# HuttleyLab/DiverseSeq

Hardware: AMD Instinct MI355X
Metric: sequences scored/sec (delta-JSD, k=6) (higher is better)
Workload: dtype f64 (results and every set update in f64; reject/accept decisions tiered: f32 and f32-log scores decide rows farther from the threshold than their proven error bands, f64 the rest)

## Files before the change

### diverseseq_amd/csrc/api.cpp

```cpp
#include "dvs_internal.h"

#include <cmath>
#include <cstring>
#include <mutex>

uint64_t dvs_pow_u64(uint32_t base, uint32_t exp, bool *overflow);
void dvs_matrix_free_fields(dvs_matrix *m);
int dvs_matrix_fill_counts(dvs_ctx *ctx, dvs_matrix *m, const dvs_seq_view &sv, const uint64_t *offsets, bool no_wait);
int dvs_matrix_fill_freq_entropy(dvs_ctx *ctx, dvs_matrix *m);
int dvs_hist_prepare(dvs_ctx *ctx, const uint64_t *offsets, uint32_t nseq, uint32_t k, uint64_t nbins, uint64_t nbytes, size_t *n_long_out);
bool dvs_hist_rows_fit_u16(const dvs_ctx *ctx, uint64_t B, size_t n_long);
int dvs_matrix_fill_freq_totals(dvs_ctx *ctx, dvs_matrix *m, const double *d_meta);
int dvs_matrix_fill_compacted(dvs_ctx *ctx, dvs_matrix *m, const double *d_in, const double *d_meta);

static std::string g_create_err;

int dvs_set_error(dvs_ctx *ctx, int code, const char *fmt, ...) {
    char buf[512];
    va_list ap;
    va_start(ap, fmt);
    vsnprintf(buf, sizeof buf, fmt, ap);
    va_end(ap);
    if (ctx) ctx->err = buf;
    else g_create_err = buf;
    return code;
}

int dvs_hip_fail(dvs_ctx *ctx, hipError_t e, const char *what) {
    (void)hipGetLastError();
    const int code = (e == hipErrorOutOfMemory) ? DVS_ERR_NOMEM : DVS_ERR_RUNTIME;
    return dvs_set_error(ctx, code, "HIP error %d (%s) in %s", int(e), hipGetErrorString(e), what);
}

int dvs_dev_alloc(dvs_ctx *ctx, void **ptr, size_t bytes, const char *what) {
    const size_t sz = ((bytes ? bytes : 1) + 4095) & ~size_t(4095);
    auto it = ctx->pool.find(sz);
    if (it != ctx->pool.end()) {
        *ptr = it->second;
        ctx->pool.erase(it);
        ctx->pool_bytes -= sz;
        ctx->live[*ptr] = sz;
        return DVS_OK;
    }
    hipError_t e = hipMalloc(ptr, sz);
    if (e != hipSuccess && !ctx->pool.empty()) {
        (void)hipGetLastError();
        dvs_dev_trim(ctx);
        e = hipMalloc(ptr, sz);
    }
    if (e != hipSuccess) {
        *ptr = nullptr;
        return dvs_hip_fail(ctx, e, what);
    }
    ctx->live[*ptr] = sz;
    return DVS_OK;
}

void dvs_dev_free(dvs_ctx *ctx, void *ptr) {
    if (!ptr) return;
    auto it = ctx ? ctx->live.find(ptr) : std::map<void *, size_t>::iterator();
    if (!ctx || it == ctx->live.end()) {
        (void)hipFree(ptr);
        return;
    }
    ctx->pool.emplace(it->second, ptr);
    ctx->pool_bytes += it->second;
    ctx->live.erase(it);
}

int dvs_pinned_get(dvs_ctx *ctx, void **ptr) {
    if (!ctx->pinned_pool.empty()) {
        *ptr = ctx->pinned_pool.back();
        ctx->pinned_pool.pop_back();
        return DVS_OK;
    }
    hipError_t e = hipHostMalloc(ptr, 4096, hipHostMallocDefault);
    if (e != hipSuccess) return dvs_hip_fail(ctx, e, "hipHostMalloc");
    return DVS_OK;
}
void dvs_pinned_put(dvs_ctx *ctx, void *ptr) {
    if (!ptr) return;
    if (ctx) ctx->pinned_pool.push_back(ptr);
    else (void)hipHostFree(ptr);
}
hipEvent_t dvs_event_get(dvs_ctx *ctx) {
    if (!ctx->event_pool.empty()) {
        hipEvent_t e = ctx->event_pool.back();
        ctx->event_pool.pop_back();
        return e;
    }
    hipEvent_t e = nullptr;
    (void)hipEventCreate(&e);
    return e;
}
void dvs_event_put(dvs_ctx *ctx, hipEvent_t e) {
    if (!e) return;
    if (ctx) ctx->event_pool.push_back(e);
    else (void)hipEventDestroy(e);
}

void dvs_dev_trim(dvs_ctx *ctx) {
    (void)hipStreamSynchronize(ctx->stream);
    for (auto &kv : ctx->pool) (void)hipFree(kv.second);
    ctx->pool.clear();
    ctx->pool_bytes = 0;
}

void dvs_knobs_from_env(dvs_knobs *k) {
    auto on = [](const char *name) { return getenv(name) != nullptr; };
    *k = dvs_knobs();
    k->no_uniform_offsets = on("DVS_NO_UNIFORM_OFFSETS");
    k->no_offsets_cache = on("DVS_NO_OFFSETS_CACHE");
    k->counts_u32 = on("DVS_COUNTS_U32");
    k->build_wait = on("DVS_BUILD_WAIT");
    k->no_packed_upload = on("DVS_NO_PACKED_UPLOAD");
    k->cu_mask_set = on("HSA_CU_MASK") || on("ROC_GLOBAL_CU_MASK");
    k->no_persist = on("DVS_NO_PERSIST");
    k->no_fast_step = on("DVS_NO_FAST_STEP");
    k->no_head_phase = on("DVS_NO_HEAD_PHASE");
    k->persist_no_seeded = on("DVS_PERSIST_NO_SEEDED");
    k->persist_no_small = on("DVS_PERSIST_NO_SMALL");
    k->persist_no_coarse = on("DVS_PERSIST_NO_COARSE");
    k->persist_no_events = on("DVS_PERSIST_NO_EVENTS");
    k->persist_debug = on("DVS_PERSIST_DEBUG");
    const char *rounds = getenv("DVS_PERSIST_WG_ROUNDS");
    k->persist_wg_rounds = rounds ? atoi(rounds) : -1;
    k->ingest_no_stream = on("DVS_INGEST_NO_STREAM");
    const char *tk = getenv("DVS_TEST_KNOBS");
    k->test_persist_fake_error = tk && strstr(tk, "fake_persist_error") != nullptr;
    if (const char *lt = tk ? strstr(tk, "long_tile_") : nullptr) k->test_long_tile = uint32_t(strtoul(lt + 10, nullptr, 10));
    k->test_rowlog_ring = 0;
    if (const char *rr = tk ? strstr(tk, "rowlog_ring_") : nullptr) k->test_rowlog_ring = uint32_t(strtoul(rr + 12, nullptr, 10));
}

extern "C" {

int dvs_abi_version(void) { return DVS_ABI_VERSION; }

int dvs_ctx_refresh_knobs(dvs_ctx *ctx) {
    if (!ctx) return dvs_set_error(ctx, DVS_ERR_VALUE, "null argument");
    dvs_knobs_from_env(&ctx->knobs);
    ctx->off_cache.n_off = 0;
    return DVS_OK;
}

int dvs_ctx_create(int device, void *stream, dvs_ctx **out) {
    if (!out) return dvs_set_error(nullptr, DVS_ERR_VALUE, "null argument");
    *out = nullptr;
    int ndev = 0;
    hipError_t e = hipGetDeviceCount(&ndev);
    if (e != hipSuccess || ndev == 0)
        return dvs_set_error(nullptr, DVS_ERR_RUNTIME,
                             "no HIP device available (%s): libdvs_hip has no CPU fallback",
                             e != hipSuccess ? hipGetErrorString(e) : "device count 0");
    if (device < 0) {
        e = hipGetDevice(&device);
        if (e != hipSuccess) return dvs_hip_fail(nullptr, e, "hipGetDevice");
    }
    if (device >= ndev)
        return dvs_set_error(nullptr, DVS_ERR_VALUE, "device %d out of range (%d devices)", device, ndev);
    e = hipSetDevice(device);
    if (e != hipSuccess) return dvs_hip_fail(nullptr, e, "hipSetDevice");
    hipDeviceProp_t prop;
    e = hipGetDeviceProperties(&prop, device);
    if (e != hipSuccess) return dvs_hip_fail(nullptr, e, "hipGetDeviceProperties");
    dvs_ctx *ctx = new dvs_ctx();
    dvs_knobs_from_env(&ctx->knobs);
    ctx->device = device;
    ctx->n_cu = prop.multiProcessorCount;
    ctx->lds_per_block = prop.sharedMemPerBlockOptin ? prop.sharedMemPerBlockOptin
                                                     : prop.sharedMemPerBlock;
    if (ctx->lds_per_block < prop.sharedMemPerBlock) ctx->lds_per_block = prop.sharedMemPerBlock;
    if (stream) {
        ctx->stream = static_cast<hipStream_t>(stream);
    } else {
        e = hipStreamCreateWithFlags(&ctx->stream, hipStreamNonBlocking);
        if (e != hipSuccess) {
            delete ctx;
            return dvs_hip_fail(nullptr, e, "hipStreamCreate");
        }
        ctx->own_stream = true;
    }
    *out = ctx;
    return DVS_OK;
}

void dvs_ctx_destroy(dvs_ctx *ctx) {
    if (!ctx || ctx->owner_gone) return;
    ctx->owner_gone = true;
    dvs_ctx_release(ctx);
}

}

int dvs_raise_dyn_lds(dvs_ctx *ctx, const void *fn, size_t bytes) {
    if (bytes <= 48 * 1024) return DVS_OK;
    size_t &have = ctx->lds_raised[fn];
    if (have >= bytes) return DVS_OK;
    DVS_HIP(ctx, hipFuncSetAttribute(fn, hipFuncAttributeMaxDynamicSharedMemorySize, int(bytes)));
    have = bytes;
    return DVS_OK;
}

hipStream_t dvs_ctx_stream2(dvs_ctx *ctx) {
    if (!ctx->stream2 && hipStreamCreateWithFlags(&ctx->stream2, hipStreamNonBlocking) != hipSuccess) {
        (void)hipGetLastError();
        ctx->stream2 = nullptr;
    }
    return ctx->stream2;
}

bool dvs_ctx_cu_split(dvs_ctx *ctx) {
    if (ctx->cu_split_tried) return ctx->stream_head != nullptr;
    ctx->cu_split_tried = true;
    if (ctx->n_cu < 128 || ctx->n_cu % 8) return false;
    if (ctx->knobs.cu_mask_set) return false;
    int head = 64;
    head = std::max(16, std::min(ctx->n_cu / 2, head)) & ~7;
    const uint32_t words = uint32_t(ctx->n_cu + 31) / 32;
    std::vector<uint32_t> lo(words, 0u), hi(words, 0u);
    for (int i = 0; i < ctx->n_cu; i++) (i < head ? lo : hi)[i / 32] |= 1u << (i % 32);
    hipStream_t a = nullptr, b = nullptr;
    if (hipExtStreamCreateWithCUMask(&a, words, lo.data()) != hipSuccess ||
        hipExtStreamCreateWithCUMask(&b, words, hi.data()) != hipSuccess) {
        (void)hipGetLastError();
        if (a) (void)hipStreamDestroy(a);
        return false;
    }
    ctx->stream_head = a;
    ctx->stream_rest = b;
    ctx->head_cus = head;
    return true;
}

void dvs_ctx_retain(dvs_ctx *ctx) {
    if (ctx) ctx->refs++;
}

void dvs_ctx_release(dvs_ctx *ctx) {
    if (!ctx || --ctx->refs > 0) return;
    (void)hipSetDevice(ctx->device);
    dvs_dev_free(ctx, ctx->off_cache.d_off);
    dvs_dev_free(ctx, ctx->off_cache.d_rows);
    dvs_dev_free(ctx, ctx->off_cache.d_tiles);
    if (ctx->off_cache.ev_up) (void)hipEventDestroy(ctx->off_cache.ev_up);
    if (ctx->off_cache.h_off) (void)hipHostFree(ctx->off_cache.h_off);
    if (ctx->pack_ev) (void)hipEventDestroy(ctx->pack_ev);
    if (ctx->h_pack) (void)hipHostFree(ctx->h_pack);
    dvs_dev_free(ctx, ctx->d_clog_tbl);
    dvs_dev_trim(ctx);
    for (void *p : ctx->pinned_pool) (void)hipHostFree(p);
    for (hipEvent_t e : ctx->event_pool) (void)hipEventDestroy(e);
    if (ctx->stream2) (void)hipStreamDestroy(ctx->stream2);
    if (ctx->stream_head) (void)hipStreamDestroy(ctx->stream_head);
    if (ctx->stream_rest) (void)hipStreamDestroy(ctx->stream_rest);
    if (ctx->own_stream && ctx->stream) (void)hipStreamDestroy(ctx->stream);
    delete ctx;
}

extern "C" {

const char *dvs_last_error(const dvs_ctx *ctx) { return ctx ? ctx->err.c_str() : g_create_err.c_str(); }

int dvs_ctx_trim(dvs_ctx *ctx) {
    if (!ctx) return DVS_ERR_VALUE;
    dvs_dev_trim(ctx);
    return DVS_OK;
}

int dvs_ctx_sync(dvs_ctx *ctx) {
    if (!ctx) return DVS_ERR_VALUE;
    DVS_HIP(ctx, hipStreamSynchronize(ctx->stream));
    return DVS_OK;
}

int dvs_ctx_set_timing(dvs_ctx *ctx, int on) {
    if (!ctx) return DVS_ERR_VALUE;
    ctx->timing = on != 0;
    return DVS_OK;
}

int dvs_ctx_device_info(dvs_ctx *ctx, char *name, size_t name_len, int *n_cu, uint64_t *hbm_bytes) {
    if (!ctx) return DVS_ERR_VALUE;
    hipDeviceProp_t prop;
    DVS_HIP(ctx, hipGetDeviceProperties(&prop, ctx->device));
    if (name && name_len) {
        snprintf(name, name_len, "%s (%s)", prop.name, prop.gcnArchName);
    }
    if (n_cu) *n_cu = prop.multiProcessorCount;
    if (hbm_bytes) *hbm_bytes = prop.totalGlobalMem;
    return DVS_OK;
}

static int matrix_alloc(dvs_ctx *ctx, dvs_matrix *m) {
    const size_t cells = size_t(m->nrows) * m->nbins;
    const size_t bytes = cells * (m->kind == 0 ? 4 : m->kind == 2 ? 2 : 8);
    size_t free_b = 0, total_b = 0;
    const bool cached = ctx->pool.count(((bytes ? bytes : 4) + 4095) & ~size_t(4095)) > 0;
    if (!cached) DVS_HIP(ctx, hipMemGetInfo(&free_b, &total_b));
    if (!cached && bytes + size_t(m->nrows) * 12 + (64u << 20) > free_b + ctx->pool_bytes)
        return dvs_set_error(ctx, DVS_ERR_NOMEM,
                             "%u x %llu matrix needs %zu bytes of HBM, %zu free", m->nrows,
                             (unsigned long long)m->nbins, bytes, free_b);
    const size_t nr = m->nrows ? m->nrows : 1;
    m->ctx = ctx;
    dvs_ctx_retain(ctx);
    int rc;
    if (m->kind == 0) rc = dvs_dev_alloc(ctx, (void **)&m->d_counts, bytes ? bytes : 4, "matrix counts");
    else if (m->kind == 2) rc = dvs_dev_alloc(ctx, (void **)&m->d_counts16, bytes ? bytes : 4, "matrix counts (16-bit)");
    else rc = dvs_dev_alloc(ctx, (void **)&m->d_freqs, bytes ? bytes : 8, "matrix freqs");
    if (!rc) rc = dvs_dev_alloc(ctx, (void **)&m->d_totals, nr * 4, "matrix totals");
    if (!rc) rc = dvs_dev_alloc(ctx, (void **)&m->d_entropy, nr * 8, "matrix entropy");
    return rc;
}

static int build_shape(dvs_ctx *ctx, uint32_t k, uint32_t num_states, uint64_t *B_out) {
    if (k == 0) return dvs_set_error(ctx, DVS_ERR_VALUE, "k cannot be 0");
    if (num_states < 1 || num_states > 255)
        return dvs_set_error(ctx, DVS_ERR_VALUE, "num_states %u outside 1..255", num_states);
    if (k > 17) return dvs_set_error(ctx, DVS_ERR_UNSUPPORTED, "k = %u > 17 is not supported", k);
    bool ovf = false;
    const uint64_t B = dvs_pow_u64(num_states, k, &ovf);
    if (ovf || B > (1ull << 32))
        return dvs_set_error(ctx, DVS_ERR_UNSUPPORTED, "%u^%u bins do not fit a dense count row",
                             num_states, k);
    *B_out = B;
    return DVS_OK;
}

static int matrix_build_view(dvs_ctx *ctx, const dvs_seq_view &sv, const uint64_t *offsets, uint32_t nseq, uint32_t k,
                             uint32_t num_states, bool no_wait, dvs_matrix **out) {
    *out = nullptr;
    uint64_t B = 0;
    const int arc = build_shape(ctx, k, num_states, &B);
    if (arc) return arc;
    size_t n_long = 0;
    if (nseq) {
        const int prc = dvs_hist_prepare(ctx, offsets, nseq, k, B, sv.nbytes, &n_long);
        if (prc) return prc;
    }
    dvs_matrix *m = new dvs_matrix();
    m->kind = (nseq && dvs_hist_rows_fit_u16(ctx, B, n_long)) ? 2 : 0;
    m->nrows = nseq;
    m->nbins = B;
    m->k = k;
    m->num_states = num_states;
    m->device = ctx->device;
    int rc = matrix_alloc(ctx, m);
    if (!rc && nseq) rc = dvs_matrix_fill_counts(ctx, m, sv, offsets, no_wait);
    if (rc) {
        dvs_matrix_free_fields(m);
        delete m;
        return rc;
    }
    *out = m;
    return DVS_OK;
}

int dvs_matrix_build(dvs_ctx *ctx, const uint8_t *seqs, int seqs_on_device, const uint64_t *offsets,
                     uint32_t nseq, uint32_t k, uint32_t num_states, dvs_matrix **out) {
    if (!ctx || !offsets || !out || (!seqs && nseq && offsets[nseq] > 0))
        return dvs_set_error(ctx, DVS_ERR_VALUE, "null argument");
    *out = nullptr;
    {
        uint64_t B_ = 0;
        const int arc = build_shape(ctx, k, num_states, &B_);
        if (arc) return arc;
    }
    DVS_HIP(ctx, hipSetDevice(ctx->device));
    const uint64_t nbytes = nseq ? offsets[nseq] : 0;
    dvs_seq_view sv;
    if (seqs_on_device) {
        if (reinterpret_cast<uintptr_t>(seqs) & 15)
            return dvs_set_error(ctx, DVS_ERR_VALUE, "device sequence buffer must be 16-byte aligned");
        sv.seqs = seqs;
        sv.nbytes = nbytes;
        return matrix_build_view(ctx, sv, offsets, nseq, k, num_states, !ctx->knobs.build_wait, out);
    }
    if (nbytes && dvs_packed_upload_wanted(ctx, num_states, nbytes)) {
        dvs_packed *p = nullptr;
        int rc = dvs_packed_alloc(ctx, nbytes, &p);
        if (!rc) rc = dvs_packed_fill_from_host(ctx, p, seqs);
        if (!rc) {
            sv.codes = p->d_codes;
            sv.mask = p->d_mask;
            sv.nbytes = nbytes;
            rc = matrix_build_view(ctx, sv, offsets, nseq, k, num_states, false, out);
        }
        if (p) {
            (void)hipStreamSynchronize(ctx->stream);
            dvs_packed_destroy(p);
        }
        return rc;
    }
    const uint64_t padded = ((nbytes + 15) & ~15ull) + 16;
    uint8_t *d_tmp = nullptr;
    int rc = dvs_dev_alloc(ctx, (void **)&d_tmp, padded, "sequence upload buffer");
    if (rc) return rc;
    hipError_t ue = hipMemsetAsync(d_tmp + (nbytes & ~15ull), 0xFF, padded - (nbytes & ~15ull), ctx->stream);
    if (ue == hipSuccess && nbytes) ue = hipMemcpyAsync(d_tmp, seqs, nbytes, hipMemcpyHostToDevice, ctx->stream);
    if (ue != hipSuccess) {
        (void)hipStreamSynchronize(ctx->stream);
        dvs_dev_free(ctx, d_tmp);
        return dvs_hip_fail(ctx, ue, "sequence upload");
    }
    sv.seqs = d_tmp;
    sv.nbytes = padded;
    rc = matrix_build_view(ctx, sv, offsets, nseq, k, num_states, false, out);
    (void)hipStreamSynchronize(ctx->stream);
    dvs_dev_free(ctx, d_tmp);
    return rc;
}

int dvs_matrix_build_packed(dvs_ctx *ctx, const dvs_packed *p, const uint64_t *offsets, uint32_t nseq, uint32_t k,
                            dvs_matrix **out) {
    if (!ctx || !p || !offsets || !out) return dvs_set_error(ctx, DVS_ERR_VALUE, "null argument");
    *out = nullptr;
    DVS_HIP(ctx, hipSetDevice(ctx->device));
    dvs_seq_view sv;
    sv.codes = p->d_codes;
    sv.mask = p->d_mask;
    sv.nbytes = p->nbases;
    p->async_readers = true;
    return matrix_build_view(ctx, sv, offsets, nseq, k, 4, !ctx->knobs.build_wait, out);
}

int dvs_matrix_from_freqs(dvs_ctx *ctx, const double *freqs, uint32_t nrows, uint64_t nbins,
                          dvs_matrix **out) {
    if (!ctx || !out || (!freqs && nrows)) return dvs_set_error(ctx, DVS_ERR_VALUE, "null argument");
    *out = nullptr;
    if (nbins == 0)
        return dvs_set_error(ctx, DVS_ERR_VALUE, "cannot calculate entropy as frequency vector empty");
    const double tol = double(nbins) * DVS_EPS;
    for (uint32_t r = 0; r < nrows; r++) {
        const double *row = freqs + uint64_t(r) * nbins;
        double tot = 0.0;
        for (uint64_t i = 0; i < nbins; i++)
            if (row[i] != 0.0) tot += row[i];
        if (!(std::fabs(tot - 1.0) <= tol))
            return dvs_set_error(ctx, DVS_ERR_VALUE,
                                 "cannot calculate entropy as frequency vector total %.17g!=1.0", tot);
    }
    DVS_HIP(ctx, hipSetDevice(ctx->device));
    dvs_matrix *m = new dvs_matrix();
    m->kind = 1;
    m->nrows = nrows;
    m->nbins = nbins;
    m->device = ctx->device;
    int rc = matrix_alloc(ctx, m);
    if (!rc && nrows) {
        std::vector<uint32_t> ones(nrows, 1u);
        hipError_t e = hipMemcpyAsync(m->d_freqs, freqs, size_t(nrows) * nbins * 8,
                                      hipMemcpyHostToDevice, ctx->stream);
        if (e == hipSuccess)
            e = hipMemcpyAsync(m->d_totals, ones.data(), size_t(nrows) * 4, hipMemcpyHostToDevice,
                               ctx->stream);
        if (e != hipSuccess) rc = dvs_hip_fail(ctx, e, "hipMemcpyAsync(freqs)");
        if (!rc) rc = dvs_matrix_fill_freq_entropy(ctx, m);
        if (!rc && hipStreamSynchronize(ctx->stream) != hipSuccess)
            rc = dvs_set_error(ctx, DVS_ERR_RUNTIME, "stream sync failed");
    }
    if (rc) {
        dvs_matrix_free_fields(m);
        delete m;
        return rc;
// ... 118 lines not shown
```

### diverseseq_amd/csrc/dvs_internal.h

```cpp
#pragma once

#include <hip/hip_runtime.h>

#include <cstdarg>
#include <cstdint>
#include <cstdio>
#include <map>
#include <string>
#include <vector>

#include "../../include/dvs_hip.h"

#define DVS_EPS 2.220446049250313e-16
#define DVS_HEAD_ROWS 1024u

struct dvs_knobs {
    bool no_uniform_offsets = false;
    bool no_offsets_cache = false;
    bool counts_u32 = false;
    bool build_wait = false;
    bool no_packed_upload = false;
    bool cu_mask_set = false;
    bool no_fast_step = false;
    bool no_persist = false;
    bool no_head_phase = false;
    bool persist_no_seeded = false;
    bool persist_no_small = false;
    bool persist_no_coarse = false;
    bool persist_no_events = false;
    bool persist_debug = false;
    int persist_wg_rounds = -1;
    bool ingest_no_stream = false;
    bool test_persist_fake_error = false;
    uint32_t test_long_tile = 0;
    uint32_t test_rowlog_ring = 0;
};
void dvs_knobs_from_env(dvs_knobs *k);

struct dvs_ctx {
    dvs_knobs knobs;
    int device = 0;
    hipStream_t stream = nullptr;
    bool own_stream = false;
    hipStream_t stream2 = nullptr;
    hipStream_t stream_head = nullptr, stream_rest = nullptr;
    int head_cus = 0;
    bool cu_split_tried = false;
    int persist_timeouts = 0;
    int n_cu = 0;
    size_t lds_per_block = 0;
    double *d_clog_tbl = nullptr;
    bool timing = false;
    std::string err;
    std::multimap<size_t, void *> pool;
    std::vector<void *> pinned_pool;
    std::vector<hipEvent_t> event_pool;
    std::map<void *, size_t> live;
    size_t pool_bytes = 0;
    int refs = 1;
    bool owner_gone = false;
    std::map<const void *, size_t> lds_raised;
    std::map<std::pair<const void *, size_t>, bool> persist_fits;
    struct OffsetsCache {
        uint64_t *h_off = nullptr;
        size_t h_cap = 0, n_off = 0;
        hipEvent_t ev_up = nullptr;
        std::vector<uint32_t> h_long_rows;
        std::vector<unsigned char> h_tiles;
        uint64_t nbytes = 0;
        uint32_t k = 0;
        void *d_off = nullptr, *d_rows = nullptr, *d_tiles = nullptr;
        size_t d_off_cap = 0;
        size_t n_long = 0, n_tiles = 0;
        bool uniform = false;
        uint64_t uni_base = 0, uni_stride = 0;
    } off_cache;
    void *h_pack = nullptr;
    size_t h_pack_cap = 0;
    hipEvent_t pack_ev = nullptr;
};
int dvs_raise_dyn_lds(dvs_ctx *ctx, const void *fn, size_t bytes);
void dvs_ctx_retain(dvs_ctx *ctx);
hipStream_t dvs_ctx_stream2(dvs_ctx *ctx);
bool dvs_ctx_cu_split(dvs_ctx *ctx);
void dvs_ctx_release(dvs_ctx *ctx);

struct dvs_matrix;
int dvs_matrix_settle(dvs_ctx *ctx, const dvs_matrix *m);
int dvs_dev_alloc(dvs_ctx *ctx, void **ptr, size_t bytes, const char *what);
void dvs_dev_free(dvs_ctx *ctx, void *ptr);
void dvs_dev_trim(dvs_ctx *ctx);
int dvs_pinned_get(dvs_ctx *ctx, void **ptr);
void dvs_pinned_put(dvs_ctx *ctx, void *ptr);
hipEvent_t dvs_event_get(dvs_ctx *ctx);
void dvs_event_put(dvs_ctx *ctx, hipEvent_t e);

int dvs_set_error(dvs_ctx *ctx, int code, const char *fmt, ...);
int dvs_hip_fail(dvs_ctx *ctx, hipError_t e, const char *what);

#define DVS_HIP(ctx, call)                                        \
    do {                                                          \
        hipError_t e__ = (call);                                  \
        if (e__ != hipSuccess) return dvs_hip_fail(ctx, e__, #call); \
    } while (0)

struct dvs_matrix {
    int kind = 0;
    uint16_t *d_counts16 = nullptr;
    uint32_t nrows = 0;
    uint64_t nbins = 0;
    uint32_t k = 0, num_states = 0;
    uint32_t *d_counts = nullptr;
    double *d_freqs = nullptr;
    uint32_t *d_totals = nullptr;
    double *d_entropy = nullptr;
    uint32_t *d_src_row = nullptr;
    std::vector<uint32_t> h_head_totals;
    uint32_t *h_head_pinned = nullptr;
    hipEvent_t ev_built = nullptr;
    hipEvent_t ev_join = nullptr;
    uint32_t head_count = 0;
    uint32_t head_rows_built = 0;
    bool rest_beside_head = false;
    int device = 0;
    dvs_ctx *ctx = nullptr;
};

struct dvs_packed {
    dvs_ctx *ctx = nullptr;
    uint32_t *d_codes = nullptr;
    uint16_t *d_mask = nullptr;
    uint64_t nbases = 0, nwords = 0;
    mutable bool async_readers = false;
};
struct dvs_seq_view {
    const uint8_t *seqs = nullptr;
    const uint32_t *codes = nullptr;
    const uint16_t *mask = nullptr;
    uint64_t nbytes = 0;
};
int dvs_packed_alloc(dvs_ctx *ctx, uint64_t nbases, dvs_packed **out);
int dvs_packed_fill_from_device(dvs_ctx *ctx, dvs_packed *p, const uint8_t *d_seqs);
int dvs_packed_fill_from_host(dvs_ctx *ctx, dvs_packed *p, const uint8_t *seqs);
bool dvs_packed_upload_wanted(const dvs_ctx *ctx, uint32_t num_states, uint64_t nbytes);

template <typename F>
auto dvs_mat_dispatch(const dvs_matrix *m, F &&f) {
    if (m->kind == 0) return f(static_cast<const uint32_t *>(m->d_counts));
    if (m->kind == 2) return f(static_cast<const uint16_t *>(m->d_counts16));
    return f(static_cast<const double *>(m->d_freqs));
}

#ifdef __HIPCC__
__device__ __forceinline__ uint32_t dvs_pack4(uint32_t w) {
    const uint32_t x = w & 0x03030303u;
    return ((x << 6) | (x >> 4) | (x >> 14) | (x >> 24)) & 0xFFu;
}
__device__ __forceinline__ uint32_t dvs_inv4(uint32_t w) {
    uint32_t t = w & 0xFCFCFCFCu;
    t |= t >> 4;
    t |= t >> 2;
    t |= t >> 1;
    t &= 0x01010101u;
    return ((t << 3) | (t >> 6) | (t >> 15) | (t >> 24)) & 0xFu;
}
__device__ __forceinline__ uint32_t dvs_pack16(uint4 v) {
    return (dvs_pack4(v.x) << 24) | (dvs_pack4(v.y) << 16) | (dvs_pack4(v.z) << 8) | dvs_pack4(v.w);
}
__device__ __forceinline__ uint32_t dvs_inv16(uint4 v) {
    return (dvs_inv4(v.x) << 12) | (dvs_inv4(v.y) << 8) | (dvs_inv4(v.z) << 4) | dvs_inv4(v.w);
}
__device__ __forceinline__ double dvs_wave_sum(double v) {
#pragma unroll
    for (int o = 32; o > 0; o >>= 1) v += __shfl_xor(v, o, 64);
    return v;
}
template <int CTRL>
__device__ __forceinline__ double dvs_dpp_mov(double v) {
    const long long b = __double_as_longlong(v);
    int lo = int(b), hi = int(b >> 32);
    lo = __builtin_amdgcn_update_dpp(0, lo, CTRL, 0xF, 0xF, true);
    hi = __builtin_amdgcn_update_dpp(0, hi, CTRL, 0xF, 0xF, true);
    return __longlong_as_double((long long)(((unsigned long long)(unsigned)hi << 32) | (unsigned)lo));
}
__device__ __forceinline__ double dvs_wave_sum_dpp(double v) {
    v += dvs_dpp_mov<0xB1>(v);
    v += dvs_dpp_mov<0x4E>(v);
    v += dvs_dpp_mov<0x141>(v);
    v += dvs_dpp_mov<0x140>(v);
    const long long b = __double_as_longlong(v);
    const int lo = int(b), hi = int(b >> 32);
    auto row = [&](int l) {
        return __longlong_as_double((long long)(((unsigned long long)(unsigned)__builtin_amdgcn_readlane(hi, l) << 32) |
                                                (unsigned)__builtin_amdgcn_readlane(lo, l)));
    };
    return (row(0) + row(16)) + (row(32) + row(48));
}
__device__ __forceinline__ double dvs_wave_min(double v) {
#pragma unroll
    for (int o = 32; o > 0; o >>= 1) v = fmin(v, __shfl_xor(v, o, 64));
    return v;
}
__device__ __forceinline__ double dvs_wave_min_dpp(double v) {
    v = fmin(v, dvs_dpp_mov<0xB1>(v));
    v = fmin(v, dvs_dpp_mov<0x4E>(v));
    v = fmin(v, dvs_dpp_mov<0x141>(v));
    v = fmin(v, dvs_dpp_mov<0x140>(v));
    const long long b = __double_as_longlong(v);
    const int lo = int(b), hi = int(b >> 32);
    auto row = [&](int l) {
        return __longlong_as_double((long long)(((unsigned long long)(unsigned)__builtin_amdgcn_readlane(hi, l) << 32) |
                                                (unsigned)__builtin_amdgcn_readlane(lo, l)));
    };
    return fmin(fmin(row(0), row(16)), fmin(row(32), row(48)));
}
__device__ __forceinline__ unsigned long long dvs_wave_sum_u64(unsigned long long v) {
#pragma unroll
    for (int o = 32; o > 0; o >>= 1) v += __shfl_xor(v, o, 64);
    return v;
}
__device__ __forceinline__ double dvs_block_sum(double v, double *scratch) {
    const int lane = threadIdx.x & 63, wave = threadIdx.x >> 6;
    const int nwave = (blockDim.x + 63) >> 6;
    v = dvs_wave_sum(v);
    __syncthreads();
    if (lane == 0) scratch[wave] = v;
    __syncthreads();
    double t = 0.0;
    for (int i = 0; i < nwave; i++) t += scratch[i];
    return t;
}
__device__ __forceinline__ double dvs_block_min(double v, double *scratch) {
    const int lane = threadIdx.x & 63, wave = threadIdx.x >> 6;
    const int nwave = (blockDim.x + 63) >> 6;
    v = dvs_wave_min(v);
    __syncthreads();
    if (lane == 0) scratch[wave] = v;
    __syncthreads();
    double t = scratch[0];
    for (int i = 1; i < nwave; i++) t = fmin(t, scratch[i]);
    return t;
}
#endif
```

### diverseseq_amd/csrc/kmer_hist.hip

```cpp
#include "dvs_internal.h"

#include <algorithm>
#include <cstring>
#include <cmath>
#include <cstdlib>

namespace {

constexpr int HIST_THREADS = 256;
constexpr int HIST_MAX_THREADS = 512;
constexpr uint32_t TILE_LEN = 32768;
static_assert(TILE_LEN < 65536, "a whole-sequence tile's counts must fit the packed 16-bit LDS counters");
constexpr int CLOG_TBL = 256;

struct KTile {
    uint64_t begin;
    uint64_t end;
    uint64_t seq_begin;
    uint32_t row;
    uint32_t single;
};

__device__ __forceinline__ uint4 load16(const uint8_t *base, uint64_t off, uint64_t nbytes) {
    if (off + 16 <= nbytes) return *reinterpret_cast<const uint4 *>(base + off);
    uint32_t w[4] = {0xFFFFFFFFu, 0xFFFFFFFFu, 0xFFFFFFFFu, 0xFFFFFFFFu};
    for (int i = 0; i < 16; i++) {
        if (off + i < nbytes) {
            w[i >> 2] &= ~(0xFFu << (8 * (i & 3)));
            w[i >> 2] |= uint32_t(base[off + i]) << (8 * (i & 3));
        }
    }
    return make_uint4(w[0], w[1], w[2], w[3]);
}

template <bool LDS_HIST, bool PK16 = false>
__device__ __forceinline__ void bump(uint32_t *hist, uint32_t idx) {
    if (PK16) atomicAdd(&hist[idx >> 1], (idx & 1u) ? 0x10000u : 1u);
    else atomicAdd(&hist[idx], 1u);
}

__device__ __forceinline__ double clog2c(uint32_t c, const double *tbl) {
    if (c < CLOG_TBL) return tbl[c];
    const double d = double(c);
    return d * log2(d);
}

template <bool NS4, bool LDS_HIST, bool PK16 = false, bool OUT16 = false, bool PACKED = false>
__global__ __launch_bounds__(HIST_MAX_THREADS) void kmer_hist_kernel(
    const uint8_t *__restrict__ seqs, const uint16_t *__restrict__ pmask, uint64_t nbytes,
    const uint64_t *__restrict__ offsets,
    const KTile *__restrict__ tiles, uint32_t *__restrict__ counts, uint32_t *__restrict__ totals,
    double *__restrict__ entropy, const double *__restrict__ clog_tbl, uint32_t k, uint32_t ns,
    uint64_t B, uint32_t hot_rows, uint32_t row0, uint64_t uni_base, uint64_t uni_stride) {
    extern __shared__ __attribute__((aligned(16))) unsigned char smem[];
    KTile t;
    if (tiles) {
        t = tiles[blockIdx.x];
    } else {
        const uint32_t r = row0 + (hot_rows ? gridDim.x - 1 - blockIdx.x : blockIdx.x);
        const uint64_t s0 = offsets ? offsets[r] : uni_base + uint64_t(r) * uni_stride;
        const uint64_t s1 = offsets ? offsets[r + 1] : s0 + uni_stride;
        t.row = r;
        t.single = 1;
        t.seq_begin = s0;
        t.begin = s0 + k - 1;
        t.end = s1;
        if (s1 - s0 >= k && s1 - t.begin > TILE_LEN) return;
        if (s1 - s0 < k) t.begin = t.end = s1;
    }
    static_assert(!OUT16 || PK16, "16-bit rows come from the packed histogram");
    static_assert(!PACKED || NS4, "only four-state sequences have a packed form");
    uint32_t *row = OUT16 ? counts + uint64_t(t.row) * (B / 2) : counts + uint64_t(t.row) * B;
    uint32_t *hist = LDS_HIST ? reinterpret_cast<uint32_t *>(smem) : row;
    double *tbl = reinterpret_cast<double *>(smem + (LDS_HIST ? ((B * (PK16 ? 2 : 4) + 15) & ~15ull) : 0));
    double *scratch = tbl + CLOG_TBL;
    const int tid = threadIdx.x;
    const int nthreads = blockDim.x;

    if (LDS_HIST) {
        if ((B & 3) == 0) {
            uint4 *h4 = reinterpret_cast<uint4 *>(hist);
            for (uint64_t i = tid; i < B / (PK16 ? 8 : 4); i += nthreads) h4[i] = make_uint4(0, 0, 0, 0);
            if (PK16 && (B & 7) && tid == 0) reinterpret_cast<uint2 *>(hist)[B / 4 - 1] = make_uint2(0, 0);
        } else {
            for (uint64_t i = tid; i < B; i += nthreads) hist[i] = 0;
        }
    }
    for (int i = tid; i < CLOG_TBL; i += nthreads) tbl[i] = clog_tbl[i];
    __syncthreads();

    uint32_t nvalid = 0;
    const uint64_t abase = t.begin & ~15ull;
    const uint64_t nchunks = t.end > t.begin ? (t.end - abase + 15) >> 4 : 0;
    const uint32_t bmask = uint32_t(B - 1);

    if (NS4) {
        const uint32_t lane = tid & 63, wave = tid >> 6, nwaves = (nthreads + 63) >> 6;
        const uint64_t per_wave = ((nchunks + nwaves - 1) / nwaves + 63) & ~63ull;
        const uint64_t c_lo = uint64_t(wave) * per_wave;
        const uint64_t c_hi = c_lo + per_wave < nchunks ? c_lo + per_wave : nchunks;
        uint32_t carryP = 0, carryI = 0xFFFFu;
        if (c_lo < c_hi) {
            const uint64_t A0 = abase + (c_lo << 4);
            if (A0 >= 16) {
                if constexpr (PACKED) {
                    carryP = reinterpret_cast<const uint32_t *>(seqs)[(A0 >> 4) - 1];
                    carryI = pmask[(A0 >> 4) - 1];
                } else {
                    const uint4 pv = load16(seqs, A0 - 16, nbytes);
                    carryP = dvs_pack16(pv);
                    carryI = dvs_inv16(pv);
                }
            }
        }
        for (uint64_t c0 = c_lo; c0 < c_hi; c0 += 64) {
            const uint64_t c = c0 + lane;
            const bool live = c < c_hi;
            const uint64_t A = abase + ((live ? c : c_hi - 1) << 4);
            uint32_t Pc, Ic = 0;
            if constexpr (PACKED) {
                Pc = reinterpret_cast<const uint32_t *>(seqs)[A >> 4];
                Ic = pmask[A >> 4];
            } else {
                const uint4 cur = load16(seqs, A, nbytes);
                Pc = dvs_pack16(cur);
                const uint32_t hib = (cur.x | cur.y | cur.z | cur.w) & 0xFCFCFCFCu;
                if (__ballot(hib != 0)) Ic = dvs_inv16(cur);
            }
            const uint32_t Pp = uint32_t(__builtin_amdgcn_update_dpp(int(carryP), int(Pc), 0x138, 0xF, 0xF, false));
            const uint32_t Ip = uint32_t(__builtin_amdgcn_update_dpp(int(carryI), int(Ic), 0x138, 0xF, 0xF, false));
            carryP = uint32_t(__builtin_amdgcn_readlane(int(Pc), 63));
            carryI = uint32_t(__builtin_amdgcn_readlane(int(Ic), 63));
            const uint64_t P = (uint64_t(Pp) << 32) | Pc;
            uint32_t I = (Ip << 16) | Ic;
            const int64_t lead = int64_t(t.seq_begin) - (int64_t(A) - 16);
            if (lead > 0) I |= (lead >= 32) ? 0xFFFFFFFFu : ~(0xFFFFFFFFu >> lead);
            uint32_t W = I;
            if (__ballot(I != 0)) {
                uint32_t cover = 1;
                while (2 * cover <= k) {
                    W |= W >> cover;
                    cover *= 2;
                }
                if (cover < k) W |= W >> (k - cover);
            }
            const uint32_t lo = t.begin > A ? uint32_t(t.begin - A < 16 ? t.begin - A : 16) : 0u;
            const uint32_t hi = t.end > A ? uint32_t(t.end - A < 16 ? t.end - A : 16) : 0u;
            const uint32_t R = (live && hi > lo) ? ((0xFFFFu >> lo) & ~(0xFFFFu >> hi)) : 0u;
            const uint32_t ok = R & ~W & 0xFFFFu;
            nvalid += __popc(ok);
            if (__ballot(ok != 0xFFFFu) == 0) {
                if constexpr (PK16) {
                    const uint64_t P2 = P << 1;
                    const uint32_t p2lo = uint32_t(P2), p2hi = uint32_t(P2 >> 32);
                    const uint32_t amask = (bmask << 1) & ~3u;
                    unsigned char *hb = smem;
#pragma unroll
                    for (int j = 0; j < 16; j++) {
                        const uint32_t tq = __builtin_amdgcn_alignbit(p2hi, p2lo, 2 * (15 - j));
                        uint32_t half = __builtin_amdgcn_ubfe(tq, 1, 1);
                        asm volatile("" : "+v"(half));
                        atomicAdd(reinterpret_cast<uint32_t *>(hb + (tq & amask)), __umul24(half, 0xFFFFu) + 1u);
                    }
                } else {
#pragma unroll
                    for (int j = 0; j < 16; j++) bump<LDS_HIST, PK16>(hist, uint32_t(P >> (2 * (15 - j))) & bmask);
                }
            } else {
#pragma unroll
                for (int j = 0; j < 16; j++) {
                    const uint32_t idx = uint32_t(P >> (2 * (15 - j))) & bmask;
                    if ((ok >> (15 - j)) & 1u) bump<LDS_HIST, PK16>(hist, idx);
                }
            }
        }
    } else {
        for (uint64_t c = tid; c < nchunks; c += nthreads) {
            const uint64_t A = abase + (c << 4);
            const uint4 cur = load16(seqs, A, nbytes);
            const uint4 prev = (A >= 16) ? load16(seqs, A - 16, nbytes)
                                         : make_uint4(0xFFFFFFFFu, 0xFFFFFFFFu, 0xFFFFFFFFu, 0xFFFFFFFFu);
            const int64_t lead = int64_t(t.seq_begin) - (int64_t(A) - 16);
            const uint32_t w[8] = {prev.x, prev.y, prev.z, prev.w, cur.x, cur.y, cur.z, cur.w};
            uint32_t idx = 0, run = 0;
            const uint32_t Bd = uint32_t(B / ns);
#pragma unroll
            for (int q = 0; q < 32; q++) {
                const uint32_t b = (w[q >> 2] >> (8 * (q & 3))) & 0xFFu;
                const bool ok = (b < ns) && (int64_t(q) >= lead);
                idx = ok ? (idx % Bd) * ns + b : 0u;
                run = ok ? run + 1 : 0u;
                if (q >= 16) {
                    const uint64_t p = A + (q - 16);
                    if (p >= t.begin && p < t.end && run >= k) {
                        bump<LDS_HIST, PK16>(hist, idx);
                        nvalid++;
                    }
                }
            }
        }
    }
    if (!LDS_HIST) __threadfence();
    __syncthreads();

    if constexpr (PK16) {
        const uint2 *h2 = reinterpret_cast<const uint2 *>(hist);
        uint4 *r4 = reinterpret_cast<uint4 *>(row);
        typedef uint32_t u32x4 __attribute__((ext_vector_type(4)));
        double sv[2] = {0.0, 0.0}, tv[2] = {0.0, 0.0};
#pragma unroll
        for (int half = 0; half < 2; half++)
            for (uint64_t u = uint64_t(tid) + 128u * half; u < B / 4; u += HIST_THREADS) {
                const uint2 w = h2[u];
                const uint4 v = make_uint4(w.x & 0xFFFFu, w.x >> 16, w.y & 0xFFFFu, w.y >> 16);
                if constexpr (OUT16) {
                    typedef uint32_t u32x2 __attribute__((ext_vector_type(2)));
                    uint2 *r2 = reinterpret_cast<uint2 *>(row);
                    if (t.row < hot_rows) r2[u] = w;
                    else __builtin_nontemporal_store((u32x2){w.x, w.y}, reinterpret_cast<u32x2 *>(r2 + u));
                } else if (t.row < hot_rows) r4[u] = v;
                else __builtin_nontemporal_store((u32x4){v.x, v.y, v.z, v.w}, reinterpret_cast<u32x4 *>(r4 + u));
                if (((w.x | w.y) & 0xFF00FF00u) == 0) sv[half] += ((tbl[v.x] + tbl[v.y]) + tbl[v.z]) + tbl[v.w];
                else sv[half] += clog2c(v.x, tbl) + clog2c(v.y, tbl) + clog2c(v.z, tbl) + clog2c(v.w, tbl);
            }
        tv[0] = double(nvalid);
        const int lane = tid & 63, wave = tid >> 6;
        double sums[2];
#pragma unroll
        for (int q = 0; q < 2; q++) {
            const double a = dvs_wave_sum(q ? tv[0] : sv[0]), b = dvs_wave_sum(q ? tv[1] : sv[1]);
            __syncthreads();
            if (lane == 0) {
                scratch[wave] = a;
                scratch[wave + 2] = b;
            }
            __syncthreads();
            double acc = 0.0;
            for (int i = 0; i < 4; i++) acc += scratch[i];
            sums[q] = acc;
        }
        if (tid == 0) {
            totals[t.row] = uint32_t(sums[1]);
            entropy[t.row] = sums[1] > 0.0 ? log2(sums[1]) - sums[0] / sums[1] : 0.0;
        }
    } else if (t.single) {
        double s = 0.0, tot = 0.0;
        if (tid >= HIST_THREADS) {
        } else if (LDS_HIST) {
            if ((B & 3) == 0) {
                const uint4 *h4 = reinterpret_cast<const uint4 *>(hist);
                uint4 *r4 = reinterpret_cast<uint4 *>(row);
                for (uint64_t i = tid; i < B / 4; i += HIST_THREADS) {
                    const uint4 v = h4[i];
                    typedef uint32_t u32x4 __attribute__((ext_vector_type(4)));
                    if (t.row < hot_rows) r4[i] = v;
                    else __builtin_nontemporal_store((u32x4){v.x, v.y, v.z, v.w}, reinterpret_cast<u32x4 *>(r4 + i));
                    s += clog2c(v.x, tbl) + clog2c(v.y, tbl) + clog2c(v.z, tbl) + clog2c(v.w, tbl);
                    tot += double(v.x) + double(v.y) + double(v.z) + double(v.w);
                }
            } else {
                for (uint64_t i = tid; i < B; i += HIST_THREADS) {
                    const uint32_t v = hist[i];
                    row[i] = v;
                    s += clog2c(v, tbl);
                    tot += double(v);
                }
            }
        } else {
            for (uint64_t i = tid; i < B; i += HIST_THREADS) {
                const uint32_t v = __hip_atomic_load(&row[i], __ATOMIC_RELAXED, __HIP_MEMORY_SCOPE_AGENT);
                s += clog2c(v, tbl);
                tot += double(v);
            }
        }
        s = dvs_block_sum(s, scratch);
        tot = dvs_block_sum(tot, scratch);
        if (tid == 0) {
            totals[t.row] = uint32_t(tot);
            entropy[t.row] = tot > 0.0 ? log2(tot) - s / tot : 0.0;
        }
    } else if (LDS_HIST) {
        for (uint64_t i = tid; i < B; i += nthreads) {
            const uint32_t v = hist[i];
            if (v) atomicAdd(&row[i], v);
        }
    }
}

__global__ void clog_tbl_kernel(double *tbl) {
    const int c = threadIdx.x;
    tbl[c] = c ? double(c) * log2(double(c)) : 0.0;
}

__global__ __launch_bounds__(HIST_THREADS) void row_stats_kernel(
    const uint32_t *__restrict__ counts, const uint32_t *__restrict__ rows,
    uint32_t *__restrict__ totals, double *__restrict__ entropy, uint64_t B) {
    __shared__ double tbl[CLOG_TBL];
    __shared__ double scratch[32];
    const int tid = threadIdx.x;
    if (tid < CLOG_TBL) tbl[tid] = tid ? double(tid) * log2(double(tid)) : 0.0;
    __syncthreads();
    const uint32_t r = rows[blockIdx.x];
    const uint32_t *row = counts + uint64_t(r) * B;
    double s = 0.0, tot = 0.0;
    for (uint64_t i = tid; i < B; i += HIST_THREADS) {
        const uint32_t v = row[i];
        s += clog2c(v, tbl);
        tot += double(v);
    }
    s = dvs_block_sum(s, scratch);
    tot = dvs_block_sum(tot, scratch);
    if (tid == 0) {
        totals[r] = uint32_t(tot);
        entropy[r] = tot > 0.0 ? log2(tot) - s / tot : 0.0;
    }
}

__global__ __launch_bounds__(HIST_THREADS) void zero_rows_kernel(uint32_t *__restrict__ counts,
                                                                const uint32_t *__restrict__ rows,
                                                                uint64_t B) {
    uint32_t *row = counts + uint64_t(rows[blockIdx.x]) * B;
    for (uint64_t i = threadIdx.x; i < B; i += HIST_THREADS) row[i] = 0;
}

__global__ __launch_bounds__(HIST_THREADS) void freq_entropy_kernel(
    const double *__restrict__ freqs, double *__restrict__ entropy, uint64_t B) {
    __shared__ double scratch[32];
    const double *row = freqs + uint64_t(blockIdx.x) * B;
    double h = 0.0;
    for (uint64_t i = threadIdx.x; i < B; i += HIST_THREADS) {
        const double f = row[i];
        if (f != 0.0) h += -f * log2(f);
    }
    h = dvs_block_sum(h, scratch);
    if (threadIdx.x == 0) entropy[blockIdx.x] = h;
}

__global__ __launch_bounds__(HIST_THREADS) void compact_freq_rows_kernel(
    const double *__restrict__ in, const double *__restrict__ meta, double *__restrict__ out,
    uint32_t *__restrict__ totals, uint32_t *__restrict__ src, uint32_t nrows, uint64_t B) {
    __shared__ uint32_t s_cnt[2];
    const uint32_t r = blockIdx.x;
    if (threadIdx.x < 2) s_cnt[threadIdx.x] = 0;
    __syncthreads();
    uint32_t before = 0, all = 0;
    for (uint32_t q = threadIdx.x; q < nrows; q += HIST_THREADS) {
        const uint32_t v = meta[2 * q + 1] != 0.0 ? 1u : 0u;
        all += v;
        if (q < r) before += v;
    }
    atomicAdd(&s_cnt[0], before);
    atomicAdd(&s_cnt[1], all);
    __syncthreads();
    const bool real = meta[2 * r + 1] != 0.0;
    const uint32_t dest = real ? s_cnt[0] : s_cnt[1] + (r - s_cnt[0]);
    const double *a = in + uint64_t(r) * B;
    double *o = out + uint64_t(dest) * B;
    for (uint64_t i = threadIdx.x; i < B; i += HIST_THREADS) o[i] = a[i];
    if (threadIdx.x == 0) {
        totals[dest] = real ? 1u : 0u;
        src[dest] = r;
    }
}

__global__ void freq_totals_kernel(uint32_t *__restrict__ totals, const double *__restrict__ meta,
                                   uint32_t nrows) {
    const uint32_t r = blockIdx.x * blockDim.x + threadIdx.x;
    if (r < nrows) totals[r] = (!meta || meta[2 * r + 1] != 0.0) ? 1u : 0u;
}

template <typename K>
int set_dyn_lds(dvs_ctx *ctx, K kernel, size_t bytes) {
    return dvs_raise_dyn_lds(ctx, reinterpret_cast<const void *>(kernel), bytes);
}

}

uint64_t dvs_pow_u64(uint32_t base, uint32_t exp, bool *overflow) {
    uint64_t r = 1;
    *overflow = false;
    for (uint32_t i = 0; i < exp; i++) {
        if (r > UINT64_MAX / (base ? base : 1)) *overflow = true;
        r *= base;
    }
    return r;
}

int dvs_matrix_settle(dvs_ctx *ctx, const dvs_matrix *cm) {
    dvs_matrix *m = const_cast<dvs_matrix *>(cm);
    if (!m || !m->ev_built) return DVS_OK;
    const hipError_t e = hipEventSynchronize(m->ev_built);
    if (e == hipSuccess) m->h_head_totals.assign(m->h_head_pinned, m->h_head_pinned + m->head_count);
    else m->h_head_totals.clear();
    dvs_event_put(m->ctx, m->ev_built);
    dvs_pinned_put(m->ctx, m->h_head_pinned);
    m->ev_built = nullptr;
    m->h_head_pinned = nullptr;
    if (e != hipSuccess) return dvs_hip_fail(ctx ? ctx : m->ctx, e, "histogram kernels");
    return DVS_OK;
}

void dvs_matrix_free_fields(dvs_matrix *m) {
    if (!m) return;
    (void)dvs_matrix_settle(m->ctx, m);
    if (m->ev_join) dvs_event_put(m->ctx, m->ev_join);
    m->ev_join = nullptr;
    dvs_dev_free(m->ctx, m->d_counts);
    dvs_dev_free(m->ctx, m->d_counts16);
    m->d_counts16 = nullptr;
    dvs_dev_free(m->ctx, m->d_freqs);
    dvs_dev_free(m->ctx, m->d_totals);
    dvs_dev_free(m->ctx, m->d_entropy);
    dvs_dev_free(m->ctx, m->d_src_row);
    m->d_src_row = nullptr;
    m->d_counts = nullptr;
    m->d_freqs = nullptr;
    m->d_totals = nullptr;
    m->d_entropy = nullptr;
    dvs_ctx_release(m->ctx);
    m->ctx = nullptr;
}

int dvs_hist_prepare(dvs_ctx *ctx, const uint64_t *offsets, uint32_t nseq, uint32_t k, uint64_t nbins, uint64_t nbytes,
                     size_t *n_long_out) {
    dvs_ctx::OffsetsCache &oc = ctx->off_cache;
    const size_t n_off = size_t(nseq) + 1;
    oc.uniform = false;
    if (nseq >= 1 && !ctx->knobs.no_uniform_offsets) {
        const uint64_t base = offsets[0], stride = offsets[1] - offsets[0];
        bool uni = offsets[1] >= offsets[0] && stride < uint64_t(TILE_LEN) + k;
        uint64_t diff = 0;
        for (uint32_t r = 0; r < nseq && uni; r += 4096) {
            const uint32_t e = std::min<uint32_t>(nseq, r + 4096);
            for (uint32_t q = r; q < e; q++) diff |= (offsets[q + 1] - offsets[q]) ^ stride;
            uni = diff == 0;
        }
        if (uni && base + uint64_t(nseq) * stride <= nbytes) {
            dvs_dev_free(ctx, oc.d_rows);
            dvs_dev_free(ctx, oc.d_tiles);
            oc.d_rows = oc.d_tiles = nullptr;
            oc.n_long = oc.n_tiles = 0;
            oc.n_off = 0;
            oc.uniform = true;
            oc.uni_base = base;
            oc.uni_stride = stride;
            *n_long_out = 0;
            return DVS_OK;
        }
    }
    const bool hit = oc.d_off && oc.h_off && oc.k == k && oc.nbytes == nbytes && oc.n_off == n_off &&
                     !ctx->knobs.no_offsets_cache && std::memcmp(oc.h_off, offsets, n_off * 8) == 0;
    if (!hit) {
        if (oc.ev_up) (void)hipEventSynchronize(oc.ev_up);
        if (oc.h_cap < n_off) {
            if (oc.h_off) (void)hipHostFree(oc.h_off);
            oc.h_off = nullptr;
            oc.h_cap = 0;
            const size_t cap = std::max<size_t>(n_off + n_off / 4, 1024);
            const hipError_t he = hipHostMalloc((void **)&oc.h_off, cap * 8, hipHostMallocDefault);
            if (he != hipSuccess) {
                oc.h_off = nullptr;
                return dvs_hip_fail(ctx, he, "pinned offsets block");
            }
            oc.h_cap = cap;
        }
        oc.n_off = 0;
        std::vector<KTile> tiles;
        std::vector<uint32_t> long_rows;
        uint64_t *dst = oc.h_off;
        uint64_t bad = 0, longest = 0;
        dst[0] = offsets[0];
        for (uint32_t r = 0; r < nseq; r++) {
            const uint64_t s0 = offsets[r], s1 = offsets[r + 1];
            dst[r + 1] = s1;
            bad |= uint64_t(s1 < s0) | uint64_t(s1 > nbytes);
            const uint64_t len = s1 - s0;
            longest = len > longest ? len : longest;
        }
        if (bad || longest >= uint64_t(TILE_LEN) + k) {
            uint64_t long_windows = 0;
            for (uint32_t r = 0; r < nseq; r++) {
                const uint64_t s0 = offsets[r], s1 = offsets[r + 1];
                if (s1 < s0 || s1 > nbytes)
                    return dvs_set_error(ctx, DVS_ERR_VALUE, "offsets[%u..%u] = %llu..%llu out of range", r,
                                         r + 1, (unsigned long long)s0, (unsigned long long)s1);
                if (s1 - s0 >= k && s1 - (s0 + k - 1) > TILE_LEN) long_windows += s1 - (s0 + k - 1);
            }
            uint64_t tile_long = TILE_LEN;
            {
                const uint64_t B_ = nbins ? nbins : 1;
                while (tile_long < 262144 && tile_long < 16 * B_ && long_windows / (2 * tile_long) >= 2048) tile_long *= 2;
                if (ctx->knobs.test_long_tile >= TILE_LEN) tile_long = std::min<uint64_t>(ctx->knobs.test_long_tile, uint64_t(1) << 20);
            }
            for (uint32_t r = 0; r < nseq; r++) {
                const uint64_t s0 = offsets[r], s1 = offsets[r + 1];
                if (s1 - s0 < k) continue;
                const uint64_t first = s0 + k - 1;
                if (s1 - first <= TILE_LEN) continue;
                long_rows.push_back(r);
                for (uint64_t b = first; b < s1; b += tile_long) {
                    KTile t;
                    t.begin = b;
                    t.end = std::min<uint64_t>(b + tile_long, s1);
                    t.seq_begin = s0;
                    t.row = r;
                    t.single = 0;
                    tiles.push_back(t);
                }
            }
        }
        dvs_dev_free(ctx, oc.d_rows);
        dvs_dev_free(ctx, oc.d_tiles);
        oc.d_rows = oc.d_tiles = nullptr;
        oc.n_long = oc.n_tiles = 0;
        int arc = DVS_OK;
        if (oc.d_off_cap < n_off) {
            dvs_dev_free(ctx, oc.d_off);
            oc.d_off = nullptr;
            oc.d_off_cap = 0;
            arc = dvs_dev_alloc(ctx, &oc.d_off, (n_off + n_off / 4) * 8, "offsets");
            if (!arc) oc.d_off_cap = n_off + n_off / 4;
        }
        if (!arc && !long_rows.empty()) arc = dvs_dev_alloc(ctx, &oc.d_rows, long_rows.size() * 4, "row list");
        if (!arc && !tiles.empty()) arc = dvs_dev_alloc(ctx, &oc.d_tiles, tiles.size() * sizeof(KTile), "tile list");
        hipError_t ue = hipSuccess;
        oc.h_tiles.assign(reinterpret_cast<const unsigned char *>(tiles.data()),
                          reinterpret_cast<const unsigned char *>(tiles.data()) + tiles.size() * sizeof(KTile));
        oc.h_long_rows = long_rows;
        if (!arc) ue = hipMemcpyAsync(oc.d_off, oc.h_off, n_off * 8, hipMemcpyHostToDevice, ctx->stream);
        if (!arc && ue == hipSuccess) {
            if (!oc.ev_up) oc.ev_up = dvs_event_get(ctx);
            if (oc.ev_up) ue = hipEventRecord(oc.ev_up, ctx->stream);
        }
        if (!arc && ue == hipSuccess && !long_rows.empty()) {
            ue = hipMemcpyAsync(oc.d_rows, oc.h_long_rows.data(), long_rows.size() * 4, hipMemcpyHostToDevice, ctx->stream);
            if (ue == hipSuccess)
                ue = hipMemcpyAsync(oc.d_tiles, oc.h_tiles.data(), oc.h_tiles.size(), hipMemcpyHostToDevice,
                                    ctx->stream);
        }
        if (arc || ue != hipSuccess) {
            dvs_dev_free(ctx, oc.d_rows);
            dvs_dev_free(ctx, oc.d_tiles);
            oc.d_rows = oc.d_tiles = nullptr;
            return arc ? arc : dvs_hip_fail(ctx, ue, "histogram setup");
        }
        oc.n_off = n_off;
        oc.nbytes = nbytes;
        oc.k = k;
        oc.n_long = long_rows.size();
        oc.n_tiles = tiles.size();
    }
    *n_long_out = oc.n_long;
    return DVS_OK;
}

bool dvs_hist_rows_fit_u16(const dvs_ctx *ctx, uint64_t B, size_t n_long) {
    return n_long == 0 && B <= 4096 && (B & 3) == 0 && !ctx->knobs.counts_u32;
}

int dvs_matrix_fill_counts(dvs_ctx *ctx, dvs_matrix *m, const dvs_seq_view &sv, const uint64_t *offsets,
                           bool no_wait) {
    const bool packed = sv.codes != nullptr;
    const uint8_t *d_seqs = packed ? reinterpret_cast<const uint8_t *>(sv.codes) : sv.seqs;
    const uint16_t *d_pmask = sv.mask;
    const uint64_t nbytes = sv.nbytes;
    const uint32_t nseq = m->nrows, k = m->k, ns = m->num_states;
    if (packed && ns != 4) return dvs_set_error(ctx, DVS_ERR_VALUE, "packed sequences have four states, not %u", ns);
    const uint64_t B = m->nbins;
    const bool lds_hist = B * 4 <= 64 * 1024;
    const bool ns4 = ns == 4;
    (void)offsets;
    dvs_ctx::OffsetsCache &oc = ctx->off_cache;
    uint64_t *d_off = oc.uniform ? nullptr : static_cast<uint64_t *>(oc.d_off);
    const uint64_t uni_base = oc.uni_base, uni_stride = oc.uni_stride;
    uint32_t *d_rows = static_cast<uint32_t *>(oc.d_rows);
    KTile *d_tiles = static_cast<KTile *>(oc.d_tiles);
    const size_t n_long = oc.n_long, n_tiles = oc.n_tiles;
    auto cleanup = [&]() {};
    int rc = DVS_OK;
    hipError_t e = hipSuccess;
    if (!lds_hist)
        e = hipMemsetAsync(m->d_counts, 0, size_t(nseq) * B * 4, ctx->stream);
    if (e == hipSuccess && n_long && lds_hist)
        hipLaunchKernelGGL(zero_rows_kernel, dim3(uint32_t(n_long)), dim3(HIST_THREADS), 0, ctx->stream,
                           m->d_counts, d_rows, B);
    if (e != hipSuccess) return dvs_hip_fail(ctx, e, "histogram setup");
    if (!ctx->d_clog_tbl) {
        rc = dvs_dev_alloc(ctx, (void **)&ctx->d_clog_tbl, CLOG_TBL * sizeof(double), "c log2 c table");
        if (rc) {
            cleanup();
            return rc;
        }
        hipLaunchKernelGGL(clog_tbl_kernel, dim3(1), dim3(CLOG_TBL), 0, ctx->stream, ctx->d_clog_tbl);
    }
    int nthreads = HIST_THREADS;
    const int tile_threads = (lds_hist && B * 4 > 32768) ? HIST_MAX_THREADS : HIST_THREADS;
    const size_t lds = (lds_hist ? ((B * 4 + 15) & ~15ull) : 0) + (CLOG_TBL + 32) * sizeof(double);
#define DVS_LAUNCH_HIST(NS4, LH, PKD, GRID, TILES, NTHR, HOT)                                             \
    do {                                                                                         \
        rc = set_dyn_lds(ctx, kmer_hist_kernel<NS4, LH, false, false, PKD>, lds);                \
        if (!rc)                                                                                 \
            hipLaunchKernelGGL((kmer_hist_kernel<NS4, LH, false, false, PKD>), dim3(GRID), dim3(NTHR), lds,  \
                               ctx->stream, d_seqs, d_pmask, nbytes, d_off, TILES, m->d_counts,  \
                               m->d_totals, m->d_entropy, ctx->d_clog_tbl, k, ns, B, HOT, 0u, uni_base, uni_stride);   \
    } while (0)
#define DVS_LAUNCH_HIST_ANY(GRID, TILES, NTHR, HOT)                            \
    do {                                                                  \
        if (packed && lds_hist) DVS_LAUNCH_HIST(true, true, true, GRID, TILES, NTHR, HOT);   \
        else if (packed) DVS_LAUNCH_HIST(true, false, true, GRID, TILES, NTHR, HOT);         \
        else if (ns4 && lds_hist) DVS_LAUNCH_HIST(true, true, false, GRID, TILES, NTHR, HOT);   \
        else if (ns4) DVS_LAUNCH_HIST(true, false, false, GRID, TILES, NTHR, HOT);         \
        else if (lds_hist) DVS_LAUNCH_HIST(false, true, false, GRID, TILES, NTHR, HOT);    \
        else DVS_LAUNCH_HIST(false, false, false, GRID, TILES, NTHR, HOT);                 \
    } while (0)
    uint32_t hot_rows = uint32_t(std::min<uint64_t>(nseq, (192ull << 20) / (B * (m->kind == 2 ? 2 : 4))));
    const bool pk16 = lds_hist && (B & 3) == 0;
    uint32_t head_rows = 0;
    if (m->kind == 2 && no_wait) {
        uint32_t want = DVS_HEAD_ROWS;
        head_rows = std::min<uint32_t>(nseq, want);
    }
    if (head_rows == nseq) head_rows = 0;
    bool head_event_done = false;
    if (m->kind == 2) {
        const size_t lds16 = ((B * 2 + 15) & ~15ull) + (CLOG_TBL + 32) * sizeof(double);
        uint32_t *out16 = reinterpret_cast<uint32_t *>(m->d_counts16);
        auto launch16 = [&](uint32_t row0, uint32_t count, uint32_t hot_end, hipStream_t on) {
            if (packed) {
                rc = set_dyn_lds(ctx, kmer_hist_kernel<true, true, true, true, true>, lds16);
                if (!rc)
                    hipLaunchKernelGGL((kmer_hist_kernel<true, true, true, true, true>), dim3(count), dim3(128), lds16, on,
                                       d_seqs, d_pmask, nbytes, d_off, static_cast<const KTile *>(nullptr), out16,
                                       m->d_totals, m->d_entropy, ctx->d_clog_tbl, k, ns, B, hot_end, row0, uni_base, uni_stride);
            } else if (ns4) {
                rc = set_dyn_lds(ctx, kmer_hist_kernel<true, true, true, true>, lds16);
                if (!rc)
                    hipLaunchKernelGGL((kmer_hist_kernel<true, true, true, true>), dim3(count), dim3(128), lds16, on,
                                       d_seqs, d_pmask, nbytes, d_off, static_cast<const KTile *>(nullptr), out16,
                                       m->d_totals, m->d_entropy, ctx->d_clog_tbl, k, ns, B, hot_end, row0, uni_base, uni_stride);
            } else {
                rc = set_dyn_lds(ctx, kmer_hist_kernel<false, true, true, true>, lds16);
                if (!rc)
                    hipLaunchKernelGGL((kmer_hist_kernel<false, true, true, true>), dim3(count), dim3(128), lds16, on,
                                       d_seqs, d_pmask, nbytes, d_off, static_cast<const KTile *>(nullptr), out16,
                                       m->d_totals, m->d_entropy, ctx->d_clog_tbl, k, ns, B, hot_end, row0, uni_base, uni_stride);
            }
        };
        if (head_rows) {
            const bool split = nseq - head_rows >= 16u * head_rows && dvs_ctx_cu_split(ctx);
            hipEvent_t ev_fork = split ? dvs_event_get(ctx) : nullptr;
            bool forked = ev_fork && hipEventRecord(ev_fork, ctx->stream) == hipSuccess &&
                          hipStreamWaitEvent(ctx->stream_rest, ev_fork, 0) == hipSuccess;
            launch16(0, head_rows, head_rows, ctx->stream);
            void *pin = nullptr;
            if (!rc && dvs_pinned_get(ctx, &pin) == DVS_OK) {
                m->head_count = uint32_t(std::min<size_t>(head_rows, 4096 / sizeof(uint32_t)));
                m->h_head_pinned = static_cast<uint32_t *>(pin);
                m->ev_built = dvs_event_get(ctx);
                if (m->ev_built &&
                    hipMemcpyAsync(m->h_head_pinned, m->d_totals, size_t(m->head_count) * 4, hipMemcpyDeviceToHost,
                                   ctx->stream) == hipSuccess &&
                    hipEventRecord(m->ev_built, ctx->stream) == hipSuccess) {
                    head_event_done = true;
                    m->head_rows_built = head_rows;
                } else {
                    if (m->ev_built) dvs_event_put(ctx, m->ev_built);
                    dvs_pinned_put(ctx, pin);
                    m->ev_built = nullptr;
                    m->h_head_pinned = nullptr;
                }
            }
            if (!rc) {
                const uint32_t hot_end = uint32_t(std::min<uint64_t>(nseq, uint64_t(head_rows) + hot_rows));
                forked = forked && head_event_done;
                launch16(head_rows, nseq - head_rows, hot_end, forked ? ctx->stream_rest : ctx->stream);
                if (forked) {
                    hipEvent_t ev_join = dvs_event_get(ctx);
                    if (!ev_join || hipEventRecord(ev_join, ctx->stream_rest) != hipSuccess ||
                        hipStreamWaitEvent(ctx->stream, ev_join, 0) != hipSuccess) {
                        (void)hipGetLastError();
                        (void)hipStreamSynchronize(ctx->stream_rest);
                    } else {
                        m->rest_beside_head = true;
                    }
                    m->ev_join = ev_join;
                }
            }
            if (ev_fork) dvs_event_put(ctx, ev_fork);
        } else {
            launch16(0, nseq, hot_rows, ctx->stream);
        }
    } else if (pk16) {
        const size_t lds16 = ((B * 2 + 15) & ~15ull) + (CLOG_TBL + 32) * sizeof(double);
        if (packed) {
            rc = set_dyn_lds(ctx, kmer_hist_kernel<true, true, true, false, true>, lds16);
            if (!rc)
                hipLaunchKernelGGL((kmer_hist_kernel<true, true, true, false, true>), dim3(nseq), dim3(128), lds16, ctx->stream,
                                   d_seqs, d_pmask, nbytes, d_off, static_cast<const KTile *>(nullptr), m->d_counts,
                                   m->d_totals, m->d_entropy, ctx->d_clog_tbl, k, ns, B, hot_rows, 0u, uni_base, uni_stride);
        } else if (ns4) {
            rc = set_dyn_lds(ctx, kmer_hist_kernel<true, true, true>, lds16);
            if (!rc)
                hipLaunchKernelGGL((kmer_hist_kernel<true, true, true>), dim3(nseq), dim3(128), lds16, ctx->stream,
                                   d_seqs, d_pmask, nbytes, d_off, static_cast<const KTile *>(nullptr), m->d_counts,
                                   m->d_totals, m->d_entropy, ctx->d_clog_tbl, k, ns, B, hot_rows, 0u, uni_base, uni_stride);
        } else {
            rc = set_dyn_lds(ctx, kmer_hist_kernel<false, true, true>, lds16);
            if (!rc)
                hipLaunchKernelGGL((kmer_hist_kernel<false, true, true>), dim3(nseq), dim3(128), lds16, ctx->stream,
                                   d_seqs, d_pmask, nbytes, d_off, static_cast<const KTile *>(nullptr), m->d_counts,
                                   m->d_totals, m->d_entropy, ctx->d_clog_tbl, k, ns, B, hot_rows, 0u, uni_base, uni_stride);
        }
    } else
        DVS_LAUNCH_HIST_ANY(nseq, static_cast<const KTile *>(nullptr), nthreads, hot_rows);
    if (!rc && n_tiles) {
        DVS_LAUNCH_HIST_ANY(uint32_t(n_tiles), d_tiles, tile_threads, 0u);
        if (!rc)
            hipLaunchKernelGGL(row_stats_kernel, dim3(uint32_t(n_long)), dim3(HIST_THREADS), 0,
                               ctx->stream, m->d_counts, d_rows, m->d_totals, m->d_entropy, B);
    }
#undef DVS_LAUNCH_HIST_ANY
#undef DVS_LAUNCH_HIST
    if (!rc && (e = hipGetLastError()) != hipSuccess) rc = dvs_hip_fail(ctx, e, "histogram launch");
    if (!rc && no_wait && head_event_done) return DVS_OK;
    if (!rc && no_wait) {
        void *pin = nullptr;
        if (dvs_pinned_get(ctx, &pin) == DVS_OK) {
            m->head_count = uint32_t(std::min<size_t>(nseq, 4096 / sizeof(uint32_t)));
            m->h_head_pinned = static_cast<uint32_t *>(pin);
            m->ev_built = dvs_event_get(ctx);
            if (m->ev_built &&
                hipMemcpyAsync(m->h_head_pinned, m->d_totals, size_t(m->head_count) * 4, hipMemcpyDeviceToHost,
                               ctx->stream) == hipSuccess &&
                hipEventRecord(m->ev_built, ctx->stream) == hipSuccess) {
                cleanup();
                return DVS_OK;
            }
            if (m->ev_built) dvs_event_put(ctx, m->ev_built);
            dvs_pinned_put(ctx, pin);
            m->ev_built = nullptr;
            m->h_head_pinned = nullptr;
        }
    }
    m->h_head_totals.assign(std::min<size_t>(nseq, 4096), 0u);
    if (!rc && !m->h_head_totals.empty() &&
        hipMemcpyAsync(m->h_head_totals.data(), m->d_totals, m->h_head_totals.size() * 4, hipMemcpyDeviceToHost,
                       ctx->stream) != hipSuccess)
        m->h_head_totals.clear();
    if (hipStreamSynchronize(ctx->stream) != hipSuccess && !rc)
        rc = dvs_set_error(ctx, DVS_ERR_RUNTIME, "histogram kernels failed");
    cleanup();
    return rc;
}

int dvs_matrix_fill_freq_entropy(dvs_ctx *ctx, dvs_matrix *m) {
    hipLaunchKernelGGL(freq_entropy_kernel, dim3(m->nrows), dim3(HIST_THREADS), 0, ctx->stream,
                       m->d_freqs, m->d_entropy, m->nbins);
    DVS_HIP(ctx, hipGetLastError());
    return DVS_OK;
}

int dvs_matrix_fill_compacted(dvs_ctx *ctx, dvs_matrix *m, const double *d_in, const double *d_meta) {
    hipLaunchKernelGGL(compact_freq_rows_kernel, dim3(m->nrows), dim3(HIST_THREADS), 0, ctx->stream, d_in, d_meta,
                       m->d_freqs, m->d_totals, m->d_src_row, m->nrows, m->nbins);
    DVS_HIP(ctx, hipGetLastError());
    return DVS_OK;
}

int dvs_matrix_fill_freq_totals(dvs_ctx *ctx, dvs_matrix *m, const double *d_meta) {
    hipLaunchKernelGGL(freq_totals_kernel, dim3((m->nrows + 255) / 256), dim3(256), 0, ctx->stream,
                       m->d_totals, d_meta, m->nrows);
    DVS_HIP(ctx, hipGetLastError());
    return DVS_OK;
}
```

### diverseseq_amd/csrc/persist.hip

```cpp
#include "select_dev.h"

#include <algorithm>
#include <type_traits>
#include <cstddef>
#include <cstdlib>
#include <cstring>

namespace {

constexpr int P_THREADS = 512;
constexpr int P_J = 8;
constexpr int P_CH = 16;
constexpr uint32_t P_MAXN = 512;
constexpr uint32_t P_MAXN_BIG = 256;
constexpr uint32_t P_MAXN_MAX = 896;
constexpr uint32_t p_maxn(bool cached, bool maxm = false) { return cached ? (maxm ? P_MAXN_MAX : P_MAXN) : P_MAXN_BIG; }
constexpr uint32_t P_SMALLN = 16;
constexpr uint32_t P_SMALL_ROWS = 13;
constexpr uint32_t p_maxjobs(bool cached, bool maxm = false) { return p_maxn(cached, maxm) + 1; }
constexpr size_t p_acc_bytes(uint32_t maxn) { return size_t(8) * (maxn + 1) * 2 * sizeof(unsigned long long); }
__device__ __forceinline__ unsigned long long p_acc_word(double v) {
    return ((unsigned long long)__double2ll_rn(v * 0x1p50) << 6) + 1ull;
}
__device__ __forceinline__ double p_acc_value(unsigned long long w) { return double((long long)w >> 6) * 0x1p-50; }
// ... 79 lines not shown
constexpr uint32_t P_TAG0 = 0xFFFFFEu;
constexpr uint32_t P_EPOCH_MAX = 0xFFFFF0u;
constexpr unsigned long long P_POS_NONE = (1ull << 37) - 1;
__device__ __forceinline__ unsigned long long p_word(uint32_t epoch, uint64_t pos, bool sure) {
    return ((unsigned long long)(P_TAG0 - epoch) << 40) | ((pos == SEL_NONE ? P_POS_NONE : pos) << 3) | (sure ? 0ull : 1ull);
}
__device__ __forceinline__ bool p_word_is(unsigned long long w, uint32_t epoch) { return uint32_t(w >> 40) == P_TAG0 - epoch; }
__device__ __forceinline__ uint64_t p_word_pos(unsigned long long w, uint32_t epoch) {
    const unsigned long long pos = (w >> 3) & P_POS_NONE;
    return (!p_word_is(w, epoch) || pos == P_POS_NONE) ? SEL_NONE : uint64_t(pos);
}
__device__ __forceinline__ bool p_word_sure(unsigned long long w) { return (w & 1ull) == 0; }
__device__ __forceinline__ uint32_t p_word_listed(unsigned long long w) { return uint32_t(w >> 1) & 3u; }

__device__ bool grid_barrier(PSync *sync, uint32_t G, uint32_t &gen, int *s_ok) {
    __syncthreads();
    if (threadIdx.x == 0) {
        const uint32_t target = gen + 1;
        const uint32_t x = blockIdx.x & 7u, ng = G < 8u ? G : 8u;
        const uint32_t gsz = (G - x + 7u) >> 3;
        int ok = 1;
        bool released = false;
        const bool last = G <= P_FLAT_GRID
                              ? __hip_atomic_fetch_add(&sync->count, 1u, RLX_AGENT) == G * target - 1
                              : (__hip_atomic_fetch_add(&sync->gcount[x].v, 1u, RLX_AGENT) == gsz * target - 1 &&
                                 __hip_atomic_fetch_add(&sync->count, 1u, RLX_AGENT) == ng * target - 1);
        if (last) {
            for (uint32_t g = 0; g < ng; g++) __hip_atomic_store(&sync->ggen[g].v, target, RLX_AGENT);
            released = true;
        }
        if (!released) {
            uint32_t spins = 0;
            while (__hip_atomic_load(&sync->ggen[x].v, RLX_AGENT) < target) {
                if ((++spins & 255u) == 0 &&
                    (spins > P_SPIN_LIMIT || __hip_atomic_load(&sync->timeout, RLX_AGENT))) {
                    __hip_atomic_store(&sync->timeout, 1u, RLX_AGENT);
                    ok = 0;
                    break;
                }
                __builtin_amdgcn_s_sleep(1);
            }
        }
        *s_ok = ok;
    }
    __syncthreads();
    gen++;
    return *s_ok != 0;
}

__device__ __forceinline__ uint4 p_load16_agent(const void *ptr) {
    uint4 v;
    asm volatile("global_load_dwordx4 %0, %1, off sc1\n\ts_waitcnt vmcnt(0)" : "=v"(v) : "v"(ptr) : "memory");
    return v;
}

struct PWin {
    uint32_t epoch;
    const unsigned long long *hintp;
    PRel *rel;
    unsigned long long *wgev;
    uint32_t *nlist;
    unsigned long long *mysoft;
};
__device__ __forceinline__ uint64_t p_hint_pos(const PWin &w) {
    return p_word_pos(__hip_atomic_load(w.hintp, RLX_AGENT), w.epoch);
}
__device__ __forceinline__ void p_post_event_wave(const PWin &w, uint64_t p, bool sure, uint32_t lane) {
    const unsigned long long word = p_word(w.epoch, p, sure);
    if (lane == 0) atomicMin(w.wgev, word);
    if (lane < 8) atomicMin(&w.rel[lane].hint, word);
}
__device__ __forceinline__ void p_post_event_thread(const PWin &w, uint64_t p, bool sure) {
    const unsigned long long word = p_word(w.epoch, p, sure);
    atomicMin(w.wgev, word);
    for (uint32_t g = 0; g < 8; g++) atomicMin(&w.rel[g].hint, word);
}
__device__ __forceinline__ void p_list_candidate(const PWin &w, uint64_t p) {
    const uint32_t idx = atomicAdd(w.nlist, 1u);
    if (idx < P_LIST) __hip_atomic_store(w.mysoft + idx, p_word(w.epoch, p, false), RLX_AGENT);
    else p_post_event_thread(w, p, false);
}
template <int CTRL>
__device__ __forceinline__ unsigned long long p_dpp_mov_u64(unsigned long long v) {
    int lo = int(uint32_t(v)), hi = int(uint32_t(v >> 32));
    lo = __builtin_amdgcn_update_dpp(0, lo, CTRL, 0xF, 0xF, true);
    hi = __builtin_amdgcn_update_dpp(0, hi, CTRL, 0xF, 0xF, true);
    return ((unsigned long long)uint32_t(hi) << 32) | uint32_t(lo);
}
__device__ __forceinline__ unsigned long long p_wave_min_u64(unsigned long long v) {
    auto mn = [](unsigned long long a, unsigned long long b) { return b < a ? b : a; };
    v = mn(v, p_dpp_mov_u64<0xB1>(v));
    v = mn(v, p_dpp_mov_u64<0x4E>(v));
    v = mn(v, p_dpp_mov_u64<0x141>(v));
    v = mn(v, p_dpp_mov_u64<0x140>(v));
    const int lo = int(uint32_t(v)), hi = int(uint32_t(v >> 32));
    auto row = [&](int l) {
        return ((unsigned long long)uint32_t(__builtin_amdgcn_readlane(hi, l)) << 32) | uint32_t(__builtin_amdgcn_readlane(lo, l));
    };
    return mn(mn(row(0), row(16)), mn(row(32), row(48)));
}

__device__ __forceinline__ unsigned long long p_gather(PSync *sync, uint32_t G, uint32_t epoch, unsigned long long own,
                                                       uint32_t lane, bool &ok, unsigned long long *seen_all = nullptr,
                                                       unsigned long long *stored = nullptr) {
    constexpr uint32_t Q = P_MAXG / 64;
    unsigned long long w[Q];
    bool have[Q];
#pragma unroll
    for (uint32_t q = 0; q < Q; q++) {
        w[q] = ~0ull;
        have[q] = lane + 64 * q >= G - 1;
    }
    uint32_t spins = 0;
    ok = true;
    for (;;) {
        unsigned long long got[Q];
#pragma unroll
        for (uint32_t q = 0; q < Q; q++)
            got[q] = have[q] ? 0ull : __hip_atomic_load(&sync->wrec[epoch & 1u][lane + 64 * q], RLX_AGENT);
        bool all = true;
#pragma unroll
        for (uint32_t q = 0; q < Q; q++) {
            if (!have[q] && p_word_is(got[q], epoch)) {
                w[q] = got[q];
                have[q] = true;
            }
            all = all && have[q];
        }
        if (__ballot(!all) == 0ull) break;
        if ((++spins & 255u) == 0 && (spins > P_SPIN_LIMIT || __hip_atomic_load(&sync->timeout, RLX_AGENT))) {
            ok = false;
            break;
        }
        __builtin_amdgcn_s_sleep(1);
    }
    if (seen_all) *seen_all = __builtin_amdgcn_s_memrealtime();
    unsigned long long m = own & ~6ull, fl = own & 6ull;
#pragma unroll
    for (uint32_t q = 0; q < Q; q++)
        if (lane + 64 * q < G - 1 && have[q]) {
            m = (w[q] & ~6ull) < m ? (w[q] & ~6ull) : m;
            fl |= w[q] & 6ull;
        }
    m = p_wave_min_u64(m);
    const bool anyl = __ballot(fl != 0ull) != 0ull;
    const unsigned long long relw = m | (anyl ? 2ull : 0ull);
    if (ok && lane < 8) __hip_atomic_store(&sync->rel[lane].rel, relw, RLX_AGENT);
    if (!ok && lane == 0) __hip_atomic_store(&sync->timeout, 1u, RLX_AGENT);
    if (stored) *stored = __builtin_amdgcn_s_memrealtime();
    return relw;
}

template <typename T, bool COARSE>
__device__ __forceinline__ void p_scan_rows(const T *__restrict__ mat,
                                            const uint32_t *__restrict__ totals,
                                            const double *__restrict__ rowH, const double *sl,
                                            const float *slf, uint64_t B, const PState &st, double he_base,
                                            const PWin &win,
                                            uint64_t first, uint64_t stride, uint64_t nrows,
                                            uint32_t lane, uint32_t &nread,
                                            uint32_t &nprecise, uint32_t &nmid, bool coarse_on,
                                            bool burst_drop = true) {
    const double dn = double(st.n), rn = 1.0 / dn;
    const double thr_lo = st.thr - st.band;
    const double thr_fast = thr_lo - FAST_BAND, thr_sure = st.thr + st.band + FAST_BAND;
    (void)thr_lo;
    const bool vec = (B & 255) == 0;
    const double cband = coarse_band(B);
    const double thr_c_lo = st.thr - st.band - cband, thr_c_hi = st.thr + st.band + cband;
    for (uint64_t r = first; r < nrows; r += stride) {
        const uint64_t p = st.cursor + r;
        const T *rp = mat + p * B;
        const uint64_t ev = p_hint_pos(win);
        const uint32_t tot = totals[p];
        const double hrow = rowH[p];
        if (ev < p) break;
        if (tot == 0) continue;
        const double rt = 1.0 / double(tot);
        const double mean_entropy = (he_base + hrow) / dn;
        nread++;
        if constexpr (COARSE) {
            if (vec && coarse_on) {
                const float rtn = float(rt * rn);
                const dvs_f2 r2 = {rtn, rtn};
                double c0 = 0.0, c1 = 0.0;
                bool done16 = false;
                if constexpr (sizeof(T) == 2) {
                    if (B == 4096) {
                        uint4 raw8[8];
#pragma unroll
                        for (int j = 0; j < 8; j++) raw8[j] = *reinterpret_cast<const uint4 *>(rp + j * 512 + lane * 8);
                        __builtin_amdgcn_sched_barrier(0);
#pragma unroll
                        for (int j = 0; j < 8; j++) {
                            asm volatile("" : "+v"(raw8[j].x), "+v"(raw8[j].y), "+v"(raw8[j].z), "+v"(raw8[j].w));
                            coarse8(raw8[j], slf + j * 512 + lane * 8, r2, c0, c1);
                        }
                        done16 = true;
                    }
                }
                if (!done16) {
                constexpr int C_CH = sizeof(T) == 2 ? 16 : 8;
                const uint64_t full = B - B % (256 * C_CH);
                uint64_t i0 = 0;
                bool dropped = false;
                for (; i0 < full; i0 += 256 * C_CH) {
                    if (i0 && burst_drop && p_hint_pos(win) < p) {
                        dropped = true;
                        break;
                    }
                    Raw4<T> raw[C_CH];
#pragma unroll
                    for (int j = 0; j < C_CH; j++) raw[j].load(rp + i0 + uint64_t(j) * 256 + lane * 4);
                    __builtin_amdgcn_sched_barrier(0);
#pragma unroll
                    for (int j = 0; j < C_CH; j += 2) {
                        const uint64_t i = i0 + uint64_t(j) * 256 + lane * 4;
                        raw[j].pin();
                        raw[j + 1].pin();
                        c0 += double(coarse4(raw[j].c, *reinterpret_cast<const float4 *>(slf + i), r2));
                        c1 += double(coarse4(raw[j + 1].c, *reinterpret_cast<const float4 *>(slf + i + 256), r2));
                    }
                }
                if (dropped) {
                    nread--;
                    break;
                }
                for (; i0 < B; i0 += 256) {
                    const uint64_t i = i0 + lane * 4;
                    Raw4<T> raw;
                    raw.load(rp + i);
                    c0 += double(coarse4(raw.c, *reinterpret_cast<const float4 *>(slf + i), r2));
                }
                }
                const double jf0 = -dvs_wave_sum_dpp(c0 + c1) - mean_entropy;
                if (!(jf0 > thr_c_lo)) continue;
                if (jf0 > thr_c_hi) {
                    p_post_event_wave(win, p, true, lane);
                    continue;
                }
                nmid++;
            }
        }
        double a0 = 0.0, a1 = 0.0, a2 = 0.0, a3 = 0.0, xmin = 0.0;
        if (vec) {
            constexpr int F_CH = COARSE ? P_CH / 2 : P_CH;
            const uint64_t full = B - B % (256 * F_CH);
            uint64_t i0 = 0;
            for (; i0 < full; i0 += 256 * F_CH) {
                Raw4<T> raw[F_CH];
#pragma unroll
                for (int j = 0; j < F_CH; j++) raw[j].load(rp + i0 + uint64_t(j) * 256 + lane * 4);
#pragma unroll
                for (int j = 0; j < F_CH; j++) {
                    const uint64_t i = i0 + uint64_t(j) * 256 + lane * 4;
                    const double2 b01 = *reinterpret_cast<const double2 *>(sl + i);
                    const double2 b23 = *reinterpret_cast<const double2 *>(sl + i + 2);
                    double v0, v1, v2, v3;
                    raw[j].get(v0, v1, v2, v3);
                    const double x0 = fma(v0, rt, b01.x) * rn, x1 = fma(v1, rt, b01.y) * rn;
                    const double x2 = fma(v2, rt, b23.x) * rn, x3 = fma(v3, rt, b23.y) * rn;
                    a0 += fast_neg_xlog2x(x0);
                    a1 += fast_neg_xlog2x(x1);
                    a2 += fast_neg_xlog2x(x2);
                    a3 += fast_neg_xlog2x(x3);
                    xmin = fmin(fmin(xmin, fmin(x0, x1)), fmin(x2, x3));
                }
            }
            for (; i0 < B; i0 += 256) {
                const uint64_t i = i0 + lane * 4;
                double v0, v1, v2, v3;
                load4(rp, i, v0, v1, v2, v3);
                const double2 b01 = *reinterpret_cast<const double2 *>(sl + i);
                const double2 b23 = *reinterpret_cast<const double2 *>(sl + i + 2);
                const double x0 = fma(v0, rt, b01.x) * rn, x1 = fma(v1, rt, b01.y) * rn;
                const double x2 = fma(v2, rt, b23.x) * rn, x3 = fma(v3, rt, b23.y) * rn;
                a0 += fast_neg_xlog2x(x0);
                a1 += fast_neg_xlog2x(x1);
                a2 += fast_neg_xlog2x(x2);
                a3 += fast_neg_xlog2x(x3);
                xmin = fmin(fmin(xmin, fmin(x0, x1)), fmin(x2, x3));
            }
        } else {
            for (uint64_t i = lane; i < B; i += 64) {
                const double x = fma(row_value(rp, i), rt, sl[i]) * rn;
                a0 += fast_neg_xlog2x(x);
                xmin = fmin(xmin, x);
            }
        }
        const double hf = dvs_wave_sum((a0 + a1) + (a2 + a3));
        const double mn = dvs_wave_min(xmin);
        const double jf = hf - mean_entropy;
        if (!(mn < 0.0) && jf > thr_sure) {
            p_post_event_wave(win, p, true, lane);
        } else if (!(mn < 0.0) && jf > thr_fast && lane == 0) {
            {
                nprecise++;
                p_list_candidate(win, p);
            }
        }
    }
}

template <typename T, bool COARSE>
__device__ __forceinline__ void p_scan_rows_wg(const T *__restrict__ mat, const uint32_t *__restrict__ totals,
                                               const double *__restrict__ rowH, const double *sl,
                                               const float *slf, uint64_t B,
                                               const PState &st, double he_base, const PWin &win,
                                               uint64_t first, uint64_t stride,
                                               uint64_t nrows, double *red, uint32_t &nread,
                                               uint32_t &nprecise, uint32_t &nmid, bool coarse_on,
                                            bool burst_drop = true) {
    const uint32_t tid = threadIdx.x, lane = tid & 63, wave = tid >> 6;
    const double dn = double(st.n), rn = 1.0 / dn;
    const double thr_fast = st.thr - st.band - FAST_BAND, thr_sure = st.thr + st.band + FAST_BAND;
    const bool vec = (B & 2047) == 0;
    const double cband = coarse_band(B);
    const double thr_c_lo = st.thr - st.band - cband, thr_c_hi = st.thr + st.band + cband;
    uint32_t par = 0;
    for (uint64_t r = first; r < nrows; r += stride, par ^= 1) {
        const uint64_t p = st.cursor + r;
        const T *rp = mat + p * B;
        const uint64_t ev = wave == 0 ? p_hint_pos(win) : 0ull;
        const uint32_t tot = totals[p];
        const double hrow = rowH[p];
        const double rt = tot ? 1.0 / double(tot) : 0.0;
        if constexpr (COARSE) {
            if (vec && B <= 4 * 2048 && coarse_on) {
                const float rtn = float(rt * rn);
                const dvs_f2 r2 = {rtn, rtn};
                double c0 = 0.0;
#pragma unroll
                for (int j = 0; j < 4; j++) {
                    const uint64_t i = uint64_t(j) * 2048 + tid * 4;
                    if (i < B) {
                        Raw4<T> raw;
                        raw.load(rp + i);
                        c0 += double(coarse4(raw.c, *reinterpret_cast<const float4 *>(slf + i), r2));
                    }
                }
                c0 = dvs_wave_sum_dpp(c0);
                double *cslot = red + 48 + par * 16;
                if (lane == 0) {
                    cslot[wave] = c0;
                    if (wave == 0) cslot[8] = __longlong_as_double((long long)ev);
                }
                __syncthreads();
                if ((unsigned long long)__double_as_longlong(cslot[8]) < p) break;
                if (tot == 0) continue;
                double hc = 0.0;
#pragma unroll
                for (int w = 0; w < P_THREADS / 64; w++) hc += cslot[w];
                const double jf0 = -hc - (he_base + hrow) / dn;
                if (tid == 0) nread++;
                if (!(jf0 > thr_c_lo)) continue;
                if (jf0 > thr_c_hi) {
                    if (tid < 8) p_post_event_wave(win, p, true, tid);
                    continue;
                }
                if (tid == 0) {
                    nmid++;
                    nread--;
                }
            }
        }
        double a0 = 0.0, a1 = 0.0, a2 = 0.0, a3 = 0.0, xmin = 0.0;
        if (vec) {
            for (uint64_t i0 = 0; i0 < B; i0 += 4 * 2048) {
                Raw4<T> raw[4];
#pragma unroll
                for (int j = 0; j < 4; j++)
                    if (i0 + uint64_t(j) * 2048 < B) raw[j].load(rp + i0 + uint64_t(j) * 2048 + tid * 4);
#pragma unroll
                for (int j = 0; j < 4; j++) {
                    const uint64_t i = i0 + uint64_t(j) * 2048 + tid * 4;
                    if (i < B) {
                        const double2 b01 = *reinterpret_cast<const double2 *>(sl + i);
                        const double2 b23 = *reinterpret_cast<const double2 *>(sl + i + 2);
                        double v0, v1, v2, v3;
                        raw[j].get(v0, v1, v2, v3);
                        const double x0 = fma(v0, rt, b01.x) * rn, x1 = fma(v1, rt, b01.y) * rn;
                        const double x2 = fma(v2, rt, b23.x) * rn, x3 = fma(v3, rt, b23.y) * rn;
                        a0 += fast_neg_xlog2x(x0);
                        a1 += fast_neg_xlog2x(x1);
                        a2 += fast_neg_xlog2x(x2);
                        a3 += fast_neg_xlog2x(x3);
                        xmin = fmin(fmin(xmin, fmin(x0, x1)), fmin(x2, x3));
                    }
                }
            }
        } else {
            for (uint64_t i = tid; i < B; i += P_THREADS) {
                const double x = fma(row_value(rp, i), rt, sl[i]) * rn;
                a0 += fast_neg_xlog2x(x);
                xmin = fmin(xmin, x);
            }
        }
        const double hw = dvs_wave_sum((a0 + a1) + (a2 + a3));
        const bool negw = __ballot(xmin < 0.0) != 0ull;
        double *slot = red + par * 24;
        if (lane == 0) {
            slot[wave] = hw;
            slot[8 + wave] = negw ? 1.0 : 0.0;
            if (wave == 0) slot[16] = __longlong_as_double((long long)ev);
        }
        __syncthreads();
        if ((unsigned long long)__double_as_longlong(slot[16]) < p) break;
        if (tot == 0) continue;
        double hf = 0.0, neg = 0.0;
#pragma unroll
        for (int w = 0; w < P_THREADS / 64; w++) {
            hf += slot[w];
            neg += slot[8 + w];
        }
        const double jf = hf - (he_base + hrow) / dn;
        if (tid < 8 && neg == 0.0 && jf > thr_fast && jf > thr_sure) p_post_event_wave(win, p, true, tid);
        if (tid == 0) {
            nread++;
            if (neg == 0.0 && jf > thr_fast) {
                if (jf > thr_sure) {
                } else {
                    nprecise++;
                    p_list_candidate(win, p);
                }
            }
        }
    }
}

template <typename T>
__device__ __forceinline__ void p_scan_rows_wg_stream(const T *__restrict__ mat,
                                                      const uint32_t *__restrict__ totals,
                                                      const double *__restrict__ rowH, const double *sl,
                                                      const float *slf, const PState &st, double he_base,
                                                      const PWin &win, uint64_t first,
                                                      uint64_t stride, uint64_t nrows, double *red,
                                                      uint32_t &nread, uint32_t &nprecise, uint32_t &nmid,
                                                      bool no_first_poll = true) {
    constexpr uint64_t B = 4096;
    constexpr int D = 4;
    const uint32_t tid = threadIdx.x, lane = tid & 63, wave = tid >> 6;
    const double dn = double(st.n), rn = 1.0 / dn;
    const double cband = coarse_band(B);
    const double thr_c_lo = st.thr - st.band - cband, thr_c_hi = st.thr + st.band + cband;
    constexpr bool W16 = sizeof(T) == 2;
    struct Row {
        Raw4<T> r0, r1;
        uint4 q;
        uint32_t tot;
        double hrow;
        unsigned long long ev;
    };
    auto issue = [&](Row &w, uint64_t r, bool poll) {
        const uint64_t p = st.cursor + r;
        const T *rp = mat + p * B;
        if constexpr (W16) {
            w.q = *reinterpret_cast<const uint4 *>(rp + tid * 8);
        } else {
            w.r0.load(rp + tid * 4);
            w.r1.load(rp + 2048 + tid * 4);
        }
        w.tot = totals[p];
        if (wave == 0) {
            w.hrow = rowH[p];
            w.ev = poll ? p_hint_pos(win) : SEL_NONE;
        }
    };
    uint32_t par = 0;
    auto process = [&](Row &w, uint64_t r) -> bool {
        const uint64_t p = st.cursor + r;
        const float rtn = w.tot ? float(rn / double(w.tot)) : 0.0f;
        const dvs_f2 r2 = {rtn, rtn};
        double c;
        if constexpr (W16) {
            asm volatile("" : "+v"(w.q.x), "+v"(w.q.y), "+v"(w.q.z), "+v"(w.q.w));
            double ca = 0.0, cb = 0.0;
            coarse8(w.q, slf + tid * 8, r2, ca, cb);
            c = ca + cb;
        } else {
            w.r0.pin();
            w.r1.pin();
            c = double(coarse4(w.r0.c, *reinterpret_cast<const float4 *>(slf + tid * 4), r2)) +
                double(coarse4(w.r1.c, *reinterpret_cast<const float4 *>(slf + 2048 + tid * 4), r2));
        }
        const double cs = dvs_wave_sum_dpp(c);
        double *slot = red + 48 + par * 16;
        par ^= 1;
        if (lane == 0) {
            slot[wave] = cs;
            if (wave == 0) {
                slot[8] = __longlong_as_double((long long)w.ev);
                slot[9] = w.hrow;
            }
        }
        __syncthreads();
        if ((unsigned long long)__double_as_longlong(slot[8]) < p) return false;
        if (w.tot == 0) return true;
        double hc = 0.0;
#pragma unroll
        for (int q = 0; q < P_THREADS / 64; q++) hc += slot[q];
        const double jf0 = -hc - (he_base + slot[9]) / dn;
        if (tid == 0) nread++;
        if (!(jf0 > thr_c_lo)) return true;
        if (jf0 > thr_c_hi) {
            if (tid < 8) p_post_event_wave(win, p, true, tid);
            return true;
        }
        if (tid == 0) {
            nmid++;
            nread--;
        }
        uint32_t nm = 0;
        p_scan_rows_wg<T, false>(mat, totals, rowH, sl, slf, B, st, he_base, win, r, nrows, nrows, red,
                                 nread, nprecise, nm, false);
        return true;
    };
    Row w[D];
#pragma unroll
    for (int d = 0; d < D; d++)
        if (first + uint64_t(d) * stride < nrows) issue(w[d], first + uint64_t(d) * stride, no_first_poll ? d >= 2 : true);
    for (uint64_t base = first; base < nrows; base += uint64_t(D) * stride) {
#pragma unroll
        for (int d = 0; d < D; d++) {
            const uint64_t r = base + uint64_t(d) * stride;
            if (r >= nrows) return;
            if (!process(w[d], r)) return;
            if (r + uint64_t(D) * stride < nrows) issue(w[d], r + uint64_t(D) * stride, true);
        }
    }
}

__device__ __forceinline__ uint32_t p_next_window(const PState &st, uint32_t nwg, uint32_t wg_thresh,
                                                  double wg_scale, bool &wgmode) {
    if (wg_thresh) {
        uint64_t w = uint64_t(double(st.cursor) * wg_scale / double(st.n ? st.n : 1u));
        w = (w + nwg - 1) / nwg * nwg;
        if (w < nwg) w = nwg;
        if (w <= uint64_t(wg_thresh) * nwg) {
            wgmode = true;
            return uint32_t(w);
        }
    }
    wgmode = false;
    return sel_next_window(st.cursor, st.n, st.wmin, st.wmax, st.wscale);
}

template <uint32_t Q>
__device__ __forceinline__ void p_argmin(const double *s_dl, const double *s_ds, uint32_t n, uint64_t B,
                                         uint32_t lane, double *scratch) {
    const double v0 = lane < n ? s_dl[lane] : 1e6;
    auto val = [&](uint32_t q) { return (Q == 1 || q == 0) ? v0 : s_dl[lane + 64 * q]; };
    double best = 1e6, acc = 0.0;
    bool rk = false;
#pragma unroll
    for (uint32_t q = 0; q < Q; q++) {
        const uint32_t r = lane + 64 * q;
        if (r < n) {
            const double v = val(q);
            rk |= sum_risky(s_ds[r], B);
            acc += v;
            if (v < best) best = v;
        }
    }
    const double dn = double(n);
    const double mnv = dvs_wave_min(best);
    double fi = 4294967295.0;
#pragma unroll
    for (uint32_t q = 0; q < Q; q++)
        if (mnv < 1e6 && lane + 64 * q < n && val(q) == mnv) fi = fmin(fi, double(lane + 64 * q));
    const double first = dvs_wave_min(fi);
    const uint32_t lw = (first < 4294967295.0) ? uint32_t(first) : 0u;
    const double mu = dvs_wave_sum(acc) / dn;
    double sec = 1e6, tv = 0.0;
#pragma unroll
    for (uint32_t q = 0; q < Q; q++) {
        const uint32_t r = lane + 64 * q;
        if (r < n) {
            const double v = val(q);
            if (r != lw && v < sec) sec = v;
            const double t = v - mu;
            tv += t * t;
        }
    }
    sec = dvs_wave_min(sec);
    const double var = dvs_wave_sum(tv);
    const unsigned long long anyr = __ballot(rk);
    if (lane == 0) {
        scratch[100] = mnv;
        scratch[101] = double(lw);
        scratch[102] = sec;
        scratch[103] = mu;
        scratch[104] = sqrt(var / (dn - 1.0));
        scratch[105] = anyr ? 1.0 : 0.0;
    }
}

template <typename T, bool CACHED, bool MAXM = false, bool SMALL = false>
__global__ __launch_bounds__(P_THREADS, 2) void persist_nmost_kernel(SelDev d, const T *__restrict__ mat,
                                                                    PSync *sync, unsigned long long *part, uint32_t G) {
    static_assert(!SMALL || (CACHED && !MAXM && sizeof(T) == 2), "SMALL: nmost, 16-bit rows, state in the register cache");
    constexpr uint32_t maxn = SMALL ? P_SMALLN : p_maxn(CACHED, MAXM);
    constexpr bool SPEC = CACHED && !MAXM && sizeof(T) <= 4;
    constexpr bool SPEC_BIG = !CACHED && !MAXM && sizeof(T) <= 4;
    constexpr bool OWN = SPEC && !SMALL;
    extern __shared__ __attribute__((aligned(16))) unsigned char smem[];
    const uint64_t B0 = d.B;
    const uint64_t B = B0;
    double *sl = reinterpret_cast<double *>(smem);
    constexpr bool COARSE = CACHED && sizeof(T) <= 4;
    float *slf = reinterpret_cast<float *>(sl + ((B + 1) & ~1ull));
    static_assert(!MAXM || CACHED, "the growth phase keeps the candidate's frequencies in registers");
    double *Sl = sl + ((B + 1) & ~1ull) + (COARSE ? ((B + 3) & ~3ull) / 2 : 0);
    double *scratch = Sl + (MAXM ? ((B + 1) & ~1ull) : 0);
    double *s_mH = scratch + 128;
    double *s_tot = s_mH + maxn;
    double *s_rt = s_tot + maxn;
    double *s_dl = s_rt + maxn;
    double *s_ds = s_dl + maxn;
    uint64_t *s_pos = reinterpret_cast<uint64_t *>(s_ds + maxn);
    uint32_t *s_slot = reinterpret_cast<uint32_t *>(s_pos + maxn);
    unsigned long long *s_win = reinterpret_cast<unsigned long long *>(s_slot + maxn + (maxn & 1));
    int *s_flag = reinterpret_cast<int *>(s_win + P_WINWORDS);
    static_assert(maxn % 4 == 0 && P_WINWORDS % 2 == 0, "s_ltab below must sit on a 16-byte boundary");
    double2 *s_ltab = reinterpret_cast<double2 *>(s_win + P_WINWORDS + 2);
    unsigned long long *s_prev = reinterpret_cast<unsigned long long *>(s_ltab + 128);
    unsigned char *s_tail = reinterpret_cast<unsigned char *>(s_prev + uint64_t(maxn + 1) * 2);
    [[maybe_unused]] uint16_t *s_rows = reinterpret_cast<uint16_t *>(s_tail);
    [[maybe_unused]] uint32_t *s_inv = reinterpret_cast<uint32_t *>(s_tail);
    [[maybe_unused]] T *s_own = reinterpret_cast<T *>(s_inv + maxn);
    [[maybe_unused]] double *s_bt = reinterpret_cast<double *>(s_tail);
    [[maybe_unused]] double *s_bH = s_bt + P_BATCH;
    [[maybe_unused]] double *s_bev = s_bH + P_BATCH;
    [[maybe_unused]] double *s_bpart = s_bev + 12 * P_BATCH;
    if (threadIdx.x < 128) log2_tab_fill(s_ltab, threadIdx.x);
    for (uint32_t i = threadIdx.x; i < (maxn + 1) * 2; i += P_THREADS) s_prev[i] = 0ull;
    SelCtl *ctl = d.ctl;
    const int tid0 = threadIdx.x;
    const int tid = tid0;
    [[maybe_unused]] const uint32_t lane = tid & 63, wave = tid >> 6;
    const bool two_roles = G >= 3;
    const bool gath = blockIdx.x == G - 1;
    const bool lead = blockIdx.x == (two_roles ? G - 2 : G - 1);
    const uint32_t n_work = G > 1 ? G - (two_roles ? 2u : 1u) : 1u;

    PState st;
    st.cursor = ctl->cursor;
    st.npos = ctl->npos;
    const bool head_phase = sync->stop_at != 0u && uint64_t(sync->stop_at) < st.npos;
    if (head_phase) st.npos = sync->stop_at;
    st.window = ctl->window;
    st.wmin = ctl->window_min;
    st.wmax = sync->wmax > ctl->window_max ? sync->wmax : ctl->window_max;
    st.n = ctl->size;
    st.li = ctl->lowest;
    st.sumH = ctl->sum_entropy;
    st.total_jsd = ctl->total_jsd;
    st.thr = ctl->thr;
    st.band = ctl->band;
    st.wscale = ctl->wscale;
    st.n_windows = st.n_events = st.n_accepts = 0;
    st.max_size = MAXM ? ctl->max_size : st.n;
    st.stat = ctl->stat;
    st.mean_d = ctl->mean_delta;
    st.std_d = ctl->std_delta;
    st.cov_d = ctl->cov_delta;
    if (lead && tid == 0) ctl->rows_before_launch = ctl->rows_scored;
    if (ctl->status != SEL_RUN || ctl->ev_kind != 0 || st.n > maxn || st.n < 2) {
        if (lead && tid == 0 && ctl->status == SEL_RUN) ctl->why[7]++;
        return;
    }
    if (MAXM && st.n < st.max_size && (ctl->s_is_resum == 0 || st.n + 2 > maxn)) {
        if (lead && tid == 0) ctl->why[6]++;
        return;
    }
    const bool seeded = !MAXM && CACHED && sync->seeded != 0u;
    for (uint32_t r = tid; r < st.n; r += P_THREADS) {
        const uint32_t slot = seeded ? r : d.ord[r];
        const uint64_t mp = seeded ? sync->seed_list[r] : d.mPos[slot];
        const double t = double(d.totals[mp]);
        s_slot[r] = slot;
        s_mH[r] = seeded ? d.rowH[mp] : d.mH[slot];
        s_pos[r] = mp;
        s_tot[r] = t;
        s_rt[r] = 1.0 / t;
    }
    __syncthreads();
    if (!seeded) {
        const double *low = d.M + uint64_t(s_slot[st.li]) * B;
        const double rn0 = 1.0 / double(st.n);
        for (uint64_t i = tid; i < B; i += P_THREADS) {
            const double v = d.S[i] - low[i];
            sl[i] = v;
            if (COARSE) slf[i] = coarse_sl(v, rn0);
            if (MAXM) Sl[i] = d.S[i];
        }
    }
    __syncthreads();

    uint32_t gen = 0, epoch = 0;
    uint32_t nread = 0, nprecise = 0, nmid = 0;
    uint32_t exit_status = SEL_RUN;
    uint32_t arb_stage = 0;
    uint64_t arb_pos = 0;
    uint32_t pend_kind = 0;
    bool bail = false;
    [[maybe_unused]] uint32_t mx_batch = 1;
    [[maybe_unused]] uint32_t n_batches = 0;
    uint32_t early_rec = 0xFFFFFFFFu;
    auto announce_early = [&](uint32_t next_epoch) {
        if (lead && two_roles && !MAXM) {
            if (threadIdx.x == 0)
                __hip_atomic_store(&sync->wrec[next_epoch & 1u][blockIdx.x], p_word(next_epoch, SEL_NONE, false), RLX_AGENT);
            early_rec = next_epoch;
        }
    };
    const uint64_t wpb = P_THREADS / 64;
    const uint32_t nwg = n_work;
    const uint64_t nwaves = uint64_t(nwg) * wpb;
    const uint32_t wg_thresh = sync->wg_thresh;
    const double wg_scale = double(sync->wg_scale);
    const bool coarse_on = (sync->no_coarse & 1u) == 0;
    bool wgmode = false;
    if (wg_thresh) st.window = p_next_window(st, nwg, wg_thresh, wg_scale, wgmode);
    const uint32_t nchunk = uint32_t((B + P_THREADS - 1) / P_THREADS);
    uint32_t K = 1, jobs = 0;
    bool one_job = false, has_job = false;
    auto set_geometry = [&](uint32_t members) {
        K = 1;
        const uint32_t kmax = (members + 1 <= n_work) ? n_work / (members + 1) : 1u;
        while (K * 2 <= kmax && K * 2 <= nchunk && K * 2 <= 32u) K *= 2;
        jobs = (members + 1) * K;
        one_job = jobs <= n_work && G > 1;
        has_job = one_job ? (blockIdx.x < jobs) : true;
    };
    set_geometry(st.n);

    if constexpr (!MAXM && CACHED) {
    if (seeded) {
        const uint32_t n = st.n;
        const double dn0 = double(n), rn0 = 1.0 / dn0, rdiv0 = 1.0 / (dn0 - 1.0);
        double Sreg[P_J];
#pragma unroll
        for (int j = 0; j < P_J; j++) Sreg[j] = 0.0;
        for (uint32_t r0 = 0; r0 < n; r0 += 4) {
            T cv[4][P_J];
#pragma unroll
            for (uint32_t q = 0; q < 4; q++) {
                const T *mrow = mat + s_pos[r0 + q < n ? r0 + q : r0] * B;
#pragma unroll
                for (int j = 0; j < P_J; j++) {
                    const uint64_t i = uint64_t(j) * P_THREADS + tid;
                    if (i < B) cv[q][j] = mrow[i];
                }
            }
#pragma unroll
            for (uint32_t q = 0; q < 4; q++) {
                if (r0 + q < n) {
                    const double mt = s_tot[r0 + q], mr = s_rt[r0 + q];
#pragma unroll
                    for (int j = 0; j < P_J; j++) {
                        const uint64_t i = uint64_t(j) * P_THREADS + tid;
                        if (i < B) Sreg[j] += count_freq_x(cv[q][j], mt, mr);
                    }
                }
            }
        }
        double sh = 0.0;
        for (uint32_t r = 0; r < n; r++) sh += s_mH[r];
#pragma unroll
        for (int j = 0; j < P_J; j++) {
            const uint64_t i = uint64_t(j) * P_THREADS + tid;
            if (i < B) {
                sl[i] = Sreg[j];
                if (lead) d.S[i] = Sreg[j];
            }
        }
        __syncthreads();
        unsigned long long *acc_all = part;
        const unsigned long long *acc = acc_all + uint64_t(blockIdx.x & 7u) * (maxn + 1) * 2;
        bool first_job = true;
        for (uint32_t job = blockIdx.x; job < jobs && has_job; job += G) {
            if ((lead || gath) && one_job) break;
            const uint32_t r = job / K, part_i = job % K;
            const T *mrow = mat + (r < n ? s_pos[r] : 0) * B;
            const double mtot = r < n ? s_tot[r] : 1.0, mrt = r < n ? s_rt[r] : 1.0;
            double h = 0.0, sv = 0.0;
#pragma unroll
            for (int j = 0; j < P_J; j++) {
                const uint64_t i = uint64_t(j) * P_THREADS + tid;
                if ((uint32_t(j) & (K - 1)) == part_i && i < B) {
                    double u;
                    if (r == n) {
                        u = Sreg[j] * rn0;
                    } else {
                        u = (Sreg[j] - count_freq_x(mrow[i], mtot, mrt)) * rdiv0;
                        if (u <= DVS_EPS) u = 0.0;
                    }
                    if (u > 0.0) h -= u * log2_tab(u, s_ltab);
                    sv += u;
                }
            }
            h = dvs_wave_sum_dpp(h);
            sv = dvs_wave_sum_dpp(sv);
            if (!first_job) __syncthreads();
            first_job = false;
            if (lane == 0) {
                scratch[64 + wave] = h;
                scratch[80 + wave] = sv;
            }
            __syncthreads();
            if (tid < 8) {
                double th = 0.0, ts = 0.0;
                for (uint32_t w = 0; w < P_THREADS / 64; w++) {
                    th += scratch[64 + w];
                    ts += scratch[80 + w];
                }
                unsigned long long *dst = acc_all + (uint64_t(tid) * (maxn + 1) + r) * 2;
                p_acc_add(dst, th, ts);
            }
        }
        if (!grid_barrier(sync, G, gen, s_flag)) {
            if (lead && tid == 0) ctl->status = SEL_ERROR;
            return;
        }
        bool acc_ok = true;
        for (uint32_t r = tid; r <= n; r += P_THREADS) {
            const double h = p_acc_value(p_acc_complete(acc + uint64_t(r) * 2, s_prev + uint64_t(r) * 2, K, acc_ok));
            const double sv = p_acc_value(p_acc_complete(acc + uint64_t(r) * 2 + 1, s_prev + uint64_t(r) * 2 + 1, K, acc_ok));
            if (r == n) {
                scratch[110] = h;
                scratch[111] = sv;
            } else {
                s_dl[r] = h - (sh - s_mH[r]) * rdiv0;
                s_ds[r] = sv;
            }
        }
        if (__syncthreads_or(acc_ok ? 0 : 1)) {
            if (lead && tid == 0) ctl->status = SEL_ERROR;
            return;
        }
        const double hm = scratch[110];
        const double tj = hm - sh / dn0;
        const bool evr = sum_risky(scratch[111], B) || !(hm == hm);
        for (uint32_t r = tid; r < n; r += P_THREADS) s_dl[r] = tj - s_dl[r];
        __syncthreads();
        if (wave == 0) p_argmin<(maxn + 63) / 64>(s_dl, s_ds, n, B, lane, scratch);
        __syncthreads();
        const double dmin0 = scratch[100], dsec0 = scratch[102], mean0 = scratch[103], sd0 = scratch[104];
        const uint32_t low0 = uint32_t(scratch[101]);
        const bool anyr0 = scratch[105] != 0.0;
        const double band0 = sel_band(tj + sh / dn0, B);
        if (anyr0 || evr || (n > 1 && dsec0 - dmin0 <= band0 && dsec0 < 1e6)) {
            if (lead && tid == 0) ctl->status = SEL_NEED_SETUP;
            return;
        }
        st.sumH = sh;
        st.total_jsd = tj;
        st.li = low0;
        st.band = band0;
        st.thr = tj + DVS_EPS;
        st.mean_d = mean0;
        st.std_d = sd0;
        st.cov_d = sd0 / mean0;
        {
            const T *lrow = mat + s_pos[low0] * B;
            const double ltot = s_tot[low0], lrt = s_rt[low0];
            T lv[P_J];
#pragma unroll
            for (int j = 0; j < P_J; j++) {
                const uint64_t i = uint64_t(j) * P_THREADS + tid;
                if (i < B) lv[j] = lrow[i];
            }
#pragma unroll
            for (int j = 0; j < P_J; j++) {
// ... 46 lines not shown

    [[maybe_unused]] const uint32_t own_slot = one_job ? blockIdx.x / K : 0u;
    [[maybe_unused]] const bool use_own = OWN && one_job;
    if constexpr (OWN) {
        bool slots_ok = true;
        for (uint32_t r = tid; r < st.n; r += P_THREADS) {
            const uint32_t a = s_slot[r];
            if (a < st.n) s_inv[a] = r;
            else slots_ok = false;
        }
        if (__syncthreads_or(slots_ok ? 0 : 1)) {
            if (lead && tid == 0) ctl->why[7]++;
            return;
        }
        if (use_own && has_job && own_slot < st.n) {
            const T *mrow = mat + s_pos[s_inv[own_slot]] * B;
#pragma unroll
            for (int j = 0; j < P_J; j++) {
                const uint64_t i = uint64_t(j) * P_THREADS + tid;
                s_own[uint32_t(tid) * P_J + j] = i < B ? mrow[i] : T(0);
            }
        }
    }
    if constexpr (SMALL) {
        const uint32_t rows_cap = sync->small_rows;
        bool fits = B == 4096 && st.n <= rows_cap;
        for (uint32_t r = 0; r < st.n; r++) fits = fits && s_slot[r] < rows_cap;
        if (!fits) return;
        for (uint32_t r = 0; r < st.n; r++) {
            const T *mrow = mat + s_pos[r] * B;
            T cv[P_J];
#pragma unroll
            for (int j = 0; j < P_J; j++) cv[j] = mrow[uint64_t(j) * P_THREADS + tid];
            uint4 q;
            q.x = uint32_t(cv[0]) | (uint32_t(cv[1]) << 16);
            q.y = uint32_t(cv[2]) | (uint32_t(cv[3]) << 16);
            q.z = uint32_t(cv[4]) | (uint32_t(cv[5]) << 16);
            q.w = uint32_t(cv[6]) | (uint32_t(cv[7]) << 16);
            *reinterpret_cast<uint4 *>(s_rows + uint64_t(s_slot[r]) * 4096 + uint32_t(tid) * 8) = q;
        }
    }
    if (sync->no_coarse & 2u) st.thr = 1e300;
#ifdef DVS_PERSIST_STAMPS
    unsigned long long *s_dbg = reinterpret_cast<unsigned long long *>(smem + sync->lds_bytes - 128);
    if (tid < 16) s_dbg[tid] = 0ull;
    __syncthreads();
    unsigned long long t_prev = __builtin_amdgcn_s_memrealtime();
#ifdef DVS_PROBE
#define P_PROBE_BEGIN(id)                                                                          \
    do {                                                                                           \
        if ((id) == DVS_PROBE && (blockIdx.x == 0 || blockIdx.x == n_work - 1) && tid == 0)        \
            t_prev = __builtin_amdgcn_s_memrealtime();                                             \
    } while (0)
#define P_PROBE_END(id)                                                                            \
    do {                                                                                           \
        if ((id) == DVS_PROBE && (blockIdx.x == 0 || blockIdx.x == n_work - 1) && tid == 0) {      \
            s_dbg[0] += __builtin_amdgcn_s_memrealtime() - t_prev;                                 \
            s_dbg[1] += 1;                                                                         \
        }                                                                                          \
    } while (0)
#define P_STAMP(k) do { } while (0)
#define P_STAMP_B0(k) do { } while (0)
#define P_TRACE(which) do { } while (0)
#define P_TRACE_G(slot) do { } while (0)
#else
#define P_PROBE_BEGIN(id) do { } while (0)
#define P_PROBE_END(id) do { } while (0)
#define P_STAMP(k)                                                         \
    do {                                                                   \
        if ((lead || blockIdx.x == 0) && tid == 0) {                       \
            const unsigned long long t_now = __builtin_amdgcn_s_memrealtime(); \
            s_dbg[k] += t_now - t_prev;                                    \
            t_prev = t_now;                                                \
        }                                                                  \
    } while (0)
#define P_STAMP_B0(k)                                                      \
    do {                                                                   \
        if (blockIdx.x == 0 && !lead && tid == 0) {                        \
            const unsigned long long t_now = __builtin_amdgcn_s_memrealtime(); \
            s_dbg[k] += t_now - t_prev;                                    \
            t_prev = t_now;                                                \
        }                                                                  \
    } while (0)
#define P_TRACE(which)                                                                             \
    do {                                                                                           \
        if (tid == 0 && (epoch == 12 || epoch == 24 || epoch == 36 || epoch == 48))               \
            sync->trace[epoch / 12 - 1][which][blockIdx.x] = __builtin_amdgcn_s_memrealtime();     \
    } while (0)
#define P_TRACE_G(slot)                                                                            \
    do {                                                                                           \
        if (tid == 0 && (epoch == 12 || epoch == 24 || epoch == 36 || epoch == 48))               \
            sync->trace[epoch / 12 - 1][3][slot] = __builtin_amdgcn_s_memrealtime();               \
    } while (0)
#endif
#else
#define P_STAMP(k) do { } while (0)
#define P_STAMP_B0(k) do { } while (0)
#define P_TRACE(which) do { } while (0)
#define P_TRACE_G(slot) do { } while (0)
#define P_PROBE_BEGIN(id) do { } while (0)
#define P_PROBE_END(id) do { } while (0)
#endif
#ifdef DVS_PERSIST_CHAOS
#define P_CHAOS(k)                                                                                         \
    do {                                                                                                   \
        uint32_t h_ = (epoch * 0x9E3779B1u) ^ ((blockIdx.x + 1u) * 0x85EBCA77u) ^ (uint32_t(k) * 0xC2B2AE3Du); \
        h_ ^= h_ >> 15;                                                                                    \
        h_ *= 0x27D4EB2Fu;                                                                                 \
        h_ ^= h_ >> 13;                                                                                    \
        if ((h_ & 15u) == 0u)                                                                              \
            for (uint32_t z_ = (h_ >> 8) & 31u; z_ > 0; z_--) __builtin_amdgcn_s_sleep(12);               \
        if ((h_ & 0xFFF0u) == 0x1230u)       \
            for (uint32_t z_ = 0; z_ < 160; z_++) __builtin_amdgcn_s_sleep(14);                            \
    } while (0)
#else
#define P_CHAOS(k) do { } while (0)
#endif
    for (;;) {
        uint64_t B = B0;
        int tid = tid0;
        asm volatile("" : "+s"(B));
        asm volatile("" : "+v"(tid));
        const uint32_t lane = uint32_t(tid) & 63u, wave = uint32_t(tid) >> 6;
        if (epoch >= P_EPOCH_MAX) {
            bail = true;
            break;
        }
        PRel *myrel = &sync->rel[blockIdx.x & 7u];
        PWin win;
        win.epoch = epoch;
        win.hintp = &myrel->hint;
        win.rel = sync->rel;
        win.wgev = s_win;
        win.nlist = reinterpret_cast<uint32_t *>(s_win + 1);
        win.mysoft = &sync->soft[epoch & 1u][blockIdx.x][0];
        if (tid == 0) {
            s_win[0] = p_word(epoch, SEL_NONE, false);
            *win.nlist = 0u;
        }
        __syncthreads();
        P_PROBE_END(6);
        P_PROBE_BEGIN(1);
        P_CHAOS(1);
        P_STAMP_B0(9);
        P_TRACE(0);
#ifdef DVS_PERSIST_STAMPS
        const unsigned long long t_window = __builtin_amdgcn_s_memrealtime();
#endif
        const uint64_t end = umin64(st.cursor + uint64_t(st.window), st.npos);
        const uint64_t nrows = end - st.cursor;
        if ((!lead && !gath) || G == 1) {
            if (wgmode && COARSE && B == 4096 && coarse_on) {
                if constexpr (COARSE)
                    p_scan_rows_wg_stream<T>(mat, d.totals, d.rowH, sl, slf, st, st.sumH - s_mH[st.li], win,
                                             blockIdx.x, nwg, nrows, scratch + 32, nread, nprecise, nmid);
            } else if (wgmode)
                p_scan_rows_wg<T, COARSE>(mat, d.totals, d.rowH, sl, slf, B, st, st.sumH - s_mH[st.li], win,
                                          blockIdx.x, nwg, nrows, scratch + 32, nread, nprecise, nmid, coarse_on);
            else
                p_scan_rows<T, COARSE>(mat, d.totals, d.rowH, sl, slf, B, st, st.sumH - s_mH[st.li], win,
                                       uint64_t(blockIdx.x) * wpb + wave, nwaves, nrows, lane, nread, nprecise, nmid, coarse_on,
                                       true);
        }
        double fr[P_J];
        [[maybe_unused]] T craw[P_J];
        [[maybe_unused]] uint64_t craw_pos = SEL_NONE;
        [[maybe_unused]] uint32_t craw_tot = 1;
        [[maybe_unused]] double craw_H = 0.0;
        [[maybe_unused]] uint64_t fr_pos = SEL_NONE;
        [[maybe_unused]] uint64_t spec_job_pos = SEL_NONE;
        [[maybe_unused]] double spec_th = 0.0, spec_ts = 0.0;
        [[maybe_unused]] auto fetch_raw = [&](uint64_t q) {
            if (craw_pos != q) {
                const T *gp = mat + q * B;
#pragma unroll
                for (int j = 0; j < P_J; j++) {
                    const uint64_t i = uint64_t(j) * P_THREADS + tid;
                    craw[j] = i < B ? gp[i] : T(0);
                }
                craw_tot = d.totals[q];
                craw_H = d.rowH[q];
                craw_pos = q;
            }
        };
        [[maybe_unused]] auto small_job = [&](uint32_t r, uint32_t part_i, uint32_t at, uint32_t n_, double &th, double &ts) {
            const double dn_ = double(n_), rn_ = 1.0 / dn_, rdiv_ = 1.0 / (dn_ - 1.0);
            const bool is_new = r == n_ - 1;
            uint32_t mcv[P_J];
#pragma unroll
            for (int j = 0; j < P_J; j++) mcv[j] = 0u;
            double mtot = 1.0, mrt = 1.0;
            if (r < n_ && !is_new) {
                if constexpr (SMALL) {
                    const uint4 q = *reinterpret_cast<const uint4 *>(s_rows + uint64_t(s_slot[at]) * 4096 + uint32_t(tid) * 8);
                    const uint32_t qw[4] = {q.x, q.y, q.z, q.w};
#pragma unroll
                    for (int j = 0; j < P_J; j++) mcv[j] = (qw[j >> 1] >> ((j & 1) * 16)) & 0xFFFFu;
                } else if (use_own) {
#pragma unroll
                    for (int j = 0; j < P_J; j++) mcv[j] = uint32_t(s_own[uint32_t(tid) * P_J + j]);
                } else {
                    const T *mrow = mat + s_pos[at] * B;
#pragma unroll
                    for (int j = 0; j < P_J; j++) {
                        const uint64_t i = uint64_t(j) * P_THREADS + tid;
                        if ((uint32_t(j) & (K - 1)) == part_i && i < B) mcv[j] = uint32_t(mrow[i]);
                    }
                }
                mtot = s_tot[at];
                mrt = s_rt[at];
            }
            double h = 0.0, sv = 0.0;
#pragma unroll
            for (int j = 0; j < P_J; j++) {
                if ((uint32_t(j) & (K - 1)) == part_i && uint64_t(j) * P_THREADS + tid < B) {
                    double v = sl[uint64_t(j) * P_THREADS + tid];
                    if (v <= DVS_EPS) v = 0.0;
                    const double sn = v + fr[j];
                    double u;
                    if (r == n_) {
                        u = sn * rn_;
                    } else {
                        u = (sn - (is_new ? fr[j] : exact_div_u32(double(mcv[j]), mtot, mrt))) * rdiv_;
                        if (u <= DVS_EPS) u = 0.0;
                    }
                    if (u > 0.0) h -= u * log2_tab(u, s_ltab);
                    sv += u;
                }
            }
            h = dvs_wave_sum_dpp(h);
            sv = dvs_wave_sum_dpp(sv);
            __syncthreads();
            if (lane == 0) {
                scratch[64 + wave] = h;
                scratch[80 + wave] = sv;
            }
            __syncthreads();
            th = ts = 0.0;
            if (tid < 8) {
                for (uint32_t w = 0; w < P_THREADS / 64; w++) {
                    th += scratch[64 + w];
                    ts += scratch[80 + w];
                }
            }
        };
        [[maybe_unused]] auto big_job = [&](uint32_t r, uint32_t part_i, uint32_t at, uint32_t n_, const T *rq, double tq,
                                            double rtq, double &th, double &ts) {
            const double dn_ = double(n_), rn_ = 1.0 / dn_, rdiv_ = 1.0 / (dn_ - 1.0);
            const bool is_new = r == n_ - 1;
            const bool need_m = r < n_ && !is_new;
            const T *mrow = mat + (need_m ? s_pos[at] : 0) * B;
            const double mtot = need_m ? s_tot[at] : 1.0, mrt = need_m ? s_rt[at] : 1.0;
            double h = 0.0, sv = 0.0;
            constexpr int NQ = sizeof(T) <= 4 ? 8 : 4;
            for (uint32_t c0 = part_i; c0 < nchunk; c0 += NQ * K) {
                T cv[NQ], mv[NQ];
#pragma unroll
                for (int q = 0; q < NQ; q++) {
                    const uint64_t i = uint64_t(c0 + q * K) * P_THREADS + tid;
                    if (c0 + q * K < nchunk && i < B) {
                        cv[q] = rq[i];
                        if (need_m) mv[q] = mrow[i];
                    }
                }
                double u[NQ];
#pragma unroll
                for (int q = 0; q < NQ; q++) {
                    const uint64_t i = uint64_t(c0 + q * K) * P_THREADS + tid;
                    u[q] = 0.0;
                    if (c0 + q * K < nchunk && i < B) {
                        double v = sl[i];
                        if (v <= DVS_EPS) v = 0.0;
                        const double f = count_freq_x(cv[q], tq, rtq);
                        u[q] = v + f;
                    }
                }
                if (r == n_) {
#pragma unroll
                    for (int q = 0; q < NQ; q++) u[q] = fmax(u[q] * rn_, 0.0);
                } else if (is_new) {
#pragma unroll
                    for (int q = 0; q < NQ; q++) {
                        const uint64_t i = uint64_t(c0 + q * K) * P_THREADS + tid;
                        if (c0 + q * K < nchunk && i < B) {
                            double x = (u[q] - count_freq_x(cv[q], tq, rtq)) * rdiv_;
                            if (x <= DVS_EPS) x = 0.0;
                            u[q] = x;
                        }
                    }
                } else {
#pragma unroll
                    for (int q = 0; q < NQ; q++) {
                        const uint64_t i = uint64_t(c0 + q * K) * P_THREADS + tid;
                        if (c0 + q * K < nchunk && i < B) {
                            double x = (u[q] - count_freq_x(mv[q], mtot, mrt)) * rdiv_;
                            if (x <= DVS_EPS) x = 0.0;
                            u[q] = x;
                        }
                    }
                }
                double mnt[NQ];
                int ex[NQ];
                double2 tb[NQ];
#pragma unroll
                for (int q = 0; q < NQ; q++) {
                    const double x = fmax(u[q], 1e-300);
                    mnt[q] = __builtin_amdgcn_frexp_mant(x);
                    ex[q] = __builtin_amdgcn_frexp_exp(x);
                    tb[q] = s_ltab[(uint32_t(__double2hiint(mnt[q])) >> 13) & 127u];
                }
#pragma unroll
                for (int q = 0; q < NQ; q++) {
                    const double r_ = fma(mnt[q], tb[q].y, -1.0);
// ... 1810 lines not shown
```

### diverseseq_amd/csrc/select.h

```cpp
#pragma once

#include "dvs_internal.h"

#define SEL_NONE 0xFFFFFFFFFFFFFFFFull
#define SEL_SEEDS_AT 512

enum : uint32_t { SEL_RUN = 0, SEL_DONE = 1, SEL_ARBITER = 2, SEL_ERROR = 3,
                  SEL_NEED_SETUP = 4 };
enum : uint32_t { ARB_RESOLVE = 1, ARB_FINALIZE = 2 };
enum : uint32_t { FORCE_NONE = 0, FORCE_ACCEPT = 1, FORCE_REJECT = 2, FORCE_COMMIT = 3, FORCE_ROLLBACK = 4 };

struct SelCtl {
    unsigned long long cursor;
    unsigned long long npos;
    unsigned long long event_pos;
    unsigned long long arb_pos;
    unsigned long long rows_scored, rows_rechecked;
    unsigned long long rows_coarse_passed;
    unsigned long long rows_before_launch;
    uint32_t window, window_min, window_max;
    uint32_t status, arb_stage, forced, forced_lowest;
    uint32_t size, lowest, mode, max_size, stat;
    uint32_t ev_kind;
    uint32_t ev_n;
    uint32_t ev_risky;
    uint32_t s_is_resum;
    uint32_t mb_rows;
    uint32_t mb_stuck;
    uint32_t n_windows, n_events, n_accepts;
    uint32_t n_logged;
    double total_jsd, sum_entropy;
    double thr, band;
    double he_base;
    double mean_delta, std_delta, cov_delta;
    double t_total_jsd, t_sum_entropy;
    double last_jsd;
    double arb_H;
    double wscale;
    uint32_t why[8];
};

struct SelDev {
    SelCtl *ctl = nullptr;
    uint64_t B = 0;
    uint32_t nlabels = 0;
    const uint32_t *order = nullptr;
    const uint32_t *labels = nullptr;
    const uint32_t *totals = nullptr;
    const double *rowH = nullptr;
    double *S = nullptr;
    double *Stmp = nullptr;
    double *base = nullptr;
    double *cand = nullptr;
    double *M = nullptr;
    double *mH = nullptr;
    double *mDelta = nullptr;
    double *dtmp = nullptr;
    double *dsum = nullptr;
    uint32_t *mLabel = nullptr;
    unsigned long long *mPos = nullptr;
    uint32_t *ord = nullptr;
    uint8_t *inset = nullptr;
    uint32_t *wg_rows = nullptr;
    unsigned long long *evlog_pos = nullptr;
    uint32_t *evlog_kind = nullptr;
    const double *gather_all = nullptr;
    uint32_t gather_world = 0;
    double *rowlog = nullptr;
    uint32_t rowlog_cap = 0;
};

struct dvs_select {
    dvs_ctx *ctx = nullptr;
    dvs_select_params params{};
    const dvs_matrix *mat = nullptr;
    int mat_kind = 0;
    uint64_t npos = 0;
    uint32_t cap = 0;
    SelDev dev;
    SelCtl *h_ctl = nullptr;
    SelCtl ctl0{};
    std::vector<uint32_t> h_order, h_labels;
    std::vector<uint32_t> h_out_labels;
    std::vector<uint64_t> seed_positions;
    uint32_t scan_grid = 0, loo_grid = 0;
    size_t scan_lds = 0;
    bool base_in_lds = true;
    bool scan_hot = false;
    bool persist = false;
    uint32_t persist_grid = 0, persist_maxn = 0, persist_maxjobs = 0;
    bool persist_small = false;
    uint32_t persist_small_rows = 0;
    size_t persist_lds = 0;
    void *psync = nullptr;
    std::vector<unsigned char> h_psync;
    std::vector<unsigned char> h_psync_head;
    void *ppart = nullptr;
    double *d_mbres = nullptr;
    uint32_t mb_jw = 0;
    uint32_t mb_launched = 0;
    void *psync_head = nullptr, *ppart_head = nullptr;
    bool persist_seeded = false;
    bool seeded_start = false;
    bool head_prepared = false;
    bool persist_prepared = false;
    bool used_side_streams = false;
    hipEvent_t ev_side_done = nullptr;
    void *d_seed_list = nullptr;
    bool seed_list_in_ctl = false;
    bool inset_clean = false;
    hipStream_t setup_side = nullptr;
    bool head_phase = false;
    int batch = 16;
    bool time_scan = false;
    std::vector<hipEvent_t> ev_pool;
    size_t ev_used = 0;
    double scan_ms = 0.0;
    double scan_ms_last = 0.0;
    uint64_t scan_launches = 0;
    uint32_t n_arbitrated = 0;
    double arbiter_ms = 0.0;
    bool fast_step = false;
    bool fs_need_scan = false;
    unsigned long long *h_fshist = nullptr;
    unsigned long long fs_launches = 0;
    unsigned long long fs_peek_floor = 0;
    double *fs_slot = nullptr;
    double *fs_packed = nullptr;
    double *d_jobres = nullptr;
    void *d_fsync = nullptr;
    uint32_t fs_K = 1, fs_jobs = 0, fs_grid = 0;
    size_t fs_lds = 0;
    std::vector<double> h_rowlog;
    uint64_t rowlog_have = 0;
    uint32_t steps_since_poll = 0;
    void *arbiter = nullptr;
};

int dvs_select_arbitrate(dvs_ctx *ctx, dvs_select *s);
void dvs_select_arbiter_free(dvs_select *s);

int dvs_persist_setup(dvs_ctx *ctx, dvs_select *s);
int dvs_persist_launch(dvs_ctx *ctx, dvs_select *s);
int dvs_persist_launch_head(dvs_ctx *ctx, dvs_select *s, uint32_t grid, uint32_t stop_at, hipStream_t on);
int dvs_persist_prepare_main(dvs_ctx *ctx, dvs_select *s);
int dvs_persist_prepare_head(dvs_ctx *ctx, dvs_select *s, uint32_t stop_at, hipStream_t on);
void dvs_persist_debug_report(dvs_ctx *ctx, const dvs_select *s);
void dvs_persist_debug_done(const SelCtl &c);

hipEvent_t dvs_scan_timing_start(dvs_ctx *ctx, dvs_select *s, hipStream_t on);
```

### diverseseq_amd/csrc/select.hip

```cpp
#include "dvs_internal.h"
#include "select.h"
#include "select_dev.h"

#include <algorithm>
#include <chrono>
#include <type_traits>
#include <cmath>
#include <cstring>
#include <cstdlib>
#include <memory>

namespace {

constexpr int SCAN_THREADS = 512;
constexpr int WIDE_THREADS = 1024;
constexpr int LOO_THREADS = 256;

template <typename T>
__device__ __forceinline__ void scan_rows_hot(SelCtl *ctl, const T *__restrict__ mat,
                                              const uint32_t *__restrict__ totals,
                                              const double *__restrict__ rowH, const double *bvec,
                                              uint64_t B, const ScanState &st, uint64_t first,
                                              uint64_t stride, uint32_t lane, uint32_t &nread,
                                              uint32_t &nprecise) {
// ... 2161 lines not shown
        {(void **)&d.M, size_t(cap) * B * 8, "d.M"},
        {(void **)&d.mH, size_t(cap) * 8, "d.mH"},
        {(void **)&d.mDelta, size_t(cap) * 8, "d.mDelta"},
        {(void **)&d.dtmp, size_t(cap) * 8, "d.dtmp"},
        {(void **)&d.dsum, size_t(cap) * 8, "d.dsum"},
        {(void **)&d.mLabel, size_t(cap) * 4, "d.mLabel"},
        {(void **)&d.mPos, size_t(cap) * 8, "d.mPos"},
        {(void **)&d.ord, size_t(cap) * 4, "d.ord"},
        {(void **)&d.inset, std::max<size_t>(nlabels, 1), "d.inset"},
        {(void **)&d.wg_rows, size_t(s->scan_grid) * 8, "d.wg_rows"},
        {(void **)&d.evlog_pos, nlog * 8, "d.evlog_pos"},
        {(void **)&d.evlog_kind, nlog * 4, "d.evlog_kind"},
    };
    for (const auto &b : blocks)
        if (int rc = dvs_dev_alloc(ctx, b.ptr, b.bytes, b.what)) return rc;
    if (s->params.flags & DVS_SELECT_STEPWISE) {
        uint64_t ring = std::min<uint64_t>(256, std::max<uint64_t>(32, (uint64_t(256) << 20) / (B * 8)));
        if (ctx->knobs.test_rowlog_ring >= 4) ring = ctx->knobs.test_rowlog_ring;
        d.rowlog_cap = uint32_t(ring);
        if (int rc = dvs_dev_alloc(ctx, (void **)&d.rowlog, size_t(ring) * B * 8, "d.rowlog")) return rc;
        uint32_t fsK = 1;
        while (uint64_t(cap + 1) * fsK * 2 <= 96 && uint64_t(fsK) * 2 * FS_JOB_THREADS <= B) fsK *= 2;
        const size_t fs_lds = ((B + 1) & ~1ull) * 16 + size_t(cap + 1) * 3 * 8 + size_t(cap + 1) * fsK * 7 * 8 + 64;
        if (s->params.mode == DVS_MODE_NMOST && s->params.n_seed >= 2 && !labels && !ctx->knobs.no_fast_step &&
            fs_lds <= ctx->lds_per_block && uint64_t(cap + 1) <= FS_MAXJOBS) {
            s->fs_K = fsK;
            s->fs_lds = fs_lds;
            s->fs_grid = uint32_t(ctx->n_cu);
            if (int rc = dvs_dev_alloc(ctx, (void **)&s->d_jobres, size_t(FS_MAXJOBS) * FS_RES * 8 + 8 * 8 * 1024, "s->d_jobres")) return rc;
            DVS_HIP(ctx, hipMemsetAsync(s->d_jobres, 0, size_t(FS_MAXJOBS) * FS_RES * 8 + 8 * 8 * 1024, ctx->stream));
            if (int rc = dvs_dev_alloc(ctx, (void **)&s->d_fsync, sizeof(FsSync), "s->d_fsync")) return rc;
            DVS_HIP(ctx, hipMemsetAsync(s->d_fsync, 0, sizeof(FsSync), ctx->stream));
            void *hh = nullptr;
            if (int rc = dvs_pinned_get(ctx, &hh)) return rc;
            memset(hh, 0, 4096);
            s->h_fshist = static_cast<unsigned long long *>(hh);
            s->fast_step = true;
            s->fs_need_scan = true;
        }
    }
    if (order) {
        if (int rc = dvs_dev_alloc(ctx, (void **)&d.order, size_t(npos) * 4, "d.order")) return rc;
        DVS_HIP(ctx, hipMemcpyAsync((void *)d.order, order, size_t(npos) * 4, hipMemcpyHostToDevice, ctx->stream));
    }
    if (labels) {
        if (int rc = dvs_dev_alloc(ctx, (void **)&d.labels, size_t(npos) * 4, "d.labels")) return rc;
        DVS_HIP(ctx, hipMemcpyAsync((void *)d.labels, labels, size_t(npos) * 4, hipMemcpyHostToDevice, ctx->stream));
    }
    static_assert(sizeof(SelCtl) <= 4096, "control block must fit a cached pinned block");
    return dvs_pinned_get(ctx, (void **)&s->h_ctl);
}

static int sel_prepare_engine(dvs_ctx *ctx, dvs_select *s, const uint32_t *order, const uint32_t *labels) {
    SelDev &d = s->dev;
    const dvs_matrix *m = s->mat;
    const uint32_t n_seed = s->params.n_seed, nlabels = d.nlabels;
    int rc = dvs_persist_setup(ctx, s);
    if (rc) return rc;
    sel_plan_setup_stream(ctx, s);
    if (s->setup_side) s->used_side_streams = true;
    DVS_HIP(ctx, hipMemsetAsync(d.inset, 0, std::max<size_t>(nlabels, 1), s->setup_side ? s->setup_side : ctx->stream));
    s->inset_clean = true;
    DVS_HIP(ctx, hipMemsetAsync(d.wg_rows, 0, size_t(s->scan_grid) * 8, s->setup_side ? s->setup_side : ctx->stream));
    s->seeded_start = s->persist && s->params.mode == DVS_MODE_NMOST && d.B <= 4096 && !order && !labels &&
                      !(s->params.flags & DVS_SELECT_STEPWISE) && n_seed >= 2 && n_seed <= 32 && !ctx->knobs.persist_no_seeded;
    s->persist_seeded = s->seeded_start;
    if (size_t(n_seed) * sizeof(uint64_t) <= 4096 - SEL_SEEDS_AT) {
        s->d_seed_list = reinterpret_cast<unsigned char *>(d.ctl) + SEL_SEEDS_AT;
        s->seed_list_in_ctl = true;
    } else if (s->seeded_start) {
        if ((rc = dvs_dev_alloc(ctx, &s->d_seed_list, size_t(n_seed) * sizeof(uint64_t), "seed list"))) return rc;
    }
    if (s->persist && m->rest_beside_head && ctx->stream_head && m->head_rows_built && s->params.mode == DVS_MODE_NMOST &&
        !order && !labels) {
        s->used_side_streams = true;
        return dvs_persist_prepare_head(ctx, s, m->head_rows_built, ctx->stream_head);
    }
    return DVS_OK;
}

static int sel_read_seeds(dvs_ctx *ctx, dvs_select *s, const uint32_t *order) {
    const dvs_matrix *m = s->mat;
    const uint32_t n_seed = s->params.n_seed;
    std::vector<uint32_t> h_tot(n_seed);
    int rc = dvs_matrix_settle(ctx, m);
    if (rc) return rc;
    hipError_t ce = hipSuccess;
    if (!order && n_seed && n_seed <= m->h_head_totals.size()) {
        std::copy(m->h_head_totals.begin(), m->h_head_totals.begin() + n_seed, h_tot.begin());
    } else if (!order && n_seed) {
        ce = hipMemcpyAsync(h_tot.data(), m->d_totals, size_t(n_seed) * 4, hipMemcpyDeviceToHost, ctx->stream);
    } else {
        for (uint64_t p = 0; p < n_seed && ce == hipSuccess; p++)
            ce = hipMemcpyAsync(&h_tot[p], m->d_totals + order[p], 4, hipMemcpyDeviceToHost, ctx->stream);
    }
    if ((order || n_seed > m->h_head_totals.size()) &&
        (hipStreamSynchronize(ctx->stream) != hipSuccess || ce != hipSuccess))
        return dvs_set_error(ctx, DVS_ERR_RUNTIME, "reading the seed rows' totals failed");
    std::vector<uint64_t> &seeds = s->seed_positions;
    for (uint64_t p = 0; p < n_seed; p++)
        if (h_tot[p] > 0) seeds.push_back(p);
    if (seeds.size() < 2)
        return seeds.empty() ? dvs_set_error(ctx, DVS_ERR_VALUE, "records cannot be empty")
                             : dvs_set_error(ctx, DVS_ERR_VALUE, "must have > 1 KmerSeq");
    return DVS_OK;
}

static void sel_init_ctl(dvs_ctx *ctx, dvs_select *s) {
    SelCtl c;
    std::memset(&c, 0, sizeof c);
    c.cursor = s->params.n_seed;
    c.npos = s->npos;
    c.event_pos = SEL_NONE;
    c.status = SEL_RUN;
    c.size = uint32_t(s->seed_positions.size());
    c.mode = s->params.mode;
    c.max_size = s->params.max_size;
    c.stat = s->params.stat;
    c.forced = FORCE_NONE;
    c.forced_lowest = 0xFFFFFFFFu;
    c.band = 0.0;
    c.wscale = 4.0;
    if (ctx->knobs.persist_no_events) c.wscale = 1e5;
    s->ctl0 = c;
}

extern "C" int dvs_select_run(dvs_ctx *ctx, const dvs_matrix *m, const uint32_t *order,
                              const uint32_t *labels, uint64_t npos,
                              const dvs_select_params *params, dvs_select **out) {
    if (!ctx || !m || !params || !out) return dvs_set_error(ctx, DVS_ERR_VALUE, "null argument");
    *out = nullptr;
    DVS_HIP(ctx, hipSetDevice(ctx->device));
    SelArgs a;
    int rc = sel_check_args(ctx, m, order, labels, npos, params, a);
    if (rc) return rc;
    labels = a.labels;
    std::unique_ptr<dvs_select, void (*)(dvs_select *)> s(new dvs_select(), sel_free);
    s->ctx = ctx;
    dvs_ctx_retain(ctx);
    s->params = *params;
    s->params.n_seed = a.n_seed;
    s->params.max_size = a.max_size;
    s->mat = m;
    s->mat_kind = m->kind;
    s->npos = npos;
    s->h_order.assign(order ? order : nullptr, order ? order + npos : nullptr);
    s->h_labels.assign(labels ? labels : nullptr, labels ? labels + npos : nullptr);
    if (a.caller_labels) s->h_out_labels.assign(a.caller_labels, a.caller_labels + npos);
    s->cap = a.cap;
    s->dev.B = m->nbins;
    s->dev.nlabels = a.nlabels;
    s->dev.totals = m->d_totals;
    s->dev.rowH = m->d_entropy;
    if ((rc = sel_geometry(ctx, s.get(), order, labels)) || (rc = sel_alloc(ctx, s.get(), order, labels)) ||
        (rc = sel_prepare_engine(ctx, s.get(), order, labels)) || (rc = sel_read_seeds(ctx, s.get(), order)))
        return rc;
    sel_init_ctl(ctx, s.get());
    if ((rc = dvs_mat_dispatch(m, [&](auto *mp) { return sel_start(ctx, s.get(), mp); }))) return rc;
    *out = s.release();
    return DVS_OK;
}

extern "C" void dvs_select_destroy(dvs_select *s) { sel_free(s); }

extern "C" int dvs_select_get_summary(dvs_ctx *ctx, const dvs_select *s, dvs_select_summary *out) {
    if (!s || !out) return dvs_set_error(ctx, DVS_ERR_VALUE, "null argument");
    const SelCtl &c = *s->h_ctl;
    std::memset(out, 0, sizeof *out);
    out->size = c.size;
    out->lowest_index = c.lowest;
    out->total_jsd = c.total_jsd;
    out->mean_delta_jsd = c.mean_delta;
    out->std_delta_jsd = c.std_delta;
    out->cov_delta_jsd = c.cov_delta;
    out->summed_entropies = c.sum_entropy;
    out->rows_scored = c.rows_scored;
    out->rows_rechecked = c.rows_rechecked;
    out->n_windows = c.n_windows;
    out->n_events = c.n_events;
    out->n_accepts = c.n_accepts;
    out->n_arbitrated = s->n_arbitrated;
    out->scan_ms = s->scan_ms;
    out->scan_launches = s->scan_launches;
    out->engine = s->persist ? 1u : 0u;
    out->rows_coarse_passed = uint32_t(std::min<unsigned long long>(c.rows_coarse_passed, 0xFFFFFFFFull));
    out->scan_ms_last = s->scan_ms_last;
    out->rows_scored_last = s->persist ? c.rows_scored - std::min(c.rows_before_launch, c.rows_scored) : 0;
    out->arbiter_ms = s->arbiter_ms;
    return DVS_OK;
}

extern "C" int dvs_select_get_members(dvs_ctx *ctx, const dvs_select *s, uint64_t *positions,
                                      uint32_t *labels, double *delta_jsd, double *entropy,
                                      double *freqs) {
    if (!s) return dvs_set_error(ctx, DVS_ERR_VALUE, "null argument");
    const uint32_t n = s->h_ctl->size;
    const uint64_t B = s->dev.B;
    std::vector<uint32_t> ord(n), lab(s->cap);
    std::vector<uint64_t> pos(s->cap);
    std::vector<double> mh(s->cap);
    DVS_HIP(ctx, hipMemcpy(ord.data(), s->dev.ord, size_t(n) * 4, hipMemcpyDeviceToHost));
    DVS_HIP(ctx, hipMemcpy(lab.data(), s->dev.mLabel, size_t(s->cap) * 4, hipMemcpyDeviceToHost));
    DVS_HIP(ctx, hipMemcpy(pos.data(), s->dev.mPos, size_t(s->cap) * 8, hipMemcpyDeviceToHost));
    DVS_HIP(ctx, hipMemcpy(mh.data(), s->dev.mH, size_t(s->cap) * 8, hipMemcpyDeviceToHost));
    if (delta_jsd)
        DVS_HIP(ctx, hipMemcpy(delta_jsd, s->dev.mDelta, size_t(n) * 8, hipMemcpyDeviceToHost));
    for (uint32_t i = 0; i < n; i++) {
        const uint32_t sl = ord[i];
        if (positions) positions[i] = pos[sl];
        if (labels) labels[i] = s->h_out_labels.empty() ? lab[sl] : s->h_out_labels[pos[sl]];
        if (entropy) entropy[i] = mh[sl];
        if (freqs)
            DVS_HIP(ctx, hipMemcpy(freqs + uint64_t(i) * B, s->dev.M + uint64_t(sl) * B, B * 8,
                                   hipMemcpyDeviceToHost));
    }
    return DVS_OK;
}

extern "C" int dvs_select_delta_jsd(dvs_ctx *ctx, const dvs_select *s, const dvs_matrix *q,
                                    const uint32_t *qlabels, double *out) {
    if (!s || !q || !out) return dvs_set_error(ctx, DVS_ERR_VALUE, "null argument");
    if (q->nbins != s->dev.B)
        return dvs_set_error(ctx, DVS_ERR_VALUE, "query matrix has %llu bins, the set %llu",
                             (unsigned long long)q->nbins, (unsigned long long)s->dev.B);
    if (q->nrows == 0) return DVS_OK;
    DVS_HIP(ctx, hipSetDevice(ctx->device));
    double *d_out = nullptr;
    uint32_t *d_lab = nullptr;
    std::vector<uint32_t> qtrans;
    if (qlabels && !s->h_out_labels.empty()) {
        const uint32_t n = s->h_ctl->size;
        std::vector<uint64_t> pos(s->cap);
        std::vector<uint32_t> ord(n);
        DVS_HIP(ctx, hipMemcpy(ord.data(), s->dev.ord, size_t(n) * 4, hipMemcpyDeviceToHost));
        DVS_HIP(ctx, hipMemcpy(pos.data(), s->dev.mPos, size_t(s->cap) * 8, hipMemcpyDeviceToHost));
        std::map<uint32_t, uint32_t> member_of;
        for (uint32_t i = 0; i < n; i++) {
            const uint64_t p = pos[ord[i]];
            if (s->h_out_labels[p] != 0xFFFFFFFFu) member_of[s->h_out_labels[p]] = uint32_t(p);
        }
        qtrans.resize(q->nrows);
        for (uint32_t i = 0; i < q->nrows; i++) {
            auto it = member_of.find(qlabels[i]);
            qtrans[i] = it == member_of.end() ? 0xFFFFFFFFu : it->second;
        }
        qlabels = qtrans.data();
    }
    DVS_HIP(ctx, hipMalloc(&d_out, size_t(q->nrows) * 8));
    if (qlabels) {
        DVS_HIP(ctx, hipMalloc(&d_lab, size_t(q->nrows) * 4));
        DVS_HIP(ctx, hipMemcpyAsync(d_lab, qlabels, size_t(q->nrows) * 4, hipMemcpyHostToDevice,
                                    ctx->stream));
    }
    dvs_mat_dispatch(q, [&](auto *qp) {
        using T = std::remove_cv_t<std::remove_pointer_t<decltype(qp)>>;
        hipLaunchKernelGGL((score_kernel<T>), dim3(q->nrows), dim3(LOO_THREADS), 0, ctx->stream, s->dev, qp,
                           q->d_totals, q->d_entropy, d_lab, d_out);
        return 0;
    });
    DVS_HIP(ctx, hipGetLastError());
    DVS_HIP(ctx, hipMemcpyAsync(out, d_out, size_t(q->nrows) * 8, hipMemcpyDeviceToHost, ctx->stream));
    DVS_HIP(ctx, hipStreamSynchronize(ctx->stream));
    (void)hipFree(d_out);
    if (d_lab) (void)hipFree(d_lab);
    return DVS_OK;
}

__global__ void log2_acc_selftest_kernel(double *out) {
    __shared__ double2 tab[128];
    if (threadIdx.x < 128) log2_tab_fill(tab, threadIdx.x);
    __syncthreads();
    const uint32_t t = blockIdx.x * blockDim.x + threadIdx.x;
    double worst = 0.0;
    for (int e = -78; e <= 1; e++) {
        const double m = 1.0 + double(t) / 131072.0;
        const double xs[3] = {ldexp(m, e), ldexp(1.4142135623730951 + (double(t) - 65536.0) * 1e-12, e),
                              ldexp(1.0 + (double(t) - 65536.0) * 2.2e-16, e)};
        for (int q = 0; q < 3; q++) {
            const double ref = log2(xs[q]);
            const double err = fabs(log2_acc(xs[q]) - ref) / fmax(1.0, fabs(ref));
            const double err_t = fabs(log2_tab(xs[q], tab) - ref) / fmax(1.0, fabs(ref));
            worst = fmax(worst, fmax(err, err_t));
        }
    }
    for (int o = 32; o > 0; o >>= 1) worst = fmax(worst, __shfl_xor(worst, o, 64));
    if ((threadIdx.x & 63) == 0)
        atomicMax(reinterpret_cast<unsigned long long *>(out), (unsigned long long)__double_as_longlong(worst));
}

__global__ void log2_f32_selftest_kernel(double *out) {
    double worst = 0.0;
    const uint64_t first = uint64_t(26) << 23, last = uint64_t(128) << 23;
    for (uint64_t b = first + uint64_t(blockIdx.x) * blockDim.x + threadIdx.x; b < last;
         b += uint64_t(gridDim.x) * blockDim.x) {
        const float y = __uint_as_float(uint32_t(b));
        const double ref = log2(double(y));
        const double err = fabs(double(__builtin_amdgcn_logf(y)) - ref) / (0x1p-23 * fmax(1.0, fabs(ref)));
        worst = fmax(worst, err);
    }
    for (int o = 32; o > 0; o >>= 1) worst = fmax(worst, __shfl_xor(worst, o, 64));
    if ((threadIdx.x & 63) == 0)
        atomicMax(reinterpret_cast<unsigned long long *>(out), (unsigned long long)__double_as_longlong(worst));
}

__global__ void exact_div_selftest_kernel(unsigned long long *bad) {
    const uint64_t t = uint64_t(blockIdx.x) * blockDim.x + threadIdx.x;
// ... 265 lines not shown
```

### diverseseq_amd/csrc/select_dev.h

```cpp
#pragma once

#include "select.h"

namespace {

__device__ __forceinline__ double log2_acc(double x) {
    double m = __builtin_amdgcn_frexp_mant(x);
    int e = __builtin_amdgcn_frexp_exp(x);
    if (m < 0.70710678118654752) {
        m *= 2.0;
        e -= 1;
    }
    const double f = m - 1.0;
    const double s = f / (2.0 + f);
    const double z = s * s;
    double p = 1.0 / 19.0;
    p = fma(p, z, 1.0 / 17.0);
    p = fma(p, z, 1.0 / 15.0);
    p = fma(p, z, 1.0 / 13.0);
    p = fma(p, z, 1.0 / 11.0);
    p = fma(p, z, 1.0 / 9.0);
    p = fma(p, z, 1.0 / 7.0);
    p = fma(p, z, 1.0 / 5.0);
    p = fma(p, z, 1.0 / 3.0);
    const double lm = fma(s * z, p, s);
    return fma(lm, 2.8853900817779268, double(e));
}

__device__ __forceinline__ void log2_tab_fill(double2 *tab, int i) {
    const double c = 0.5 + (double(i) + 0.5) / 256.0;
    tab[i] = make_double2(log2_acc(c), 1.0 / c);
}
__device__ __forceinline__ double log2_tab(double x, const double2 *tab) {
    const double m = __builtin_amdgcn_frexp_mant(x);
    const int e = __builtin_amdgcn_frexp_exp(x);
    const uint32_t i = (uint32_t(__double2hiint(m)) >> 13) & 127u;
    const double2 t = tab[i];
    const double r = fma(m, t.y, -1.0);
    double p = 1.0 / 7.0;
    p = fma(p, r, -1.0 / 6.0);
    p = fma(p, r, 1.0 / 5.0);
    p = fma(p, r, -1.0 / 4.0);
    p = fma(p, r, 1.0 / 3.0);
    p = fma(p, r, -1.0 / 2.0);
    p = fma(p, r, 1.0);
    return fma(p * r, 1.4426950408889634, double(e) + t.x);
}

struct Ent {
    double h = 0.0, sum = 0.0, mn = 0.0;
    __device__ __forceinline__ void add(double x) {
        if (x > 0.0) h -= x * log2_acc(x);
        sum += x;
        mn = fmin(mn, x);
    }
    __device__ __forceinline__ void add(double x, const double2 *tab) {
        if (x > 0.0) h -= x * log2_tab(x, tab);
        sum += x;
        mn = fmin(mn, x);
    }
};

__device__ __forceinline__ uint64_t umin64(uint64_t a, uint64_t b) { return a < b ? a : b; }

__device__ __forceinline__ double sel_band(double hmean, uint64_t B) {
    return 4.0 * double(B) * DVS_EPS * fmax(1.0, fabs(hmean));
}

__device__ __forceinline__ double row_value(const uint32_t *row, uint64_t i) { return double(row[i]); }
__device__ __forceinline__ double row_value(const uint16_t *row, uint64_t i) { return double(row[i]); }
__device__ __forceinline__ double row_value(const double *row, uint64_t i) { return row[i]; }

constexpr double FAST_BAND = 4e-7;
constexpr int SCAN_CH = 16;

__device__ __forceinline__ double fast_neg_xlog2x(double x) {
    const double xm = fmax(x, 1e-300);
    const double m = __builtin_amdgcn_frexp_mant(xm);
    const int e = __builtin_amdgcn_frexp_exp(xm);
    const float l = __builtin_amdgcn_logf(float(m));
    return -xm * (double(e) + double(l));
}

typedef float dvs_f2 __attribute__((ext_vector_type(2)));
__device__ __forceinline__ double coarse_band(uint64_t B) {
    return 1.25 * 0x1p-24 * (9.0 * log2(double(B)) + 7.4);
}
__device__ __forceinline__ float coarse_sl(double v, double rn) { return v == 0.0 ? 1e-30f : float(v * rn); }
__device__ __forceinline__ float coarse4(const uint4 c, const float4 b, const dvs_f2 r2) {
    const dvs_f2 c01 = {float(c.x), float(c.y)}, c23 = {float(c.z), float(c.w)};
    const dvs_f2 y01 = __builtin_elementwise_fma(c01, r2, (dvs_f2){b.x, b.y});
    const dvs_f2 y23 = __builtin_elementwise_fma(c23, r2, (dvs_f2){b.z, b.w});
    const dvs_f2 l01 = {__builtin_amdgcn_logf(y01.x), __builtin_amdgcn_logf(y01.y)};
    const dvs_f2 l23 = {__builtin_amdgcn_logf(y23.x), __builtin_amdgcn_logf(y23.y)};
    const dvs_f2 s = y01 * l01 + y23 * l23;
    return s.x + s.y;
}

__device__ __forceinline__ float coarse4(const uint2 c, const float4 b, const dvs_f2 r2) {
    const dvs_f2 c01 = {float(c.x & 0xFFFFu), float(c.x >> 16)}, c23 = {float(c.y & 0xFFFFu), float(c.y >> 16)};
    const dvs_f2 y01 = __builtin_elementwise_fma(c01, r2, (dvs_f2){b.x, b.y});
    const dvs_f2 y23 = __builtin_elementwise_fma(c23, r2, (dvs_f2){b.z, b.w});
    const dvs_f2 l01 = {__builtin_amdgcn_logf(y01.x), __builtin_amdgcn_logf(y01.y)};
    const dvs_f2 l23 = {__builtin_amdgcn_logf(y23.x), __builtin_amdgcn_logf(y23.y)};
    const dvs_f2 s = y01 * l01 + y23 * l23;
    return s.x + s.y;
}

__device__ __forceinline__ void coarse8(const uint4 c, const float *b, const dvs_f2 r2, double &a0, double &a1) {
    a0 += double(coarse4(make_uint2(c.x, c.y), *reinterpret_cast<const float4 *>(b), r2));
    a1 += double(coarse4(make_uint2(c.z, c.w), *reinterpret_cast<const float4 *>(b + 4), r2));
}

template <typename T> struct Raw4;
template <> struct Raw4<uint32_t> {
    uint4 c;
    __device__ __forceinline__ void load(const uint32_t *p) { c = *reinterpret_cast<const uint4 *>(p); }
    __device__ __forceinline__ void pin() { asm volatile("" : "+v"(c.x), "+v"(c.y), "+v"(c.z), "+v"(c.w)); }
    __device__ __forceinline__ void get(double &v0, double &v1, double &v2, double &v3) const {
        v0 = double(c.x); v1 = double(c.y); v2 = double(c.z); v3 = double(c.w);
    }
};
template <> struct Raw4<uint16_t> {
    uint2 c;
    __device__ __forceinline__ void load(const uint16_t *p) { c = *reinterpret_cast<const uint2 *>(p); }
    __device__ __forceinline__ void pin() { asm volatile("" : "+v"(c.x), "+v"(c.y)); }
    __device__ __forceinline__ void get(double &v0, double &v1, double &v2, double &v3) const {
        v0 = double(c.x & 0xFFFFu); v1 = double(c.x >> 16); v2 = double(c.y & 0xFFFFu); v3 = double(c.y >> 16);
    }
};
template <> struct Raw4<double> {
    double2 a, b;
    __device__ __forceinline__ void load(const double *p) {
        a = *reinterpret_cast<const double2 *>(p);
        b = *reinterpret_cast<const double2 *>(p + 2);
    }
    __device__ __forceinline__ void pin() {}
    __device__ __forceinline__ void get(double &v0, double &v1, double &v2, double &v3) const {
        v0 = a.x; v1 = a.y; v2 = b.x; v3 = b.y;
    }
};

template <typename T>
__device__ __forceinline__ void load4(const T *rp, uint64_t i, double &v0, double &v1, double &v2,
                                      double &v3) {
    if constexpr (sizeof(T) == 4) {
        const uint4 c = *reinterpret_cast<const uint4 *>(rp + i);
        v0 = double(c.x); v1 = double(c.y); v2 = double(c.z); v3 = double(c.w);
    } else if constexpr (sizeof(T) == 2) {
        const uint2 c = *reinterpret_cast<const uint2 *>(rp + i);
        v0 = double(c.x & 0xFFFFu); v1 = double(c.x >> 16); v2 = double(c.y & 0xFFFFu); v3 = double(c.y >> 16);
    } else {
        const double2 a = *reinterpret_cast<const double2 *>(rp + i);
        const double2 b = *reinterpret_cast<const double2 *>(rp + i + 2);
        v0 = a.x; v1 = a.y; v2 = b.x; v3 = b.y;
    }
}

struct ScanState {
    uint64_t cursor, nrows;
    double thr_lo, thr_fast, thr_sure, he_base, dsize;
};

__device__ __forceinline__ void fast4(const double2 b01, const double2 b23, double v0, double v1,
                                      double v2, double v3, double rinv, double &a0, double &a1,
                                      double &a2, double &a3, double &xmin) {
    const double x0 = fma(v0, rinv, b01.x), x1 = fma(v1, rinv, b01.y);
    const double x2 = fma(v2, rinv, b23.x), x3 = fma(v3, rinv, b23.y);
    a0 += fast_neg_xlog2x(x0);
    a1 += fast_neg_xlog2x(x1);
    a2 += fast_neg_xlog2x(x2);
    a3 += fast_neg_xlog2x(x3);
    xmin = fmin(fmin(xmin, fmin(x0, x1)), fmin(x2, x3));
}

template <typename T>
__device__ __forceinline__ bool precise_row(const T *rp, const double *bvec, uint64_t B, double rinv,
                                            double mean_entropy, double thr_lo, uint32_t lane) {
    Ent e;
    if ((B & 255) == 0) {
        for (uint64_t i0 = 0; i0 < B; i0 += 256) {
            const uint64_t i = i0 + lane * 4;
            double v0, v1, v2, v3;
            load4(rp, i, v0, v1, v2, v3);
            e.add(fma(v0, rinv, bvec[i]));
            e.add(fma(v1, rinv, bvec[i + 1]));
            e.add(fma(v2, rinv, bvec[i + 2]));
            e.add(fma(v3, rinv, bvec[i + 3]));
        }
    } else {
        for (uint64_t i = lane; i < B; i += 64) e.add(fma(row_value(rp, i), rinv, bvec[i]));
    }
    const double h = dvs_wave_sum(e.h);
    return h - mean_entropy > thr_lo;
}

__device__ __forceinline__ double cand_freq(const uint32_t *row, uint64_t i, double tot) {
    return double(row[i]) / tot;
}
__device__ __forceinline__ double cand_freq(const uint16_t *row, uint64_t i, double tot) { return double(row[i]) / tot; }
__device__ __forceinline__ double cand_freq(const double *row, uint64_t i, double) { return row[i]; }

__device__ __forceinline__ double exact_div_u32(double c, double tot, double rt) {
    const double q0 = c * rt;
    const double r0 = fma(-tot, q0, c);
    return fma(r0, rt, q0);
}
__device__ __forceinline__ double cand_freq_x(const uint32_t *row, uint64_t i, double tot, double rt) {
    return exact_div_u32(double(row[i]), tot, rt);
}
__device__ __forceinline__ double cand_freq_x(const uint16_t *row, uint64_t i, double tot, double rt) {
    return exact_div_u32(double(row[i]), tot, rt);
}
__device__ __forceinline__ double cand_freq_x(const double *row, uint64_t i, double, double) { return row[i]; }
__device__ __forceinline__ double count_freq_x(uint32_t c, double tot, double rt) { return exact_div_u32(double(c), tot, rt); }
__device__ __forceinline__ double count_freq_x(uint16_t c, double tot, double rt) { return exact_div_u32(double(c), tot, rt); }
__device__ __forceinline__ double count_freq_x(double f, double, double) { return f; }

__device__ __forceinline__ void block_red3(double &h, double &mn, double &sm, double *scratch) {
    const int lane = threadIdx.x & 63, wave = threadIdx.x >> 6;
    const int nwave = (blockDim.x + 63) >> 6;
#pragma unroll
    for (int o = 32; o > 0; o >>= 1) {
        const double t0 = __shfl_xor(h, o, 64), t1 = __shfl_xor(mn, o, 64), t2 = __shfl_xor(sm, o, 64);
        h += t0;
        mn = fmin(mn, t1);
        sm += t2;
    }
    __syncthreads();
    if (lane == 0) {
        scratch[wave] = h;
        scratch[16 + wave] = mn;
        scratch[32 + wave] = sm;
    }
    __syncthreads();
    double a = 0.0, b = scratch[16], c = 0.0;
    for (int i = 0; i < nwave; i++) {
        a += scratch[i];
        b = fmin(b, scratch[16 + i]);
        c += scratch[32 + i];
    }
    h = a;
    mn = b;
    sm = c;
}

__device__ __forceinline__ uint32_t sel_next_window(uint64_t cursor, uint32_t size, uint32_t wmin,
                                                    uint32_t wmax, double wscale) {
    uint64_t w = uint64_t(double(cursor) * wscale / double(size ? size : 1u));
    if (w < wmin) w = wmin;
    if (w > wmax) w = wmax;
    return uint32_t(w);
}
__device__ __forceinline__ void ctl_next_window(SelCtl *ctl) {
    ctl->window = sel_next_window(ctl->cursor, ctl->size, ctl->window_min, ctl->window_max, ctl->wscale);
}

__device__ __forceinline__ bool sum_risky(double sum, uint64_t B) {
    return !(fabs(sum - 1.0) <= 0.25 * double(B) * DVS_EPS);
}


__device__ __forceinline__ void block_red5(double &a, double &mn, double &b, double &c, double &e,
                                           double *scratch) {
// ... 38 lines not shown
```

Baseline: 70.27 million.

## Add 8-bit count companion matrix for coarse k=6 scans

When the 16-bit count matrix has 4096 bins, the histogram kernel also writes an 8-bit packed companion matrix and totals. The totals carry a high-bit flag for rows whose counts exceed 255. The persistent select kernels read the 8-bit rows for the f32 coarse screen, halving the bytes streamed per row. Rows flagged wide skip the coarse decision and go to the precise path. The cost is extra HBM, an extra write pass at build time, and the 16-bit rows no longer being kept cache-hot beyond the head rows.

Result: no change. 69.28 million, median of 2 (-1.4%).

```diff
diff --git a/diverseseq_amd/csrc/api.cpp b/diverseseq_amd/csrc/api.cpp
--- a/diverseseq_amd/csrc/api.cpp
+++ b/diverseseq_amd/csrc/api.cpp
@@ -112,6 +112,7 @@
     k->no_uniform_offsets = on("DVS_NO_UNIFORM_OFFSETS");
     k->no_offsets_cache = on("DVS_NO_OFFSETS_CACHE");
     k->counts_u32 = on("DVS_COUNTS_U32");
+    k->no_counts8 = on("DVS_NO_COUNTS8");
     k->build_wait = on("DVS_BUILD_WAIT");
     k->no_packed_upload = on("DVS_NO_PACKED_UPLOAD");
     k->cu_mask_set = on("HSA_CU_MASK") || on("ROC_GLOBAL_CU_MASK");
@@ -131,6 +132,7 @@
     if (const char *lt = tk ? strstr(tk, "long_tile_") : nullptr) k->test_long_tile = uint32_t(strtoul(lt + 10, nullptr, 10));
     k->test_rowlog_ring = 0;
     if (const char *rr = tk ? strstr(tk, "rowlog_ring_") : nullptr) k->test_rowlog_ring = uint32_t(strtoul(rr + 12, nullptr, 10));
+    k->test_counts8_no_room = tk && strstr(tk, "counts8_no_room") != nullptr;
 }
 
 extern "C" {
@@ -292,6 +294,28 @@
     return DVS_OK;
 }
 
+static void matrix_alloc_counts8(dvs_ctx *ctx, dvs_matrix *m) {
+    if (m->kind != 2 || m->nbins != 4096 || !m->nrows || ctx->knobs.no_counts8 || ctx->knobs.test_counts8_no_room) return;
+    const size_t bytes = size_t(m->nrows) * m->nbins;
+    if (!ctx->pool.count((bytes + 4095) & ~size_t(4095))) {
+        size_t free_b = 0, total_b = 0;
+        if (hipMemGetInfo(&free_b, &total_b) != hipSuccess) {
+            (void)hipGetLastError();
+            return;
+        }
+        if (bytes + size_t(m->nrows) * 4 + (256u << 20) > free_b) return;
+    }
+    const std::string err = ctx->err;
+    if (dvs_dev_alloc(ctx, (void **)&m->d_counts8, bytes, "matrix counts (8-bit companion)") ||
+        dvs_dev_alloc(ctx, (void **)&m->d_tot8, size_t(m->nrows) * 4, "matrix totals (8-bit companion)")) {
+        dvs_dev_free(ctx, m->d_counts8);
+        dvs_dev_free(ctx, m->d_tot8);
+        m->d_counts8 = nullptr;
+        m->d_tot8 = nullptr;
+        ctx->err = err;
+    }
+}
+
 static int matrix_alloc(dvs_ctx *ctx, dvs_matrix *m) {
     const size_t cells = size_t(m->nrows) * m->nbins;
     const size_t bytes = cells * (m->kind == 0 ? 4 : m->kind == 2 ? 2 : 8);
@@ -311,6 +335,7 @@
     else rc = dvs_dev_alloc(ctx, (void **)&m->d_freqs, bytes ? bytes : 8, "matrix freqs");
     if (!rc) rc = dvs_dev_alloc(ctx, (void **)&m->d_totals, nr * 4, "matrix totals");
     if (!rc) rc = dvs_dev_alloc(ctx, (void **)&m->d_entropy, nr * 8, "matrix entropy");
+    if (!rc) matrix_alloc_counts8(ctx, m);
     return rc;
 }
 
diff --git a/diverseseq_amd/csrc/dvs_internal.h b/diverseseq_amd/csrc/dvs_internal.h
--- a/diverseseq_amd/csrc/dvs_internal.h
+++ b/diverseseq_amd/csrc/dvs_internal.h
@@ -18,6 +18,7 @@
     bool no_uniform_offsets = false;
     bool no_offsets_cache = false;
     bool counts_u32 = false;
+    bool no_counts8 = false;
     bool build_wait = false;
     bool no_packed_upload = false;
     bool cu_mask_set = false;
@@ -34,6 +35,7 @@
     bool test_persist_fake_error = false;
     uint32_t test_long_tile = 0;
     uint32_t test_rowlog_ring = 0;
+    bool test_counts8_no_room = false;
 };
 void dvs_knobs_from_env(dvs_knobs *k);
 
@@ -107,6 +109,8 @@
 struct dvs_matrix {
     int kind = 0;
     uint16_t *d_counts16 = nullptr;
+    uint8_t *d_counts8 = nullptr;
+    uint32_t *d_tot8 = nullptr;
     uint32_t nrows = 0;
     uint64_t nbins = 0;
     uint32_t k = 0, num_states = 0;
diff --git a/diverseseq_amd/csrc/kmer_hist.hip b/diverseseq_amd/csrc/kmer_hist.hip
--- a/diverseseq_amd/csrc/kmer_hist.hip
+++ b/diverseseq_amd/csrc/kmer_hist.hip
@@ -51,7 +51,8 @@
     const uint64_t *__restrict__ offsets,
     const KTile *__restrict__ tiles, uint32_t *__restrict__ counts, uint32_t *__restrict__ totals,
     double *__restrict__ entropy, const double *__restrict__ clog_tbl, uint32_t k, uint32_t ns,
-    uint64_t B, uint32_t hot_rows, uint32_t row0, uint64_t uni_base, uint64_t uni_stride) {
+    uint64_t B, uint32_t hot_rows, uint32_t row0, uint64_t uni_base, uint64_t uni_stride,
+    uint32_t *__restrict__ counts8, uint32_t *__restrict__ tot8, uint32_t hot16) {
     extern __shared__ __attribute__((aligned(16))) unsigned char smem[];
     KTile t;
     if (tiles) {
@@ -208,6 +209,8 @@
         uint4 *r4 = reinterpret_cast<uint4 *>(row);
         typedef uint32_t u32x4 __attribute__((ext_vector_type(4)));
         double sv[2] = {0.0, 0.0}, tv[2] = {0.0, 0.0};
+        uint32_t *row8 = OUT16 && counts8 ? counts8 + uint64_t(t.row) * (B / 4) : nullptr;
+        uint32_t orw = 0;
 #pragma unroll
         for (int half = 0; half < 2; half++)
             for (uint64_t u = uint64_t(tid) + 128u * half; u < B / 4; u += HIST_THREADS) {
@@ -216,8 +219,14 @@
                 if constexpr (OUT16) {
                     typedef uint32_t u32x2 __attribute__((ext_vector_type(2)));
                     uint2 *r2 = reinterpret_cast<uint2 *>(row);
-                    if (t.row < hot_rows) r2[u] = w;
+                    if (t.row < hot16) r2[u] = w;
                     else __builtin_nontemporal_store((u32x2){w.x, w.y}, reinterpret_cast<u32x2 *>(r2 + u));
+                    if (row8) {
+                        const uint32_t b4 = __builtin_amdgcn_perm(w.y, w.x, 0x06040200u);
+                        if (t.row < hot_rows) row8[u] = b4;
+                        else __builtin_nontemporal_store(b4, row8 + u);
+                        orw |= w.x | w.y;
+                    }
                 } else if (t.row < hot_rows) r4[u] = v;
                 else __builtin_nontemporal_store((u32x4){v.x, v.y, v.z, v.w}, reinterpret_cast<u32x4 *>(r4 + u));
                 if (((w.x | w.y) & 0xFF00FF00u) == 0) sv[half] += ((tbl[v.x] + tbl[v.y]) + tbl[v.z]) + tbl[v.w];
@@ -225,6 +234,7 @@
             }
         tv[0] = double(nvalid);
         const int lane = tid & 63, wave = tid >> 6;
+        const bool wide_w = __ballot((orw & 0xFF00FF00u) != 0u) != 0ull;
         double sums[2];
 #pragma unroll
         for (int q = 0; q < 2; q++) {
@@ -233,6 +243,7 @@
             if (lane == 0) {
                 scratch[wave] = a;
                 scratch[wave + 2] = b;
+                if (q) scratch[wave + 4] = wide_w ? 1.0 : 0.0;
             }
             __syncthreads();
             double acc = 0.0;
@@ -242,6 +253,7 @@
         if (tid == 0) {
             totals[t.row] = uint32_t(sums[1]);
             entropy[t.row] = sums[1] > 0.0 ? log2(sums[1]) - sums[0] / sums[1] : 0.0;
+            if (row8) tot8[t.row] = uint32_t(sums[1]) | (scratch[4] + scratch[5] != 0.0 ? 0x80000000u : 0u);
         }
     } else if (t.single) {
         double s = 0.0, tot = 0.0;
@@ -408,6 +420,10 @@
     dvs_dev_free(m->ctx, m->d_counts);
     dvs_dev_free(m->ctx, m->d_counts16);
     m->d_counts16 = nullptr;
+    dvs_dev_free(m->ctx, m->d_counts8);
+    dvs_dev_free(m->ctx, m->d_tot8);
+    m->d_counts8 = nullptr;
+    m->d_tot8 = nullptr;
     dvs_dev_free(m->ctx, m->d_freqs);
     dvs_dev_free(m->ctx, m->d_totals);
     dvs_dev_free(m->ctx, m->d_entropy);
@@ -602,7 +618,8 @@
         if (!rc)                                                                                 \
             hipLaunchKernelGGL((kmer_hist_kernel<NS4, LH, false, false, PKD>), dim3(GRID), dim3(NTHR), lds,  \
                                ctx->stream, d_seqs, d_pmask, nbytes, d_off, TILES, m->d_counts,  \
-                               m->d_totals, m->d_entropy, ctx->d_clog_tbl, k, ns, B, HOT, 0u, uni_base, uni_stride);   \
+                               m->d_totals, m->d_entropy, ctx->d_clog_tbl, k, ns, B, HOT, 0u, uni_base, uni_stride,  \
+                               nullptr, nullptr, HOT);                                                 \
     } while (0)
 #define DVS_LAUNCH_HIST_ANY(GRID, TILES, NTHR, HOT)                            \
     do {                                                                  \
@@ -613,7 +630,8 @@
         else if (lds_hist) DVS_LAUNCH_HIST(false, true, false, GRID, TILES, NTHR, HOT);    \
         else DVS_LAUNCH_HIST(false, false, false, GRID, TILES, NTHR, HOT);                 \
     } while (0)
-    uint32_t hot_rows = uint32_t(std::min<uint64_t>(nseq, (192ull << 20) / (B * (m->kind == 2 ? 2 : 4))));
+    uint32_t *out8 = reinterpret_cast<uint32_t *>(m->d_counts8);
+    uint32_t hot_rows = uint32_t(std::min<uint64_t>(nseq, (192ull << 20) / (B * (m->kind == 2 ? (out8 ? 1 : 2) : 4))));
     const bool pk16 = lds_hist && (B & 3) == 0;
     uint32_t head_rows = 0;
     if (m->kind == 2 && no_wait) {
@@ -625,25 +643,28 @@
     if (m->kind == 2) {
         const size_t lds16 = ((B * 2 + 15) & ~15ull) + (CLOG_TBL + 32) * sizeof(double);
         uint32_t *out16 = reinterpret_cast<uint32_t *>(m->d_counts16);
-        auto launch16 = [&](uint32_t row0, uint32_t count, uint32_t hot_end, hipStream_t on) {
+        auto launch16 = [&](uint32_t row0, uint32_t count, uint32_t hot_end, uint32_t hot16_end, hipStream_t on) {
             if (packed) {
                 rc = set_dyn_lds(ctx, kmer_hist_kernel<true, true, true, true, true>, lds16);
                 if (!rc)
                     hipLaunchKernelGGL((kmer_hist_kernel<true, true, true, true, true>), dim3(count), dim3(128), lds16, on,
                                        d_seqs, d_pmask, nbytes, d_off, static_cast<const KTile *>(nullptr), out16,
-                                       m->d_totals, m->d_entropy, ctx->d_clog_tbl, k, ns, B, hot_end, row0, uni_base, uni_stride);
+                                       m->d_totals, m->d_entropy, ctx->d_clog_tbl, k, ns, B, hot_end, row0, uni_base, uni_stride,
+                                       out8, m->d_tot8, hot16_end);
             } else if (ns4) {
                 rc = set_dyn_lds(ctx, kmer_hist_kernel<true, true, true, true>, lds16);
                 if (!rc)
                     hipLaunchKernelGGL((kmer_hist_kernel<true, true, true, true>), dim3(count), dim3(128), lds16, on,
                                        d_seqs, d_pmask, nbytes, d_off, static_cast<const KTile *>(nullptr), out16,
-                                       m->d_totals, m->d_entropy, ctx->d_clog_tbl, k, ns, B, hot_end, row0, uni_base, uni_stride);
+                                       m->d_totals, m->d_entropy, ctx->d_clog_tbl, k, ns, B, hot_end, row0, uni_base, uni_stride,
+                                       out8, m->d_tot8, hot16_end);
             } else {
                 rc = set_dyn_lds(ctx, kmer_hist_kernel<false, true, true, true>, lds16);
                 if (!rc)
                     hipLaunchKernelGGL((kmer_hist_kernel<false, true, true, true>), dim3(count), dim3(128), lds16, on,
                                        d_seqs, d_pmask, nbytes, d_off, static_cast<const KTile *>(nullptr), out16,
-                                       m->d_totals, m->d_entropy, ctx->d_clog_tbl, k, ns, B, hot_end, row0, uni_base, uni_stride);
+                                       m->d_totals, m->d_entropy, ctx->d_clog_tbl, k, ns, B, hot_end, row0, uni_base, uni_stride,
+                                       out8, m->d_tot8, hot16_end);
             }
         };
         if (head_rows) {
@@ -651,7 +672,7 @@
             hipEvent_t ev_fork = split ? dvs_event_get(ctx) : nullptr;
             bool forked = ev_fork && hipEventRecord(ev_fork, ctx->stream) == hipSuccess &&
                           hipStreamWaitEvent(ctx->stream_rest, ev_fork, 0) == hipSuccess;
-            launch16(0, head_rows, head_rows, ctx->stream);
+            launch16(0, head_rows, head_rows, head_rows, ctx->stream);
             void *pin = nullptr;
             if (!rc && dvs_pinned_get(ctx, &pin) == DVS_OK) {
                 m->head_count = uint32_t(std::min<size_t>(head_rows, 4096 / sizeof(uint32_t)));
@@ -673,7 +694,8 @@
             if (!rc) {
                 const uint32_t hot_end = uint32_t(std::min<uint64_t>(nseq, uint64_t(head_rows) + hot_rows));
                 forked = forked && head_event_done;
-                launch16(head_rows, nseq - head_rows, hot_end, forked ? ctx->stream_rest : ctx->stream);
+                launch16(head_rows, nseq - head_rows, hot_end, out8 ? head_rows : hot_end,
+                         forked ? ctx->stream_rest : ctx->stream);
                 if (forked) {
                     hipEvent_t ev_join = dvs_event_get(ctx);
                     if (!ev_join || hipEventRecord(ev_join, ctx->stream_rest) != hipSuccess ||
@@ -688,7 +710,7 @@
             }
             if (ev_fork) dvs_event_put(ctx, ev_fork);
         } else {
-            launch16(0, nseq, hot_rows, ctx->stream);
+            launch16(0, nseq, hot_rows, out8 ? 0u : hot_rows, ctx->stream);
         }
     } else if (pk16) {
         const size_t lds16 = ((B * 2 + 15) & ~15ull) + (CLOG_TBL + 32) * sizeof(double);
@@ -697,19 +719,22 @@
             if (!rc)
                 hipLaunchKernelGGL((kmer_hist_kernel<true, true, true, false, true>), dim3(nseq), dim3(128), lds16, ctx->stream,
                                    d_seqs, d_pmask, nbytes, d_off, static_cast<const KTile *>(nullptr), m->d_counts,
-                                   m->d_totals, m->d_entropy, ctx->d_clog_tbl, k, ns, B, hot_rows, 0u, uni_base, uni_stride);
+                                   m->d_totals, m->d_entropy, ctx->d_clog_tbl, k, ns, B, hot_rows, 0u, uni_base, uni_stride,
+                                   nullptr, nullptr, hot_rows);
         } else if (ns4) {
             rc = set_dyn_lds(ctx, kmer_hist_kernel<true, true, true>, lds16);
             if (!rc)
                 hipLaunchKernelGGL((kmer_hist_kernel<true, true, true>), dim3(nseq), dim3(128), lds16, ctx->stream,
                                    d_seqs, d_pmask, nbytes, d_off, static_cast<const KTile *>(nullptr), m->d_counts,
-                                   m->d_totals, m->d_entropy, ctx->d_clog_tbl, k, ns, B, hot_rows, 0u, uni_base, uni_stride);
+                                   m->d_totals, m->d_entropy, ctx->d_clog_tbl, k, ns, B, hot_rows, 0u, uni_base, uni_stride,
+                                   nullptr, nullptr, hot_rows);
         } else {
             rc = set_dyn_lds(ctx, kmer_hist_kernel<false, true, true>, lds16);
             if (!rc)
                 hipLaunchKernelGGL((kmer_hist_kernel<false, true, true>), dim3(nseq), dim3(128), lds16, ctx->stream,
                                    d_seqs, d_pmask, nbytes, d_off, static_cast<const KTile *>(nullptr), m->d_counts,
-                                   m->d_totals, m->d_entropy, ctx->d_clog_tbl, k, ns, B, hot_rows, 0u, uni_base, uni_stride);
+                                   m->d_totals, m->d_entropy, ctx->d_clog_tbl, k, ns, B, hot_rows, 0u, uni_base, uni_stride,
+                                   nullptr, nullptr, hot_rows);
         }
     } else
         DVS_LAUNCH_HIST_ANY(nseq, static_cast<const KTile *>(nullptr), nthreads, hot_rows);
diff --git a/diverseseq_amd/csrc/persist.hip b/diverseseq_amd/csrc/persist.hip
--- a/diverseseq_amd/csrc/persist.hip
+++ b/diverseseq_amd/csrc/persist.hip
@@ -255,7 +255,7 @@
 }
 
 template <typename T, bool COARSE>
-__device__ __forceinline__ void p_scan_rows(const T *__restrict__ mat,
+__device__ __forceinline__ void p_scan_rows(const T *__restrict__ mat, const uint8_t *__restrict__ c8,
                                             const uint32_t *__restrict__ totals,
                                             const double *__restrict__ rowH, const double *sl,
                                             const float *slf, uint64_t B, const PState &st, double he_base,
@@ -275,21 +275,37 @@
         const uint64_t p = st.cursor + r;
         const T *rp = mat + p * B;
         const uint64_t ev = p_hint_pos(win);
-        const uint32_t tot = totals[p];
+        const uint32_t tw = totals[p];
         const double hrow = rowH[p];
+        const uint32_t tot = sizeof(T) == 2 ? tw & 0x7FFFFFFFu : tw;
+        const bool wide = sizeof(T) == 2 && (tw >> 31) != 0u;
         if (ev < p) break;
         if (tot == 0) continue;
         const double rt = 1.0 / double(tot);
         const double mean_entropy = (he_base + hrow) / dn;
         nread++;
         if constexpr (COARSE) {
-            if (vec && coarse_on) {
+            if (vec && coarse_on && wide) {
+                nmid++;
+            } else if (vec && coarse_on) {
                 const float rtn = float(rt * rn);
                 const dvs_f2 r2 = {rtn, rtn};
                 double c0 = 0.0, c1 = 0.0;
                 bool done16 = false;
                 if constexpr (sizeof(T) == 2) {
-                    if (B == 4096) {
+                    if (B == 4096 && c8) {
+                        const uint8_t *r8 = c8 + p * 4096;
+                        uint2 raw8[8];
+#pragma unroll
+                        for (int j = 0; j < 8; j++) raw8[j] = *reinterpret_cast<const uint2 *>(r8 + j * 512 + lane * 8);
+                        __builtin_amdgcn_sched_barrier(0);
+#pragma unroll
+                        for (int j = 0; j < 8; j++) {
+                            asm volatile("" : "+v"(raw8[j].x), "+v"(raw8[j].y));
+                            coarse8u8(raw8[j], slf + j * 512 + lane * 8, r2, c0, c1);
+                        }
+                        done16 = true;
+                    } else if (B == 4096) {
                         uint4 raw8[8];
 #pragma unroll
                         for (int j = 0; j < 8; j++) raw8[j] = *reinterpret_cast<const uint4 *>(rp + j * 512 + lane * 8);
@@ -532,7 +548,8 @@
 }
 
 template <typename T>
-__device__ __forceinline__ void p_scan_rows_wg_stream(const T *__restrict__ mat,
+__device__ __forceinline__ void p_scan_rows_wg_stream(const T *__restrict__ mat, const uint8_t *__restrict__ c8,
+                                                      const uint32_t *__restrict__ ctot,
                                                       const uint32_t *__restrict__ totals,
                                                       const double *__restrict__ rowH, const double *sl,
                                                       const float *slf, const PState &st, double he_base,
@@ -558,12 +575,18 @@
         const uint64_t p = st.cursor + r;
         const T *rp = mat + p * B;
         if constexpr (W16) {
-            w.q = *reinterpret_cast<const uint4 *>(rp + tid * 8);
+            if (c8) {
+                const uint2 q8 = *reinterpret_cast<const uint2 *>(c8 + p * B + tid * 8);
+                w.q.x = q8.x;
+                w.q.y = q8.y;
+            } else {
+                w.q = *reinterpret_cast<const uint4 *>(rp + tid * 8);
+            }
         } else {
             w.r0.load(rp + tid * 4);
             w.r1.load(rp + 2048 + tid * 4);
         }
-        w.tot = totals[p];
+        w.tot = ctot[p];
         if (wave == 0) {
             w.hrow = rowH[p];
             w.ev = poll ? p_hint_pos(win) : SEL_NONE;
@@ -572,13 +595,20 @@
     uint32_t par = 0;
     auto process = [&](Row &w, uint64_t r) -> bool {
         const uint64_t p = st.cursor + r;
-        const float rtn = w.tot ? float(rn / double(w.tot)) : 0.0f;
+        const uint32_t tot = W16 ? w.tot & 0x7FFFFFFFu : w.tot;
+        const bool wide = W16 && (w.tot >> 31) != 0u;
+        const float rtn = tot ? float(rn / double(tot)) : 0.0f;
         const dvs_f2 r2 = {rtn, rtn};
         double c;
         if constexpr (W16) {
-            asm volatile("" : "+v"(w.q.x), "+v"(w.q.y), "+v"(w.q.z), "+v"(w.q.w));
             double ca = 0.0, cb = 0.0;
-            coarse8(w.q, slf + tid * 8, r2, ca, cb);
+            if (c8) {
+                asm volatile("" : "+v"(w.q.x), "+v"(w.q.y));
+                coarse8u8(make_uint2(w.q.x, w.q.y), slf + tid * 8, r2, ca, cb);
+            } else {
+                asm volatile("" : "+v"(w.q.x), "+v"(w.q.y), "+v"(w.q.z), "+v"(w.q.w));
+                coarse8(w.q, slf + tid * 8, r2, ca, cb);
+            }
             c = ca + cb;
         } else {
             w.r0.pin();
@@ -598,16 +628,18 @@
         }
         __syncthreads();
         if ((unsigned long long)__double_as_longlong(slot[8]) < p) return false;
-        if (w.tot == 0) return true;
+        if (tot == 0) return true;
         double hc = 0.0;
 #pragma unroll
         for (int q = 0; q < P_THREADS / 64; q++) hc += slot[q];
         const double jf0 = -hc - (he_base + slot[9]) / dn;
         if (tid == 0) nread++;
-        if (!(jf0 > thr_c_lo)) return true;
-        if (jf0 > thr_c_hi) {
-            if (tid < 8) p_post_event_wave(win, p, true, tid);
-            return true;
+        if (!wide) {
+            if (!(jf0 > thr_c_lo)) return true;
+            if (jf0 > thr_c_hi) {
+                if (tid < 8) p_post_event_wave(win, p, true, tid);
+                return true;
+            }
         }
         if (tid == 0) {
             nmid++;
@@ -823,6 +855,7 @@
     const uint32_t wg_thresh = sync->wg_thresh;
     const double wg_scale = double(sync->wg_scale);
     const bool coarse_on = (sync->no_coarse & 1u) == 0;
+    const uint8_t *c8 = COARSE && sizeof(T) == 2 && B == 4096 ? d.counts8 : nullptr;
     bool wgmode = false;
     if (wg_thresh) st.window = p_next_window(st, nwg, wg_thresh, wg_scale, wgmode);
     const uint32_t nchunk = uint32_t((B + P_THREADS - 1) / P_THREADS);
@@ -1175,13 +1208,14 @@
         if ((!lead && !gath) || G == 1) {
             if (wgmode && COARSE && B == 4096 && coarse_on) {
                 if constexpr (COARSE)
-                    p_scan_rows_wg_stream<T>(mat, d.totals, d.rowH, sl, slf, st, st.sumH - s_mH[st.li], win,
-                                             blockIdx.x, nwg, nrows, scratch + 32, nread, nprecise, nmid);
+                    p_scan_rows_wg_stream<T>(mat, c8, c8 ? d.tot8 : d.totals, d.totals, d.rowH, sl, slf, st,
+                                             st.sumH - s_mH[st.li], win, blockIdx.x, nwg, nrows, scratch + 32, nread,
+                                             nprecise, nmid);
             } else if (wgmode)
                 p_scan_rows_wg<T, COARSE>(mat, d.totals, d.rowH, sl, slf, B, st, st.sumH - s_mH[st.li], win,
                                           blockIdx.x, nwg, nrows, scratch + 32, nread, nprecise, nmid, coarse_on);
             else
-                p_scan_rows<T, COARSE>(mat, d.totals, d.rowH, sl, slf, B, st, st.sumH - s_mH[st.li], win,
+                p_scan_rows<T, COARSE>(mat, c8, c8 ? d.tot8 : d.totals, d.rowH, sl, slf, B, st, st.sumH - s_mH[st.li], win,
                                        uint64_t(blockIdx.x) * wpb + wave, nwaves, nrows, lane, nread, nprecise, nmid, coarse_on,
                                        true);
         }
diff --git a/diverseseq_amd/csrc/select.h b/diverseseq_amd/csrc/select.h
--- a/diverseseq_amd/csrc/select.h
+++ b/diverseseq_amd/csrc/select.h
@@ -48,6 +48,8 @@
     const uint32_t *labels = nullptr;
     const uint32_t *totals = nullptr;
     const double *rowH = nullptr;
+    const uint8_t *counts8 = nullptr;
+    const uint32_t *tot8 = nullptr;
     double *S = nullptr;
     double *Stmp = nullptr;
     double *base = nullptr;
diff --git a/diverseseq_amd/csrc/select.hip b/diverseseq_amd/csrc/select.hip
--- a/diverseseq_amd/csrc/select.hip
+++ b/diverseseq_amd/csrc/select.hip
@@ -2337,6 +2337,10 @@
     s->dev.nlabels = a.nlabels;
     s->dev.totals = m->d_totals;
     s->dev.rowH = m->d_entropy;
+    if (m->d_counts8 && !ctx->knobs.no_counts8) {
+        s->dev.counts8 = m->d_counts8;
+        s->dev.tot8 = m->d_tot8;
+    }
     if ((rc = sel_geometry(ctx, s.get(), order, labels)) || (rc = sel_alloc(ctx, s.get(), order, labels)) ||
         (rc = sel_prepare_engine(ctx, s.get(), order, labels)) || (rc = sel_read_seeds(ctx, s.get(), order)))
         return rc;
diff --git a/diverseseq_amd/csrc/select_dev.h b/diverseseq_amd/csrc/select_dev.h
--- a/diverseseq_amd/csrc/select_dev.h
+++ b/diverseseq_amd/csrc/select_dev.h
@@ -110,6 +110,20 @@
 __device__ __forceinline__ void coarse8(const uint4 c, const float *b, const dvs_f2 r2, double &a0, double &a1) {
     a0 += double(coarse4(make_uint2(c.x, c.y), *reinterpret_cast<const float4 *>(b), r2));
     a1 += double(coarse4(make_uint2(c.z, c.w), *reinterpret_cast<const float4 *>(b + 4), r2));
+}
+
+__device__ __forceinline__ float coarse4u8(const uint32_t c, const float4 b, const dvs_f2 r2) {
+    const dvs_f2 c01 = {float(c & 0xFFu), float((c >> 8) & 0xFFu)}, c23 = {float((c >> 16) & 0xFFu), float(c >> 24)};
+    const dvs_f2 y01 = __builtin_elementwise_fma(c01, r2, (dvs_f2){b.x, b.y});
+    const dvs_f2 y23 = __builtin_elementwise_fma(c23, r2, (dvs_f2){b.z, b.w});
+    const dvs_f2 l01 = {__builtin_amdgcn_logf(y01.x), __builtin_amdgcn_logf(y01.y)};
+    const dvs_f2 l23 = {__builtin_amdgcn_logf(y23.x), __builtin_amdgcn_logf(y23.y)};
+    const dvs_f2 s = y01 * l01 + y23 * l23;
+    return s.x + s.y;
+}
+__device__ __forceinline__ void coarse8u8(const uint2 c, const float *b, const dvs_f2 r2, double &a0, double &a1) {
+    a0 += double(coarse4u8(c.x, *reinterpret_cast<const float4 *>(b), r2));
+    a1 += double(coarse4u8(c.y, *reinterpret_cast<const float4 *>(b + 4), r2));
 }
 
 template <typename T> struct Raw4;
```
